# umar-ahmed/webgpu-pathtracer

Measured on AMD Instinct MI355X. Metric: Mrays/s, higher is better.
Workload: dtype f32; 1 GPU; dragon-class procedural mesh (869882 triangles) + synthetic env map, 1920x1080, 8 bounces, 16 frames (= 16 spp) per step, 863 steps = 13808 spp; triangles=869882, bvh_nodes=1739763, max_bounces=8, parallelism=single GPU

## Files before the change

include/mi3pt.h:

```cpp
#ifndef MI3PT_H
#define MI3PT_H

#include <stddef.h>
#include <stdint.h>

#ifdef __cplusplus
extern "C" {
#endif

#define MI3PT_ABI_VERSION 4

typedef enum mi3pt_status {
    MI3PT_OK = 0,
    MI3PT_ERR_INVALID = 1,
    MI3PT_ERR_NO_DEVICE = 2,
    MI3PT_ERR_HIP = 3,
    MI3PT_ERR_STATE = 4
} mi3pt_status;

#define MI3PT_TRIANGLE_STRIDE 112
#define MI3PT_BVHNODE_STRIDE 48
#define MI3PT_MATERIAL_STRIDE 64
#define MI3PT_RAYTRACE_UNIFORMS_SIZE 96
#define MI3PT_ACCUMULATE_UNIFORMS_SIZE 16
// ... 47 lines not shown
int mi3pt_device_count(int *count);
int mi3pt_device_name(int device, char *name, size_t capacity);

int mi3pt_create(int device, mi3pt_ctx **out_ctx);
int mi3pt_destroy(mi3pt_ctx *ctx);
int mi3pt_create_group(const int *devices, int ndevices, int block_rows, mi3pt_ctx **out_ctx);
int mi3pt_group_size(mi3pt_ctx *ctx, int *members);
int mi3pt_group_member(mi3pt_ctx *ctx, int index, mi3pt_ctx **member);

int mi3pt_set_stream(mi3pt_ctx *ctx, void *hip_stream);
int mi3pt_set_storage(mi3pt_ctx *ctx, int storage );

int mi3pt_set_tile(mi3pt_ctx *ctx, int rank, int nranks, int block_rows);
int mi3pt_tile_local_rows(int height, int rank, int nranks, int block_rows);
int mi3pt_tile_global_row(int local_row, int rank, int nranks, int block_rows);
int mi3pt_tile_owner(int y, int nranks, int block_rows);

int mi3pt_upload_triangles(mi3pt_ctx *ctx, const void *bytes, size_t nbytes);
int mi3pt_upload_materials(mi3pt_ctx *ctx, const void *bytes, size_t nbytes);
int mi3pt_upload_bvh(mi3pt_ctx *ctx, const void *bytes, size_t nbytes);

int mi3pt_upload_environment(mi3pt_ctx *ctx, const float *rgba, int width, int height);
int mi3pt_upload_environment_cdf(mi3pt_ctx *ctx, const float *rgba, int width, int height);

int mi3pt_resize(mi3pt_ctx *ctx, int width, int height);
int mi3pt_reset(mi3pt_ctx *ctx);

int mi3pt_set_uniforms(mi3pt_ctx *ctx, int pass , const void *bytes, size_t nbytes);

int mi3pt_submit(mi3pt_ctx *ctx, unsigned pass_mask);
int mi3pt_submit_frames(mi3pt_ctx *ctx, unsigned pass_mask, uint32_t count);
int mi3pt_sync(mi3pt_ctx *ctx);
int mi3pt_set_present_mode(mi3pt_ctx *ctx, int mode );
int mi3pt_flush(mi3pt_ctx *ctx);
int mi3pt_batch_capacity(mi3pt_ctx *ctx, int *frames);

int mi3pt_read_texture(mi3pt_ctx *ctx, int which , float *dst, size_t nfloats);
int mi3pt_read_canvas_rgba8(mi3pt_ctx *ctx, uint8_t *dst, size_t nbytes);
int mi3pt_write_texture(mi3pt_ctx *ctx, int which , const float *src, size_t nfloats);

int mi3pt_accumulation_device_ptr(mi3pt_ctx *ctx, void **dev_ptr, size_t *nbytes);
int mi3pt_bind_accumulation(mi3pt_ctx *ctx, void *dev_ptr, size_t nbytes);

int mi3pt_enable_timing(mi3pt_ctx *ctx, int enabled);
int mi3pt_pass_time_us(mi3pt_ctx *ctx, int pass, float *microseconds);
int mi3pt_raytrace_launch_stats(mi3pt_ctx *ctx, int reset, double *total_ms, uint64_t *launches, uint64_t *frames);
int mi3pt_raytrace_launch_span(mi3pt_ctx *ctx, double *span_ms);

int mi3pt_get_counters(mi3pt_ctx *ctx, uint64_t out[MI3PT_CNT_COUNT]);
int mi3pt_reset_counters(mi3pt_ctx *ctx);

int mi3pt_set_kernel_variant(mi3pt_ctx *ctx, int variant);
typedef enum mi3pt_option {
    MI3PT_OPT_WALK_MIN = 0,
    MI3PT_OPT_LEAF_MIN = 1,
    MI3PT_OPT_SHADE_SPLIT = 2,
    MI3PT_OPT_TAIL_POLICY = 3,
    MI3PT_OPT_TOP_PACKETS = 4,
    MI3PT_OPT_TRI_PAIR = 5,
    MI3PT_OPT_JOB_REVERSE = 6,
    MI3PT_OPT_JOB_GROUP = 7,
    MI3PT_OPT_JOB_CHUNK = 8,
    MI3PT_OPT_BATCH_LIMIT = 9,
    MI3PT_OPT_BATCH = 10,
    MI3PT_OPT_WAVES_PER_CU = 11,
    MI3PT_OPT_CULL = 12,
    MI3PT_OPT_WIDE = 13,
    MI3PT_OPT_GATE = 14,
    MI3PT_OPT_GATE_TIMEOUT_MS = 22,
    MI3PT_OPT_GATE_RELEASES = 23,
    MI3PT_OPT_CAMERA_BASE = 25,
    MI3PT_OPT_PACKET_ORDER = 26,
    MI3PT_OPT_SIX_WAVES = 27,
    MI3PT_OPT_LAST_BUILD = 29,
    MI3PT_OPT_WALK_ADAPT = 30,
    MI3PT_OPT_COLLAPSE = 28,
    MI3PT_OPT_DEBUG_SUPPRESS_DRAIN = 24,
    MI3PT_OPT_SLOT_SETS = 15,
    MI3PT_OPT_PIPELINE = 16,
    MI3PT_OPT_PRESENT_DEPTH = 18,
    MI3PT_OPT_HOST_ANALYSES = 19,
    MI3PT_OPT_DIAG_LITE = 21,
    MI3PT_OPT_GATHER_STAGED = 20,
    MI3PT_OPT_COST_ORDER = 17
} mi3pt_option;
int mi3pt_debug_set_option(mi3pt_ctx *ctx, int option , int value);
int mi3pt_debug_get_option(mi3pt_ctx *ctx, int option , int *value);
int mi3pt_debug_active_variant(mi3pt_ctx *ctx, int *variant);
int mi3pt_debug_last_launch(mi3pt_ctx *ctx, int *kind, int *variant, int *lean, int *workgroups);
int mi3pt_set_env_sampling(mi3pt_ctx *ctx, int enabled);
int mi3pt_set_pipelining(mi3pt_ctx *ctx, int enabled);

int mi3pt_debug_intersect(mi3pt_ctx *ctx, const float *rays, size_t n, float *out);
int mi3pt_device_build_bvh(mi3pt_ctx *ctx, void *nodes_out, size_t nodes_capacity_bytes, size_t *nnodes_out, float *build_ms);

int mi3pt_debug_set_packet_layout(mi3pt_ctx *ctx, int layout);

int mi3pt_debug_math(mi3pt_ctx *ctx, int fn, const float *a, const float *b, float *out, size_t n);

int mi3pt_debug_wave_times(mi3pt_ctx *ctx, int enable, uint64_t *out, size_t capacity_slots, size_t *slots_out);

int mi3pt_host_build_bvh(const void *triangles, size_t ntris, void *nodes_out,
                         size_t nodes_capacity_bytes, size_t *nnodes_out, int nthreads);
int mi3pt_host_build_bvh_f64(const double *positions, size_t ntris, void *nodes_out,
                             size_t nodes_capacity_bytes, size_t *nnodes_out, int nthreads);
int mi3pt_host_env_cdf(const float *rgba, int width, int height, float *cdf_rgba_out);
int mi3pt_host_eight_wide_check(const void *nodes, size_t nodes_bytes, const void *triangles, size_t triangles_bytes, int greedy, uint64_t out[6]);

#ifdef __cplusplus
}
#endif
#endif
```

webgpu-pathtracer_amd/csrc/pt_context.hip:

```cpp
#include "../../include/mi3pt.h"
#include "pt_internal.h"
#include "pt_kernels.h"

#include <hip/hip_runtime.h>
#include <cmath>
#include <cstdio>
#include <cstdlib>
#include <array>
#include <cstring>
#include <string>
#include <utility>
#include <algorithm>
#include <vector>
#include <map>
#include <chrono>
#include <thread>

static thread_local std::string g_last_error;

int pt_set_error(int code, const std::string &msg)
{
    g_last_error = msg;
    return code;
}

#define HIP_TRY(expr)                                                                       \
    do {                                                                                    \
        hipError_t e_ = (expr);                                                             \
        if (e_ != hipSuccess)                                                               \
            return pt_set_error(MI3PT_ERR_HIP, std::string(#expr) + ": " + hipGetErrorString(e_)); \
    } while (0)

struct mi3pt_ctx {
    int device = 0;
    hipStream_t own_stream = nullptr;
    hipStream_t stream = nullptr;

    void *d_tris = nullptr, *d_nodes = nullptr, *d_mats = nullptr, *d_env = nullptr, *d_cdf = nullptr;
    void *d_packets = nullptr, *d_tripk = nullptr;
    void *d_leaf_rank = nullptr;
    int leaf_cap = 0;
    bool cull_stack_ok = false;
    size_t ntris = 0, nnodes = 0, nmats = 0, npackets = 0;
    uint32_t root_ref = 0;
    uint32_t scene_flags = 0;
    bool wide_root_nested = false;
    int64_t max_tri_ref = -1;
    int64_t max_mat_ref = -1;
    bool cull_enabled = true;
    bool cull_dirty = true;
    bool cull_ok = false;
    float cull_ka = 0.0f, cull_kb = 0.0f;
    bool wide_enabled = true;
#ifdef MI3PT_EXPERIMENTS
    bool exp_force_slow_slab = false;
    double exp_cull_scale = 1.0;
#endif
    int auto_wide_variant = 10;
    bool wide_ok = false;
    bool cwide_ok = false;
    void *d_cwide = nullptr, *d_tripk64 = nullptr;
    bool cw8_tried = false;
    bool cw8_ok = false;
    void *d_cw8 = nullptr, *d_tripk8 = nullptr;
    size_t ncw8 = 0, cw8_records = 0;
    int cw8_height = 0;
    void *d_wide = nullptr;
    size_t nwide = 0;
    int wide_leaf_cap = 0;
    uint32_t wide_root = 0;
    int num_cus = 256;
    pt::RtRoute last_route = { 0, 0, false, 0, 0, false, 0 };
    int layout = 0;
    bool layout_dirty = false;
    int cost_order = 0;
    int cost_state = 0;
    uint32_t *d_tile_cost = nullptr, *d_tile_perm[2] = { nullptr, nullptr };
    size_t cost_tiles = 0;
    int perm_cur = 0;
    hipEvent_t cost_event = nullptr, perm_used[2] = { nullptr, nullptr };
    bool perm_used_valid[2] = { false, false };
    hipStream_t cost_stream = nullptr;
    uint8_t cost_key[MI3PT_RAYTRACE_UNIFORMS_SIZE] = {};
    struct GroupState *group = nullptr;
    std::map<const void *, size_t> buf_bytes;
    uint64_t scene_epoch = 1;
    uint64_t host_analyses = 0;
    bool tree_proper = false;
    bool layout_active = false;
    void *d_tris_perm = nullptr;

    int width = 0, height = 0, local_rows = 0;
    int rank = 0, nranks = 1, block_rows = 8;
    int next_rank = 0, next_nranks = 1, next_block_rows = 8;
    bool partial() const { return nranks != 1; }
    float4 *d_radiance = nullptr, *d_accum_own = nullptr, *d_accum = nullptr, *d_canvas = nullptr;
    float4 *d_slots[3] = { nullptr, nullptr, nullptr };
    int slots_alloc[3] = { 0, 0, 0 };
    int slot_sets = 2;
    int batch_cap = 1;
    float4 *last_radiance = nullptr;
    float4 *d_cam_base[2] = { nullptr, nullptr };
    uint8_t cam_base_key[2][80] = {};
    bool cam_base_valid[2] = { false, false };
    bool cam_base_enabled = true;
    int collapse = -1;
    int six_waves = -1;
    int packet_order = 0;
    uint32_t *d_canvas8 = nullptr;
    bool output_is_accum = false;
    uint64_t *d_block_counters = nullptr;
    uint32_t *d_tile_counter = nullptr;
    int job_reverse = 1;
    int job_group = -1;
    int tri_pair = 1;
    int job_chunk = PT_DEFAULT_JOB_CHUNK;
    uint32_t *d_drain_flag = nullptr;
    bool gate_enabled = false;
    uint32_t launch_seq = 0;
    int gate_timeout_ms = 2000;
    int gate_releases = 0;
    int gate_stalls_in_a_row = 0;
    bool debug_suppress_drain = false;
    hipStream_t gate_release_stream = nullptr;
    volatile uint32_t *h_drain_flag = nullptr;
    int walk_adapt = 1;
    bool deep_by_view = false;
    uint64_t *h_walk_stats = nullptr;
    uint64_t *d_walk_stats = nullptr;
    uint64_t *d_walk_prev = nullptr;
    uint64_t walk_stats_seq = 0, walk_stats_seen = 0;
    float *d_park = nullptr;
    uint32_t *d_stack_overflow = nullptr;
    void *d_fs_taps = nullptr;
    float fs_taps_res[2] = { 0.0f, 0.0f };
    bool fs_taps_valid = false;
    uint8_t *d_service = nullptr;
    uint64_t *d_wave_times = nullptr;
    int diag_lite = 0;
    int wave_times_slots = 0;
    int nblocks = 0;

    uint8_t u_rt[MI3PT_RAYTRACE_UNIFORMS_SIZE] = {};
    uint8_t u_acc[MI3PT_ACCUMULATE_UNIFORMS_SIZE] = {};
    uint8_t u_fs[MI3PT_FULLSCREEN_UNIFORMS_SIZE] = {};

    int storage = MI3PT_STORAGE_F32;
    int variant = 0;
    bool env_sampling = false;
    int tail_policy = PT_DEFAULT_TAIL_POLICY;
    int shade_split = PT_DEFAULT_SHADE_SPLIT;
    int leaf_min = PT_DEFAULT_LEAF_MIN;
    int walk_min = 0;
    int waves_per_cu = 0;
    int top_packets = 64;

    bool pipeline = true;
    hipStream_t rt_stream[2] = { nullptr, nullptr };
    hipEvent_t rt_done[2] = {}, acc_done[3] = {}, main_mark = nullptr;
    bool acc_done_valid[3] = { false, false, false };
    bool main_dirty = true;
    uint64_t seq = 0;

    struct PendingFrame {
        uint8_t u_rt[MI3PT_RAYTRACE_UNIFORMS_SIZE] = {}; uint8_t u_acc[MI3PT_ACCUMULATE_UNIFORMS_SIZE] = {};
        bool present = false;
        uint8_t u_fs[MI3PT_FULLSCREEN_UNIFORMS_SIZE] = {};
    };
    std::vector<PendingFrame> pending;
    int batch_limit_frames = 512;
    int batch_max = 256;
    hipEvent_t ev_rt[2][2] = {};
    bool ev_rt_pending[2] = { false, false };
    double rt_total_ms = 0.0, rt_last_ms = 0.0;
    uint64_t rt_launches = 0, rt_frames = 0;
    int ev_rt_frames[2] = { 0, 0 };
    int ev_rt_newest = 0;
    hipEvent_t ev_span_start = nullptr;
    bool span_started = false;

    int present_mode = MI3PT_PRESENT_EXACT;
    int present_depth = 16;
    uint64_t accum_version = 1;
    uint64_t presented_version = 0;
    bool want_present = false;
    uint8_t presented_fs[MI3PT_FULLSCREEN_UNIFORMS_SIZE] = {};

    bool timing = false;
    hipEvent_t ev[3][2] = {};
    bool ev_recorded[3] = { false, false, false };
};

static_assert(MI3PT_ENV_WIDTH == pt::ENV_W && MI3PT_ENV_HEIGHT == pt::ENV_H, "the tuned kernels' environment size is the API's");
static const int SERVICE_SLOTS = 8;
static size_t service_slot_bytes() { return (pt::service_block_bytes() + 255) / 256 * 256; }

// ... 137 lines not shown
    return true;
}

static hipError_t ctx_wait(mi3pt_ctx *ctx, hipStream_t s, hipEvent_t ev, const char *why)
{
    if (!(ctx->gate_enabled && ctx->d_drain_flag && ctx->launch_seq != 0 && ctx->gate_timeout_ms > 0))
        return ev ? hipEventSynchronize(ev) : hipStreamSynchronize(s);
    using clock = std::chrono::steady_clock;
    const clock::time_point t0 = clock::now();
    clock::time_point mark = t0;
    GateView last = gate_view(ctx);
    for (unsigned spins = 0;; spins++) {
        const hipError_t e = ev ? hipEventQuery(ev) : hipStreamQuery(s);
        if (e != hipErrorNotReady) return e;
        (void)hipGetLastError();
        const clock::time_point now = clock::now();
        if (std::chrono::duration_cast<std::chrono::milliseconds>(now - mark).count() >= (ctx->gate_timeout_ms < 8 ? ctx->gate_timeout_ms : ctx->gate_timeout_ms / 8)) {
            const GateView v = gate_view(ctx);
            if (v.word != last.word || v.busy[0] != last.busy[0] || v.busy[1] != last.busy[1]) {
                last = v;
                mark = now;
                ctx->gate_stalls_in_a_row = 0;
            } else if (std::chrono::duration_cast<std::chrono::milliseconds>(now - mark).count() >= ctx->gate_timeout_ms) {
                if (gate_launch_held(ctx)) {
                    uint32_t published = v.word;
                    if (!gate_release_from_host(ctx, v, why, &published)) {
                        ctx->gate_enabled = false;
                        pt_set_error(MI3PT_ERR_HIP, std::string("launch gate: a launch is held and no way of publishing its mark from the host works (") + why + ")");
                        return hipErrorUnknown;
                    }
                    last = gate_view(ctx);
                    last.word = published;
                }
                mark = now;
            }
        }
        if (!ctx->gate_enabled) return ev ? hipEventSynchronize(ev) : hipStreamSynchronize(s);
        if (std::chrono::duration_cast<std::chrono::microseconds>(now - t0).count() < 3000) std::this_thread::yield();
        else std::this_thread::sleep_for(std::chrono::microseconds(spins < 4096 ? 50 : 500));
    }
}
static hipError_t ctx_stream_sync(mi3pt_ctx *ctx, hipStream_t s, const char *why = "stream wait") { return ctx_wait(ctx, s, nullptr, why); }
static hipError_t ctx_event_sync(mi3pt_ctx *ctx, hipEvent_t ev, const char *why = "event wait") { return ctx_wait(ctx, nullptr, ev, why); }

extern "C" int mi3pt_create(int device, mi3pt_ctx **out_ctx)
{
    if (!out_ctx) return pt_set_error(MI3PT_ERR_INVALID, "null argument");
    *out_ctx = nullptr;
    int n = 0;
    if (hipGetDeviceCount(&n) != hipSuccess || n <= 0) {
        (void)hipGetLastError();
        return pt_set_error(MI3PT_ERR_NO_DEVICE, "HIP device not found.");
    }
    if (device < 0 || device >= n) return pt_set_error(MI3PT_ERR_NO_DEVICE, "HIP device index out of range.");
    HIP_TRY(hipSetDevice(device));
    mi3pt_ctx *ctx = new mi3pt_ctx();
    ctx->device = device;
#define CREATE_TRY(expr)                                                                                \
    do {                                                                                                \
        hipError_t e_ = (expr);                                                                         \
        if (e_ != hipSuccess) {                                                                         \
            const std::string msg_ = std::string("mi3pt_create: " #expr ": ") + hipGetErrorString(e_);  \
            (void)hipGetLastError();                                                                    \
            mi3pt_destroy(ctx);                                                                         \
            return pt_set_error(MI3PT_ERR_HIP, msg_);                                                   \
        }                                                                                               \
    } while (0)
    hipDeviceProp_t prop;
    CREATE_TRY(hipGetDeviceProperties(&prop, device));
    ctx->num_cus = prop.multiProcessorCount > 0 ? prop.multiProcessorCount : 256;
    int prio_least = 0, prio_greatest = 0;
    CREATE_TRY(hipDeviceGetStreamPriorityRange(&prio_least, &prio_greatest));
    if (hipStreamCreateWithPriority(&ctx->own_stream, hipStreamNonBlocking, prio_greatest) != hipSuccess) {
        (void)hipGetLastError();
        CREATE_TRY(hipStreamCreateWithFlags(&ctx->own_stream, hipStreamNonBlocking));
    }
    ctx->stream = ctx->own_stream;
    for (int k = 0; k < 2; k++) {
        if (hipStreamCreateWithPriority(&ctx->rt_stream[k], hipStreamNonBlocking, prio_least) != hipSuccess) {
            (void)hipGetLastError();
            CREATE_TRY(hipStreamCreateWithFlags(&ctx->rt_stream[k], hipStreamNonBlocking));
        }
        CREATE_TRY(hipEventCreateWithFlags(&ctx->rt_done[k], hipEventDisableTiming));
    }
    for (int k = 0; k < 3; k++) CREATE_TRY(hipEventCreateWithFlags(&ctx->acc_done[k], hipEventDisableTiming));
    CREATE_TRY(hipEventCreateWithFlags(&ctx->main_mark, hipEventDisableTiming));
    for (int k = 0; k < 2; k++)
        for (int j = 0; j < 2; j++) CREATE_TRY(hipEventCreate(&ctx->ev_rt[k][j]));
    for (int p = 0; p < 3; p++)
        for (int k = 0; k < 2; k++) CREATE_TRY(hipEventCreate(&ctx->ev[p][k]));
    CREATE_TRY(hipEventCreate(&ctx->ev_span_start));
    CREATE_TRY(hipEventCreateWithFlags(&ctx->cost_event, hipEventDisableTiming));
    for (int k = 0; k < 2; k++) CREATE_TRY(hipEventCreateWithFlags(&ctx->perm_used[k], hipEventDisableTiming));
    CREATE_TRY(hipStreamCreateWithFlags(&ctx->cost_stream, hipStreamNonBlocking));
    const size_t env_bytes = (size_t)MI3PT_ENV_WIDTH * MI3PT_ENV_HEIGHT * 16;
    CREATE_TRY(hipMalloc(&ctx->d_env, env_bytes));
    CREATE_TRY(hipMalloc(&ctx->d_cdf, env_bytes));
    CREATE_TRY(hipMalloc((void **)&ctx->d_tile_counter, 256));
    CREATE_TRY(hipMalloc((void **)&ctx->d_stack_overflow, (size_t)2 * pt::PT_MAX_RESIDENT_WAVES * pt::SM_OVERFLOW_ENTRIES * 64 * 4));
    CREATE_TRY(hipMalloc((void **)&ctx->d_park, (size_t)2 * pt::PT_MAX_RESIDENT_WAVES * 6 * 64 * sizeof(float)));
    if (hipHostMalloc((void **)&ctx->h_walk_stats, 64, hipHostMallocMapped) == hipSuccess &&
        hipHostGetDevicePointer((void **)&ctx->d_walk_stats, ctx->h_walk_stats, 0) == hipSuccess &&
        hipMalloc((void **)&ctx->d_walk_prev, 32) == hipSuccess) {
        std::memset(ctx->h_walk_stats, 0, 64);
        CREATE_TRY(hipMemsetAsync(ctx->d_walk_prev, 0, 32, ctx->stream));
    } else {
        (void)hipGetLastError();
        if (ctx->h_walk_stats) (void)hipHostFree(ctx->h_walk_stats);
        ctx->h_walk_stats = nullptr; ctx->d_walk_stats = nullptr;
    }
    CREATE_TRY(hipMalloc((void **)&ctx->d_service, (size_t)(SERVICE_SLOTS + 1) * service_slot_bytes()));
    CREATE_TRY(hipMalloc(&ctx->d_fs_taps, pt::fullscreen_taps_bytes()));
    CREATE_TRY(hipMemsetAsync(ctx->d_tile_counter, 0, 256, ctx->stream));
    if (hipExtMallocWithFlags((void **)&ctx->d_drain_flag, 8, hipMallocSignalMemory) == hipSuccess) {
        CREATE_TRY(hipMemsetAsync(ctx->d_drain_flag, 0, 8, ctx->stream));
        ctx->gate_enabled = !profiler_attached();
        hipPointerAttribute_t attr;
        if (hipPointerGetAttributes(&attr, ctx->d_drain_flag) == hipSuccess && attr.type == hipMemoryTypeHost && attr.hostPointer)
            ctx->h_drain_flag = static_cast<volatile uint32_t *>(attr.hostPointer);
        else
            (void)hipGetLastError();
    } else {
        (void)hipGetLastError();
        ctx->d_drain_flag = nullptr;
    }
    CREATE_TRY(hipMemsetAsync(ctx->d_env, 0, env_bytes, ctx->stream));
    CREATE_TRY(hipMemsetAsync(ctx->d_cdf, 0, env_bytes, ctx->stream));
    CREATE_TRY(hipStreamSynchronize(ctx->stream));
#undef CREATE_TRY
#ifdef MI3PT_EXPERIMENTS
    {
        static const struct { const char *name; int opt; } env_opts[] = {
            { "MI3PT_WALK_MIN", MI3PT_OPT_WALK_MIN }, { "MI3PT_LEAF_MIN", MI3PT_OPT_LEAF_MIN }, { "MI3PT_SHADE_SPLIT", MI3PT_OPT_SHADE_SPLIT },
            { "MI3PT_TAIL_POLICY", MI3PT_OPT_TAIL_POLICY }, { "MI3PT_TOP_PACKETS", MI3PT_OPT_TOP_PACKETS }, { "MI3PT_TRI_PAIR", MI3PT_OPT_TRI_PAIR },
            { "MI3PT_JOB_REVERSE", MI3PT_OPT_JOB_REVERSE }, { "MI3PT_JOB_GROUP", MI3PT_OPT_JOB_GROUP }, { "MI3PT_JOB_CHUNK", MI3PT_OPT_JOB_CHUNK },
            { "MI3PT_BATCH_LIMIT", MI3PT_OPT_BATCH_LIMIT }, { "MI3PT_BATCH", MI3PT_OPT_BATCH }, { "MI3PT_WAVES_PER_CU", MI3PT_OPT_WAVES_PER_CU },
            { "MI3PT_CULL", MI3PT_OPT_CULL }, { "MI3PT_WIDE", MI3PT_OPT_WIDE }, { "MI3PT_GATE", MI3PT_OPT_GATE }, { "MI3PT_SLOT_SETS", MI3PT_OPT_SLOT_SETS },
            { "MI3PT_PIPELINE", MI3PT_OPT_PIPELINE }, { "MI3PT_COST_ORDER", MI3PT_OPT_COST_ORDER }, { "MI3PT_DIAG_LITE", MI3PT_OPT_DIAG_LITE },
        };
        for (const auto &eo : env_opts)
            if (const char *e = std::getenv(eo.name)) (void)mi3pt_debug_set_option(ctx, eo.opt, std::atoi(e));
        if (std::getenv("MI3PT_FORCE_SLOW_SLAB")) ctx->exp_force_slow_slab = true;
        if (const char *e = std::getenv("MI3PT_CULL_SCALE")) ctx->exp_cull_scale = std::atof(e);
    }
#endif
    std::memset(ctx->u_rt, 0, sizeof ctx->u_rt);
    std::memset(ctx->u_acc, 0, sizeof ctx->u_acc);
    std::memset(ctx->u_fs, 0, sizeof ctx->u_fs);
    *out_ctx = ctx;
    return MI3PT_OK;
}

static void free_textures(mi3pt_ctx *ctx)
{
    for (void *p : { (void *)ctx->d_radiance, (void *)ctx->d_slots[0], (void *)ctx->d_slots[1], (void *)ctx->d_slots[2], (void *)ctx->d_accum_own,
                     (void *)ctx->d_canvas, (void *)ctx->d_canvas8, (void *)ctx->d_block_counters, (void *)ctx->d_cam_base[0], (void *)ctx->d_cam_base[1] })
        if (p) (void)hipFree(p);
    ctx->d_cam_base[0] = ctx->d_cam_base[1] = nullptr;
    ctx->cam_base_valid[0] = ctx->cam_base_valid[1] = false;
    ctx->d_radiance = ctx->d_slots[0] = ctx->d_slots[1] = ctx->d_slots[2] = ctx->last_radiance = nullptr;
    ctx->slots_alloc[0] = ctx->slots_alloc[1] = ctx->slots_alloc[2] = 0;
    ctx->d_accum_own = ctx->d_accum = ctx->d_canvas = nullptr;
    ctx->d_canvas8 = nullptr;
    ctx->d_block_counters = nullptr;
    ctx->nblocks = 0;
}

extern "C" int mi3pt_destroy(mi3pt_ctx *ctx)
{
    PT_GROUP(ctx, group_destroy(ctx));
    if (!ctx) return MI3PT_OK;
    (void)hipSetDevice(ctx->device);
    if (ctx->d_drain_flag && ctx->launch_seq != 0) {
        hipStream_t rel = nullptr;
        if (hipStreamCreateWithFlags(&rel, hipStreamNonBlocking) == hipSuccess) {
            if (hipStreamWriteValue32(rel, ctx->d_drain_flag, ctx->launch_seq, 0) == hipSuccess) (void)hipStreamSynchronize(rel);
            (void)hipStreamDestroy(rel);
        }
        (void)hipGetLastError();
    }
    if (ctx->stream) (void)hipStreamSynchronize(ctx->stream);
    for (int k = 0; k < 2; k++)
        if (ctx->rt_stream[k]) (void)hipStreamSynchronize(ctx->rt_stream[k]);
    if (ctx->gate_release_stream) (void)hipStreamDestroy(ctx->gate_release_stream);
    if (ctx->h_walk_stats) (void)hipHostFree(ctx->h_walk_stats);
    if (ctx->d_walk_prev) (void)hipFree(ctx->d_walk_prev);
    free_textures(ctx);
    for (void *p : { ctx->d_cw8, ctx->d_tripk8, ctx->d_cwide, ctx->d_tripk64, ctx->d_wide, ctx->d_tris, ctx->d_tris_perm, ctx->d_nodes, ctx->d_mats, ctx->d_env, ctx->d_cdf, ctx->d_packets, ctx->d_tripk, ctx->d_leaf_rank,
                     (void *)ctx->d_tile_counter, (void *)ctx->d_drain_flag, (void *)ctx->d_wave_times, (void *)ctx->d_stack_overflow, (void *)ctx->d_park, (void *)ctx->d_service, ctx->d_fs_taps })
        if (p) (void)hipFree(p);
    for (int p = 0; p < 3; p++)
        for (int k = 0; k < 2; k++)
            if (ctx->ev[p][k]) (void)hipEventDestroy(ctx->ev[p][k]);
    for (int k = 0; k < 2; k++) {
        if (ctx->rt_stream[k]) (void)hipStreamDestroy(ctx->rt_stream[k]);
        if (ctx->rt_done[k]) (void)hipEventDestroy(ctx->rt_done[k]);
    }
    for (int k = 0; k < 3; k++)
        if (ctx->acc_done[k]) (void)hipEventDestroy(ctx->acc_done[k]);
    if (ctx->main_mark) (void)hipEventDestroy(ctx->main_mark);
    if (ctx->ev_span_start) (void)hipEventDestroy(ctx->ev_span_start);
    if (ctx->cost_event) (void)hipEventDestroy(ctx->cost_event);
    for (int k = 0; k < 2; k++)
        if (ctx->perm_used[k]) (void)hipEventDestroy(ctx->perm_used[k]);
    if (ctx->cost_stream) (void)hipStreamDestroy(ctx->cost_stream);
    for (void *q : { (void *)ctx->d_tile_cost, (void *)ctx->d_tile_perm[0], (void *)ctx->d_tile_perm[1] })
        if (q) (void)hipFree(q);
    for (int k = 0; k < 2; k++)
        for (int j = 0; j < 2; j++)
            if (ctx->ev_rt[k][j]) (void)hipEventDestroy(ctx->ev_rt[k][j]);
    if (ctx->own_stream) (void)hipStreamDestroy(ctx->own_stream);
    delete ctx;
    return MI3PT_OK;
}

extern "C" int mi3pt_set_stream(mi3pt_ctx *ctx, void *hip_stream)
{
    PT_GROUP(ctx, group_unsupported("mi3pt_set_stream: a device group runs on its members' own streams"));
    if (int rc = require_idle(ctx)) return rc;
    HIP_TRY(ctx_stream_sync(ctx, ctx->stream));
    ctx->stream = hip_stream ? static_cast<hipStream_t>(hip_stream) : ctx->own_stream;
    ctx->main_dirty = true;
    ctx->acc_done_valid[0] = ctx->acc_done_valid[1] = ctx->acc_done_valid[2] = false;
    return MI3PT_OK;
}

extern "C" int mi3pt_set_storage(mi3pt_ctx *ctx, int storage)
{
    PT_GROUP_ALL(ctx, true, mi3pt_set_storage(m, storage));
    if (!ctx) return pt_set_error(MI3PT_ERR_INVALID, "null context");
    if (storage != MI3PT_STORAGE_F32 && storage != MI3PT_STORAGE_F16)
        return pt_set_error(MI3PT_ERR_INVALID, "storage must be MI3PT_STORAGE_F32 or MI3PT_STORAGE_F16");
    if (int rc = require_idle(ctx)) return rc;
    ctx->storage = storage;
    return MI3PT_OK;
}

extern "C" int mi3pt_set_env_sampling(mi3pt_ctx *ctx, int enabled)
{
    PT_GROUP_ALL(ctx, false, mi3pt_set_env_sampling(m, enabled));
    if (int rc = require_idle(ctx)) return rc;
    if (enabled && !ctx->d_cdf)
        return pt_set_error(MI3PT_ERR_STATE, "environment CDF texture has not been uploaded (mi3pt_upload_environment_cdf)");
    ctx->env_sampling = enabled != 0;
    return MI3PT_OK;
}

extern "C" int mi3pt_set_kernel_variant(mi3pt_ctx *ctx, int variant)
{
    PT_GROUP_ALL(ctx, false, mi3pt_set_kernel_variant(m, variant));
    if (!ctx) return pt_set_error(MI3PT_ERR_INVALID, "null context");
    if (variant < 0 || variant > 14) return pt_set_error(MI3PT_ERR_INVALID, "variant must be 0..14");
#ifndef MI3PT_EXPERIMENTS
    if (variant == 3 || variant == 5 || variant == 6 || variant == 8 || variant == 11 || variant == 12)
        return pt_set_error(MI3PT_ERR_INVALID, "kernel variants 3, 5, 6, 8 (measured, not adopted) and 11, 12 (superseded by 13) exist in the experiment build only: make -C webgpu-pathtracer_amd/csrc experiments");
#endif
    if (int rc = require_idle(ctx)) return rc;
    ctx->variant = variant;
    if (variant == 14 && !ctx->cw8_ok && !ctx->cw8_tried) ctx->cull_dirty = true;
    return MI3PT_OK;
}

static void recompute_batch_cap(mi3pt_ctx *ctx)
{
    if (ctx->width == 0) return;
    ctx->batch_cap = batch_limit(ctx, ctx->nranks);
    const size_t tex_bytes = (size_t)ctx->local_rows * ctx->width * 16;
    size_t free_b = 0, total_b = 0;
    if (tex_bytes && hipMemGetInfo(&free_b, &total_b) == hipSuccess) {
        const size_t per_frame = (size_t)ctx->slot_sets * tex_bytes;
        const size_t fit = (free_b / 4) / per_frame;
        if ((size_t)ctx->batch_cap > fit) ctx->batch_cap = fit < 1 ? 1 : (int)fit;
    } else {
        (void)hipGetLastError();
    }
}

extern "C" int mi3pt_debug_set_option(mi3pt_ctx *ctx, int option, int value)
{
    PT_GROUP(ctx, group_set_option(ctx, option, value));
    if (!ctx) return pt_set_error(MI3PT_ERR_INVALID, "null context");
    if (int rc = require_idle(ctx)) return rc;
    switch (option) {
    case MI3PT_OPT_WALK_MIN: ctx->walk_min = value; break;
    case MI3PT_OPT_LEAF_MIN: ctx->leaf_min = value; break;
    case MI3PT_OPT_SHADE_SPLIT: ctx->shade_split = value; break;
    case MI3PT_OPT_TAIL_POLICY: ctx->tail_policy = value; break;
    case MI3PT_OPT_TOP_PACKETS: ctx->top_packets = value; break;
    case MI3PT_OPT_TRI_PAIR: ctx->tri_pair = value != 0; break;
    case MI3PT_OPT_JOB_REVERSE: ctx->job_reverse = value != 0; break;
    case MI3PT_OPT_JOB_GROUP: ctx->job_group = value; break;
    case MI3PT_OPT_JOB_CHUNK: ctx->job_chunk = (value < 1 || value > 64) ? 1 : value; break;
    case MI3PT_OPT_BATCH_LIMIT:
        if (value < 1 || value > 4096) return pt_set_error(MI3PT_ERR_INVALID, "batch limit must be in [1, 4096]");
        ctx->batch_limit_frames = value;
        if (ctx->batch_max > ctx->batch_limit_frames) ctx->batch_max = ctx->batch_limit_frames;
        recompute_batch_cap(ctx);
        break;
    case MI3PT_OPT_BATCH:
        ctx->batch_max = value < 1 ? 1 : (value > ctx->batch_limit_frames ? ctx->batch_limit_frames : value);
        recompute_batch_cap(ctx);
        break;
    case MI3PT_OPT_WAVES_PER_CU: ctx->waves_per_cu = value; break;
    case MI3PT_OPT_CULL: ctx->cull_enabled = value != 0; break;
    case MI3PT_OPT_WIDE: ctx->wide_enabled = value != 0; break;
    case MI3PT_OPT_GATE: ctx->gate_enabled = value != 0 && ctx->d_drain_flag != nullptr; if (ctx->gate_enabled) { ctx->gate_releases = 0; ctx->gate_stalls_in_a_row = 0; } break;
    case MI3PT_OPT_CAMERA_BASE: ctx->cam_base_enabled = value != 0; break;
    case MI3PT_OPT_SIX_WAVES: ctx->six_waves = value < 0 ? -1 : (value != 0 ? 1 : 0); break;
    case MI3PT_OPT_WALK_ADAPT: ctx->walk_adapt = value != 0; if (!ctx->walk_adapt) ctx->deep_by_view = false; break;
    case MI3PT_OPT_COLLAPSE:
        if (value < -1 || value > 1) return pt_set_error(MI3PT_ERR_INVALID, "collapse: 0 greedy, 1 optimal, -1 by the packet width");
        if (ctx->collapse != value) { ctx->collapse = value; ctx->cull_dirty = true; }
        break;
    case MI3PT_OPT_PACKET_ORDER:
        if (value < 0 || value > 2) return pt_set_error(MI3PT_ERR_INVALID, "packet order: 0 breadth-first, 1 depth-first, 2 treelets");
        if (ctx->packet_order != value) { ctx->packet_order = value; ctx->cull_dirty = true; }
        break;
    case MI3PT_OPT_GATE_TIMEOUT_MS: if (value < 0) return pt_set_error(MI3PT_ERR_INVALID, "gate time-out must be >= 0 ms"); ctx->gate_timeout_ms = value; break;
    case MI3PT_OPT_GATE_RELEASES: return pt_set_error(MI3PT_ERR_INVALID, "MI3PT_OPT_GATE_RELEASES is read-only");
    case MI3PT_OPT_LAST_BUILD: return pt_set_error(MI3PT_ERR_INVALID, "MI3PT_OPT_LAST_BUILD is read-only");
    case MI3PT_OPT_DEBUG_SUPPRESS_DRAIN: ctx->debug_suppress_drain = value != 0; break;
    case MI3PT_OPT_SLOT_SETS:
        if (value != 2 && value != 3) return pt_set_error(MI3PT_ERR_INVALID, "slot sets: 2 or 3");
        if (ctx->width != 0 && value != ctx->slot_sets) return pt_set_error(MI3PT_ERR_STATE, "slot sets must be chosen before mi3pt_resize");
        ctx->slot_sets = value;
        break;
    case MI3PT_OPT_PIPELINE: ctx->pipeline = value != 0; break;
    case MI3PT_OPT_COST_ORDER: ctx->cost_order = value < 0 ? 0 : (value > 2 ? 2 : value); ctx->cost_state = 0; break;
    case MI3PT_OPT_HOST_ANALYSES: return pt_set_error(MI3PT_ERR_INVALID, "MI3PT_OPT_HOST_ANALYSES is read-only");
    case MI3PT_OPT_DIAG_LITE:
#ifdef MI3PT_EXPERIMENTS
        ctx->diag_lite = value != 0;
        break;
#else
        return pt_set_error(MI3PT_ERR_INVALID, "MI3PT_OPT_DIAG_LITE: the lean build with lane counts exists in the experiment build only");
#endif
    case MI3PT_OPT_GATHER_STAGED: break;
    case MI3PT_OPT_PRESENT_DEPTH:
        if (value < 1) return pt_set_error(MI3PT_ERR_INVALID, "present depth must be >= 1");
        ctx->present_depth = value;
        break;
    default:
        return pt_set_error(MI3PT_ERR_INVALID, "unknown option");
    }
    return MI3PT_OK;
}

static int group_get_option(mi3pt_ctx *g, int option, int *value);

extern "C" int mi3pt_debug_get_option(mi3pt_ctx *ctx, int option, int *value)
{
    PT_GROUP(ctx, group_get_option(ctx, option, value));
    if (!ctx || !value) return pt_set_error(MI3PT_ERR_INVALID, "null argument");
    switch (option) {
    case MI3PT_OPT_HOST_ANALYSES: *value = (int)ctx->host_analyses; break;
    case MI3PT_OPT_DIAG_LITE: *value = ctx->diag_lite; break;
    case MI3PT_OPT_GATHER_STAGED: *value = 0; break;
    case MI3PT_OPT_WALK_MIN: *value = ctx->walk_min; break;
    case MI3PT_OPT_LEAF_MIN: *value = ctx->leaf_min; break;
    case MI3PT_OPT_SHADE_SPLIT: *value = ctx->shade_split; break;
    case MI3PT_OPT_TAIL_POLICY: *value = ctx->tail_policy; break;
    case MI3PT_OPT_TOP_PACKETS: *value = ctx->top_packets; break;
    case MI3PT_OPT_TRI_PAIR: *value = ctx->tri_pair ? 1 : 0; break;
    case MI3PT_OPT_JOB_REVERSE: *value = ctx->job_reverse ? 1 : 0; break;
    case MI3PT_OPT_JOB_GROUP: *value = ctx->job_group; break;
    case MI3PT_OPT_JOB_CHUNK: *value = ctx->job_chunk; break;
    case MI3PT_OPT_BATCH_LIMIT: *value = ctx->batch_limit_frames; break;
    case MI3PT_OPT_BATCH: *value = ctx->batch_max; break;
    case MI3PT_OPT_WAVES_PER_CU: *value = ctx->waves_per_cu; break;
    case MI3PT_OPT_CULL: *value = ctx->cull_enabled ? 1 : 0; break;
    case MI3PT_OPT_WIDE: *value = ctx->wide_enabled ? 1 : 0; break;
    case MI3PT_OPT_GATE: *value = ctx->gate_enabled ? 1 : 0; break;
    case MI3PT_OPT_CAMERA_BASE: *value = ctx->cam_base_enabled ? 1 : 0; break;
    case MI3PT_OPT_SIX_WAVES: *value = ctx->six_waves; break;
    case MI3PT_OPT_COLLAPSE: *value = ctx->collapse; break;
    case MI3PT_OPT_WALK_ADAPT: *value = ctx->walk_adapt; break;
    case MI3PT_OPT_LAST_BUILD: *value = ctx->last_route.waves | (ctx->last_route.ymax ? 0x100 : 0) | (ctx->last_route.walk_min << 16); break;
    case MI3PT_OPT_PACKET_ORDER: *value = ctx->packet_order; break;
    case MI3PT_OPT_GATE_TIMEOUT_MS: *value = ctx->gate_timeout_ms; break;
    case MI3PT_OPT_GATE_RELEASES: *value = ctx->gate_releases; break;
    case MI3PT_OPT_DEBUG_SUPPRESS_DRAIN: *value = ctx->debug_suppress_drain ? 1 : 0; break;
    case MI3PT_OPT_SLOT_SETS: *value = ctx->slot_sets; break;
    case MI3PT_OPT_PIPELINE: *value = ctx->pipeline ? 1 : 0; break;
    case MI3PT_OPT_COST_ORDER: *value = ctx->cost_order; break;
    case MI3PT_OPT_PRESENT_DEPTH: *value = ctx->present_depth; break;
    default:
        return pt_set_error(MI3PT_ERR_INVALID, "unknown option");
    }
    return MI3PT_OK;
}

extern "C" int mi3pt_debug_active_variant(mi3pt_ctx *ctx, int *variant)
{
    PT_GROUP(ctx, mi3pt_debug_active_variant(group_member0(ctx), variant));
    if (!ctx || !variant) return pt_set_error(MI3PT_ERR_INVALID, "null argument");
    if (int rc = require_idle(ctx)) return rc;
    if (int rc = check_scene(ctx)) return rc;
    if (int rc = prepare_layout(ctx)) return rc;
    if (int rc = prepare_cull(ctx)) return rc;
    *variant = pick_variant(ctx);
    return MI3PT_OK;
}

extern "C" int mi3pt_debug_last_launch(mi3pt_ctx *ctx, int *kind, int *variant, int *lean, int *workgroups)
{
    PT_GROUP(ctx, mi3pt_debug_last_launch(group_member0(ctx), kind, variant, lean, workgroups));
    if (!ctx) return pt_set_error(MI3PT_ERR_INVALID, "null context");
    if (kind) *kind = ctx->last_route.kind;
    if (variant) *variant = ctx->last_route.variant;
    if (lean) *lean = ctx->last_route.lean ? 1 : 0;
    if (workgroups) *workgroups = ctx->last_route.blocks;
    return MI3PT_OK;
}

extern "C" int mi3pt_set_pipelining(mi3pt_ctx *ctx, int enabled)
{
    PT_GROUP_ALL(ctx, false, mi3pt_set_pipelining(m, enabled));
    if (int rc = require_idle(ctx)) return rc;
    HIP_TRY(ctx_stream_sync(ctx, ctx->stream));
    ctx->pipeline = enabled != 0;
    ctx->main_dirty = true;
    return MI3PT_OK;
}

extern "C" int mi3pt_set_tile(mi3pt_ctx *ctx, int rank, int nranks, int block_rows)
{
    PT_GROUP(ctx, group_unsupported("mi3pt_set_tile: a device group deals the image's row blocks to its members itself"));
    if (!ctx) return pt_set_error(MI3PT_ERR_INVALID, "null context");
    if (nranks <= 0 || rank < 0 || rank >= nranks || block_rows <= 0)
        return pt_set_error(MI3PT_ERR_INVALID, "bad tile: need 0 <= rank < nranks, block_rows > 0");
    ctx->next_rank = rank;
    ctx->next_nranks = nranks;
    ctx->next_block_rows = block_rows;
    return MI3PT_OK;
}

static int replace_buffer(mi3pt_ctx *ctx, void **dst, const void *bytes, size_t nbytes)
{
    void *fresh = nullptr;
    HIP_TRY(hipMalloc(&fresh, nbytes));
    hipError_t e = ctx_stream_sync(ctx, ctx->stream, "upload");
    if (e == hipSuccess) e = hipMemcpyAsync(fresh, bytes, nbytes, hipMemcpyHostToDevice, ctx->stream);
    if (e == hipSuccess) e = ctx_stream_sync(ctx, ctx->stream);
    if (e != hipSuccess) {
        (void)hipFree(fresh);
        return pt_set_error(MI3PT_ERR_HIP, std::string("upload: ") + hipGetErrorString(e));
    }
    if (*dst) { ctx->buf_bytes.erase(*dst); (void)hipFree(*dst); }
    *dst = fresh;
    ctx->buf_bytes[fresh] = nbytes;
    ctx->scene_epoch++;
    return MI3PT_OK;
}

static pt::TriPacket tri_packet_of(const uint8_t *rec)
{
// ... 116 lines not shown
        } else {
            for (size_t off : { (size_t)32, (size_t)36 }) {
                const int32_t c = ldi(r, off);
                if (c >= 0 && ((size_t)c >= n || (size_t)c <= i))
                    return pt_set_error(MI3PT_ERR_INVALID,
                                        "BVH child index must be greater than its parent's and inside the buffer "
                                        "(breadth-first order, raytrace.ts:667-694)");
            }
            packet_of[i] = (uint32_t)npackets++;
        }
    }
    std::vector<pt::NodePacket> pk;
    build_packets(src, n, packet_of, npackets, nullptr, pk);
    auto ref_of = [&](int32_t child) -> uint32_t { return child_ref(src, packet_of, nullptr, child); };
    std::vector<uint32_t> leaf_rank((size_t)(max_tri + 1 > 0 ? max_tri + 1 : 1), 0xffffffffu);
    int leaf_cap = 0;
    bool cull_stack_ok = false, tree_proper = false;
    {
        std::vector<uint32_t> st;
        std::vector<uint8_t> seen(n, 0);
        st.push_back(0);
        size_t visited = 0, worst = 0, worst_internal = 0, internal = 0;
        uint32_t rank = 0;
        bool proper = true;
        auto is_leaf = [&](uint32_t node) { return ldi(src + (size_t)node * MI3PT_BVHNODE_STRIDE, 28) == 1; };
        if (!is_leaf(0)) internal = 1;
        while (!st.empty() && proper) {
            if (st.size() > worst) worst = st.size();
            if (internal > worst_internal) worst_internal = internal;
            const uint32_t node = st.back();
            st.pop_back();
            if (seen[node]) { proper = false; break; }
            seen[node] = 1;
            visited++;
            const uint8_t *r = src + (size_t)node * MI3PT_BVHNODE_STRIDE;
            if (ldi(r, 28) == 1) {
                const int32_t ti = ldi(r, 40);
                if (leaf_rank[(size_t)ti] != 0xffffffffu) { proper = false; break; }
                leaf_rank[(size_t)ti] = rank++;
            } else {
                internal--;
                const int32_t left = ldi(r, 32), right = ldi(r, 36);
                if (left < 0 || right < 0) { proper = false; break; }
                st.push_back((uint32_t)left);
                st.push_back((uint32_t)right);
                internal += (is_leaf((uint32_t)left) ? 0 : 1) + (is_leaf((uint32_t)right) ? 0 : 1);
            }
        }
        if (proper && worst < 64 && (int)worst_internal <= pt::SM_LDS_DEPTH - 4) leaf_cap = pt::SM_LDS_DEPTH - (int)worst_internal;
        tree_proper = proper && worst < 64;
        (void)visited;
        cull_stack_ok = false;
        if (proper && worst < 64 && !is_leaf(0)) {
            std::vector<std::pair<uint32_t, uint32_t>> work;
            work.emplace_back(0u, 1u);
            size_t worst_any = 1;
            while (!work.empty()) {
                const auto [node, occ] = work.back();
                work.pop_back();
                const uint8_t *r = src + (size_t)node * MI3PT_BVHNODE_STRIDE;
                const uint32_t kids[2] = { (uint32_t)ldi(r, 32), (uint32_t)ldi(r, 36) };
                const uint32_t m = (is_leaf(kids[0]) ? 0u : 1u) + (is_leaf(kids[1]) ? 0u : 1u);
                for (uint32_t c : kids) {
                    if (is_leaf(c)) continue;
                    const uint32_t oc = occ - 1u + m;
                    if (oc > worst_any) worst_any = oc;
                    work.emplace_back(c, oc);
                }
            }
            cull_stack_ok = worst_any <= (size_t)pt::SM_CULL_STACK_MAX;
        }
    }
    if (int rc = replace_buffer(ctx, &ctx->d_nodes, bytes, nbytes)) return rc;
    if (int rc = replace_buffer(ctx, &ctx->d_packets, pk.data(), pk.size() * sizeof(pt::NodePacket))) return rc;
    if (int rc = replace_buffer(ctx, &ctx->d_leaf_rank, leaf_rank.data(), leaf_rank.size() * sizeof(uint32_t))) return rc;
    ctx->leaf_cap = leaf_cap;
    ctx->cull_stack_ok = cull_stack_ok;
    ctx->tree_proper = tree_proper;
    ctx->nnodes = n;
    ctx->npackets = npackets;
    ctx->root_ref = ref_of(0);
    ctx->scene_flags = node_box_safe(src, 0) ? 1u : 0u;
    ctx->max_tri_ref = max_tri;
    ctx->cull_dirty = true;
    ctx->cost_state = 0;
    ctx->layout_active = false;
    ctx->layout_dirty = ctx->layout != 0;
    ctx->scene_epoch++;
    ctx->host_analyses++;
    return MI3PT_OK;
}

static int upload_env_like(mi3pt_ctx *ctx, void *dst, const float *rgba, int width, int height)
{
    if (int rc = require_idle(ctx)) return rc;
    if (!rgba) return pt_set_error(MI3PT_ERR_INVALID, "null argument");
    if (width != MI3PT_ENV_WIDTH || height != MI3PT_ENV_HEIGHT)
        return pt_set_error(MI3PT_ERR_INVALID,
                            "Environment texture must be 1024x512 pixels. Please resize the texture and try again.");
    const size_t nbytes = (size_t)width * height * 16;
    HIP_TRY(ctx_stream_sync(ctx, ctx->stream, "upload"));
    HIP_TRY(hipMemcpyAsync(dst, rgba, nbytes, hipMemcpyHostToDevice, ctx->stream));
    HIP_TRY(ctx_stream_sync(ctx, ctx->stream));
    ctx->scene_epoch++;
    return MI3PT_OK;
}

extern "C" int mi3pt_upload_environment(mi3pt_ctx *ctx, const float *rgba, int width, int height)
{
    PT_GROUP(ctx, mi3pt_upload_environment(group_member0(ctx), rgba, width, height));
    if (!ctx) return pt_set_error(MI3PT_ERR_INVALID, "null context");
    return upload_env_like(ctx, ctx->d_env, rgba, width, height);
}

extern "C" int mi3pt_upload_environment_cdf(mi3pt_ctx *ctx, const float *rgba, int width, int height)
{
    PT_GROUP(ctx, mi3pt_upload_environment_cdf(group_member0(ctx), rgba, width, height));
    if (!ctx) return pt_set_error(MI3PT_ERR_INVALID, "null context");
    return upload_env_like(ctx, ctx->d_cdf, rgba, width, height);
}

static pt::Tile tile_of(const mi3pt_ctx *ctx)
{
    pt::Tile t;
    t.tex_w = ctx->width; t.tex_h = ctx->height; t.local_rows = ctx->local_rows;
    t.rank = ctx->rank; t.nranks = ctx->nranks; t.block_rows = ctx->block_rows;
    return t;
}

static int zero_textures(mi3pt_ctx *ctx)
{
    const size_t tex_bytes = (size_t)ctx->local_rows * ctx->width * 16;
    const size_t canvas_px = (size_t)ctx->width * ctx->height;
    if (tex_bytes) {
        HIP_TRY(hipMemsetAsync(ctx->d_radiance, 0, tex_bytes, ctx->stream));
        HIP_TRY(hipMemsetAsync(ctx->d_accum, 0, tex_bytes, ctx->stream));
    }
    if (canvas_px) {
        HIP_TRY(hipMemsetAsync(ctx->d_canvas, 0, canvas_px * 16, ctx->stream));
        HIP_TRY(hipMemsetAsync(ctx->d_canvas8, 0, canvas_px * 4, ctx->stream));
    }
    ctx->output_is_accum = false;
    ctx->last_radiance = ctx->d_radiance;
    ctx->main_dirty = true;
    ctx->accum_version++;
    ctx->presented_version = 0;
    ctx->want_present = false;
    return MI3PT_OK;
}

static int batch_limit(const mi3pt_ctx *ctx, int nranks)
{
    long b = (long)ctx->batch_max * (nranks > 1 ? nranks : 1);
    if (ctx->batch_max <= 1) b = 1;
    return (int)(b > ctx->batch_limit_frames ? ctx->batch_limit_frames : b);
}

extern "C" int mi3pt_resize(mi3pt_ctx *ctx, int width, int height)
{
    PT_GROUP(ctx, group_resize(ctx, width, height));
    if (int rc = require_idle(ctx)) return rc;
    if (width <= 0 || height <= 0 || width > 32768 || height > 32768)
        return pt_set_error(MI3PT_ERR_INVALID, "width/height must be in [1, 32768]");
    HIP_TRY(ctx_stream_sync(ctx, ctx->stream));
    for (int k = 0; k < 2; k++) HIP_TRY(ctx_stream_sync(ctx, ctx->rt_stream[k]));
    free_textures(ctx);
// ... 653 lines not shown
    ctx->presented_version = 0;
    ctx->want_present = false;
    return MI3PT_OK;
}

static int auto_exact_wide(const mi3pt_ctx *ctx)
{
#ifdef MI3PT_EXPERIMENTS
    return ctx->auto_wide_variant;
#else
    (void)ctx;
    return 10;
#endif
}

static int pick_variant(const mi3pt_ctx *ctx)
{
    if (ctx->env_sampling) return 2;
    const bool defer_ok = ctx->leaf_cap >= 4;
    const bool cull_ok = ctx->cull_stack_ok && ctx->cull_ok && !ctx->cull_dirty;
    const bool wide_ok = cull_ok && ctx->wide_ok;
    if (ctx->variant == 0)
        return cull_ok && ctx->cull_enabled ? (wide_ok && ctx->wide_enabled ? (ctx->cwide_ok ? 13 : auto_exact_wide(ctx)) : 9) : (defer_ok ? 7 : 4);
    if (ctx->variant == 14 && cull_ok && ctx->cw8_ok) return 14;
    if ((ctx->variant == 13 || ctx->variant == 14) && wide_ok && ctx->cwide_ok) return 13;
    if ((ctx->variant == 13 || ctx->variant == 14) && !(wide_ok && ctx->cwide_ok)) return wide_ok ? auto_exact_wide(ctx) : (cull_ok ? 9 : (defer_ok ? 7 : 4));
    if (ctx->variant >= 10 && ctx->variant <= 12 && !wide_ok) return cull_ok ? 9 : (defer_ok ? 7 : 4);
    if (ctx->variant == 9 && !cull_ok) return defer_ok ? 7 : 4;
    if ((ctx->variant == 7 || ctx->variant == 8) && !defer_ok) return ctx->variant == 8 ? 6 : 4;
    return ctx->variant;
}
static int pick_walk(const mi3pt_ctx *ctx) { return ctx->variant == 0 ? 3 : (ctx->variant >= 4 ? 3 : (ctx->variant == 3 ? 2 : ctx->variant)); }

static pt::AccUniforms acc_uniforms(const mi3pt_ctx *ctx)
{
    pt::AccUniforms a;
    a.res_w = ldu(ctx->u_acc, 0); a.res_h = ldu(ctx->u_acc, 4);
    a.frame = ldu(ctx->u_acc, 8); a.enabled = ldu(ctx->u_acc, 12);
    return a;
}

static pt::RtLaunch build_launch(const mi3pt_ctx *ctx, const uint8_t *u, const pt::AccUniforms &acc)
{
    pt::RtLaunch L;
    L.scene = scene_refs(ctx);
    L.un.res_x = ldf(u, 0); L.un.res_y = ldf(u, 4); L.un.aspect = ldf(u, 8);
    L.un.frame = ldu(u, 12);
    L.un.max_bounces = ldi(u, 16); L.un.samples_per_frame = ldi(u, 20);
    for (int k = 0; k < 3; k++) { L.un.cam_pos[k] = ldf(u, 32 + 4 * k); L.un.cam_dir[k] = ldf(u, 48 + 4 * k); }
    L.un.fov = ldf(u, 60); L.un.focal_distance = ldf(u, 64); L.un.aperture = ldf(u, 68);
    L.un.env_intensity = ldf(u, 80); L.un.env_rotation = ldf(u, 84);
    L.acc = acc;
    L.tile = tile_of(ctx);
    L.radiance = ctx->d_radiance;
    L.slot_pixels = (size_t)ctx->local_rows * ctx->width;
    L.nframes = 1;
    L.accum = ctx->d_accum;
    L.block_counters = ctx->d_block_counters;
    L.tile_counter = ctx->d_tile_counter;
    L.job_chunk = ctx->job_chunk;
    L.job_reverse = ctx->job_reverse;
    L.tri_pair = ctx->tri_pair;
    L.job_group = ctx->job_group;
    if (ctx->job_group < 0) {
        const int tiles_x = (L.tile.tex_w + 7) / 8, ntiles = tiles_x * ((L.tile.local_rows + 7) / 8);
        const int rows = ntiles / 8 / tiles_x;
        L.job_group = (rows < 1 ? 1 : rows) * tiles_x;
    }
    L.wave_times = ctx->d_wave_times;
    L.diag_lite = ctx->diag_lite;
    L.stack_overflow = ctx->d_stack_overflow;
    L.store_f16 = ctx->storage == MI3PT_STORAGE_F16;
    L.walk_min = ctx->variant == 5 ? 48 : (ctx->walk_min > 0 ? ctx->walk_min
                                           : ((pick_variant(ctx) == 13 ? (ctx->nwide >= (1u << 20) && ctx->wide_ok && ctx->cwide_ok) : (pick_variant(ctx) == 14 && ctx->ncw8 >= (1u << 19))) ? PT_DEEP_WALK_MIN : PT_DEFAULT_WALK_MIN));
    L.leaf_min = ctx->leaf_min;
    L.shade_split = ctx->shade_split;
    L.tail_policy = ctx->tail_policy;
    L.drain_flag = nullptr;
    L.drain_seq = 0;
    L.waves_per_cu = ctx->waves_per_cu;
    L.num_cus = ctx->num_cus;
    L.service = nullptr;
    L.cam_base = nullptr;
    L.park = ctx->d_park;
    L.six_waves = ctx->six_waves;
    L.tile_cost = nullptr;
    L.tile_perm = nullptr;
    L.top_packets = ctx->top_packets;
    if (pick_variant(ctx) == 13 && (size_t)L.top_packets > ctx->nwide) L.top_packets = (int)ctx->nwide;
    if (pick_variant(ctx) == 1) L.scene.tris = static_cast<const float4 *>(ctx->d_tris);
    return L;
}

static pt::AccUniforms acc_from(const uint8_t *u)
{
    pt::AccUniforms a;
    a.res_w = ldu(u, 0); a.res_h = ldu(u, 4); a.frame = ldu(u, 8); a.enabled = ldu(u, 12);
    return a;
}

static int collect_rt_time(mi3pt_ctx *ctx, int par)
{
    if (!ctx->ev_rt_pending[par]) return MI3PT_OK;
    HIP_TRY(ctx_event_sync(ctx, ctx->ev_rt[par][1]));
    float ms = 0.0f;
    HIP_TRY(hipEventElapsedTime(&ms, ctx->ev_rt[par][0], ctx->ev_rt[par][1]));
    ctx->rt_total_ms += ms;
    ctx->rt_last_ms = ms;
    ctx->rt_launches++;
    ctx->rt_frames += (uint64_t)ctx->ev_rt_frames[par];
    ctx->ev_rt_pending[par] = false;
    return MI3PT_OK;
}

static int ensure_slots(mi3pt_ctx *ctx, int par , int n)
{
    if (ctx->slots_alloc[par] >= n) return MI3PT_OK;
    const size_t tex_bytes = (size_t)ctx->local_rows * ctx->width * 16;
    int want = n <= 1 ? 1 : (n <= 8 ? 8 : ctx->batch_cap);
    if (want > ctx->batch_cap) want = ctx->batch_cap;
    if (want > n && tex_bytes) {
        size_t free_b = 0, total_b = 0;
        if (hipMemGetInfo(&free_b, &total_b) == hipSuccess) {
            const size_t fit = (free_b / 2) / ((size_t)ctx->slot_sets * tex_bytes);
            if ((size_t)want > fit) want = fit > (size_t)n ? (int)fit : n;
        } else {
            (void)hipGetLastError();
        }
    }
    if (want < n) want = n;
    float4 *fresh = nullptr;
    hipError_t e = hipMalloc((void **)&fresh, tex_bytes ? tex_bytes * (size_t)want : 16);
    if (e != hipSuccess && want > n) {
        (void)hipGetLastError();
        want = n;
        e = hipMalloc((void **)&fresh, tex_bytes ? tex_bytes * (size_t)want : 16);
    }
    if (e != hipSuccess) {
        (void)hipGetLastError();
        return pt_set_error(MI3PT_ERR_HIP, std::string("radiance slots: ") + hipGetErrorString(e));
    }
    if (ctx->d_slots[par]) (void)hipFree(ctx->d_slots[par]);
    ctx->d_slots[par] = fresh;
    ctx->slots_alloc[par] = want;
    if (want == ctx->batch_cap && want > 8) {
        for (int other = 0; other < ctx->slot_sets; other++) {
            if (other == par || ctx->slots_alloc[other] >= want) continue;
            float4 *more = nullptr;
            if (hipMalloc((void **)&more, tex_bytes ? tex_bytes * (size_t)want : 16) != hipSuccess) { (void)hipGetLastError(); break; }
            if (ctx->d_slots[other]) (void)hipFree(ctx->d_slots[other]);
            ctx->d_slots[other] = more;
            ctx->slots_alloc[other] = want;
        }
    }
    return MI3PT_OK;
}

static int cost_order_collect(mi3pt_ctx *ctx, bool wait)
{
    if (ctx->cost_state != 1) return MI3PT_OK;
    if (!wait) {
        const hipError_t q = hipEventQuery(ctx->cost_event);
        if (q == hipErrorNotReady) { (void)hipGetLastError(); return MI3PT_OK; }
        if (q != hipSuccess) { (void)hipGetLastError(); ctx->cost_state = 0; return MI3PT_OK; }
    }
    const size_t n = ctx->cost_tiles;
// ... 2 lines not shown
    std::vector<uint32_t> cost(n), perm(n);
    HIP_TRY(hipStreamWaitEvent(ctx->cost_stream, ctx->cost_event, 0));
    HIP_TRY(hipMemcpyAsync(cost.data(), ctx->d_tile_cost, n * 4, hipMemcpyDeviceToHost, ctx->cost_stream));
    HIP_TRY(hipStreamSynchronize(ctx->cost_stream));
    if (ctx->perm_used_valid[target]) HIP_TRY(hipEventSynchronize(ctx->perm_used[target]));
    std::vector<uint32_t> sorted(cost);
    const size_t q = n / 4;
    std::nth_element(sorted.begin(), sorted.begin() + (std::ptrdiff_t)q, sorted.end());
    const uint32_t cut = sorted[q];
    size_t at = 0;
    if (ctx->cost_order == 2) {
        for (size_t t = 0; t < n; t++) perm[t] = (uint32_t)t;
        std::stable_sort(perm.begin(), perm.end(), [&](uint32_t a, uint32_t b) { return cost[a] > cost[b]; });
        at = n;
    } else {
        for (size_t t = n; t-- > 0;) if (cost[t] >= cut) perm[at++] = (uint32_t)t;
        for (size_t t = n; t-- > 0;) if (cost[t] < cut) perm[at++] = (uint32_t)t;
    }
    HIP_TRY(hipMemcpyAsync(ctx->d_tile_perm[target], perm.data(), n * 4, hipMemcpyHostToDevice, ctx->cost_stream));
    HIP_TRY(hipStreamSynchronize(ctx->cost_stream));
    ctx->perm_cur = target;
    ctx->cost_state = 2;
    return MI3PT_OK;
}

static int cost_order_prepare(mi3pt_ctx *ctx, pt::RtLaunch &L, const uint8_t *u_rt, int variant, hipStream_t rs, bool *measuring, bool *ordered)
{
    *measuring = *ordered = false;
    const size_t n = (size_t)pt::raytrace_grid_blocks(L.tile);
    if (!ctx->cost_order || variant < 9 || variant > 13 || L.un.samples_per_frame != 1 || n < 2) return MI3PT_OK;
    uint8_t key[MI3PT_RAYTRACE_UNIFORMS_SIZE];
    std::memcpy(key, u_rt, sizeof key);
    std::memset(key + 12, 0, 4);
    if (ctx->cost_tiles != n) {
        HIP_TRY(ctx_stream_sync(ctx, ctx->rt_stream[0]));
        HIP_TRY(ctx_stream_sync(ctx, ctx->rt_stream[1]));
        for (uint32_t **q : { &ctx->d_tile_cost, &ctx->d_tile_perm[0], &ctx->d_tile_perm[1] }) {
            if (*q) (void)hipFree(*q);
            *q = nullptr;
            HIP_TRY(hipMalloc((void **)q, n * 4));
        }
        ctx->cost_tiles = n;
        ctx->cost_state = 0;
        ctx->perm_used_valid[0] = ctx->perm_used_valid[1] = false;
    }
    if (ctx->cost_state != 0 && std::memcmp(key, ctx->cost_key, sizeof key) != 0) ctx->cost_state = 0;
    if (int rc = cost_order_collect(ctx, false)) return rc;
    if (ctx->cost_state == 0) {
        std::memcpy(ctx->cost_key, key, sizeof key);
        HIP_TRY(hipMemsetAsync(ctx->d_tile_cost, 0, n * 4, rs));
        L.tile_cost = ctx->d_tile_cost;
        *measuring = true;
    } else if (ctx->cost_state == 2) {
        L.tile_perm = ctx->d_tile_perm[ctx->perm_cur];
        L.job_reverse = 0;
        *ordered = true;
    }
    return MI3PT_OK;
}

static int run_fullscreen(mi3pt_ctx *ctx, const uint8_t *u_fs);

#define WALK_ADAPT_ENTER 40.0
#define WALK_ADAPT_LEAVE 30.0
static void adapt_walk(mi3pt_ctx *ctx)
{
    if (!ctx->walk_adapt || !ctx->h_walk_stats) { ctx->deep_by_view = false; return; }
    volatile uint64_t *h = ctx->h_walk_stats;
    uint64_t best_seq = ctx->walk_stats_seen, box = 0, rays = 0;
    for (int par = 0; par < 2; par++) {
        const uint64_t s0 = __atomic_load_n(&ctx->h_walk_stats[4 * par], __ATOMIC_ACQUIRE);
        const uint64_t b = h[4 * par + 1], r = h[4 * par + 2];
        const uint64_t s1 = __atomic_load_n(&ctx->h_walk_stats[4 * par], __ATOMIC_ACQUIRE);
        if (s0 == s1 && s0 > best_seq && s0 <= ctx->walk_stats_seq) { best_seq = s0; box = b; rays = r; }
    }
    if (best_seq == ctx->walk_stats_seen) return;
    ctx->walk_stats_seen = best_seq;
    if (rays < 65536) return;
    const double per_ray = (double)box / (double)rays;
    if (per_ray >= WALK_ADAPT_ENTER) ctx->deep_by_view = true;
    else if (per_ray <= WALK_ADAPT_LEAVE) ctx->deep_by_view = false;
}

static int launch_batch(mi3pt_ctx *ctx, const mi3pt_ctx::PendingFrame *frames, int n)
{
    adapt_walk(ctx);
    const mi3pt_ctx::PendingFrame &first = frames[0];
    const pt::AccUniforms acc = acc_from(first.u_acc);
    pt::RtLaunch L = build_launch(ctx, first.u_rt, acc);
    const bool f16 = ctx->storage == MI3PT_STORAGE_F16;
    const int par = (int)(ctx->seq & 1u);
    const int set = (int)(ctx->seq % (uint64_t)ctx->slot_sets);
    if (int rc = ensure_slots(ctx, set, n)) {
        if (n == 1 || ensure_slots(ctx, set, 1) != MI3PT_OK) return rc;
        ctx->batch_cap = 1;
        return MI3PT_ERR_STATE;
    }
    ctx->seq++;
    hipStream_t rs = ctx->rt_stream[par];
    if (ctx->main_dirty) {
        HIP_TRY(hipEventRecord(ctx->main_mark, ctx->stream));
        HIP_TRY(hipStreamWaitEvent(ctx->rt_stream[0], ctx->main_mark, 0));
        HIP_TRY(hipStreamWaitEvent(ctx->rt_stream[1], ctx->main_mark, 0));
        ctx->main_dirty = false;
    }
    if (ctx->acc_done_valid[set]) HIP_TRY(hipStreamWaitEvent(rs, ctx->acc_done[set], 0));
    L.radiance = ctx->d_slots[set];
    L.nframes = n;
    if (ctx->deep_by_view && ctx->walk_min == 0 && L.walk_min == PT_DEFAULT_WALK_MIN && pick_variant(ctx) == 13 &&
        (long long)pt::raytrace_grid_blocks(L.tile) * n >= 250000)
        L.walk_min = PT_DEEP_WALK_MIN;
    L.block_counters = ctx->d_block_counters + (size_t)par * ctx->nblocks * pt::CNT_COUNT;
    L.tile_counter = ctx->d_tile_counter + par * 32;
    L.stack_overflow = ctx->d_stack_overflow + (size_t)par * pt::PT_MAX_RESIDENT_WAVES * pt::SM_OVERFLOW_ENTRIES * 64;
    L.park = ctx->d_park + (size_t)par * pt::PT_MAX_RESIDENT_WAVES * 6 * 64;
    L.service = reinterpret_cast<pt::RtService *>(ctx->d_service + (size_t)((ctx->seq - 1) % SERVICE_SLOTS) * service_slot_bytes());
    bool cost_measuring = false, cost_ordered = false;
    if (int rc = cost_order_prepare(ctx, L, first.u_rt, pick_variant(ctx), rs, &cost_measuring, &cost_ordered)) return rc;
    if (ctx->timing)
        if (int rc = collect_rt_time(ctx, par)) return rc;
    const uint32_t seq_before = ctx->launch_seq;
    const bool launches = pt::raytrace_grid_blocks(L.tile) > 0;
    ctx->last_route = pt::raytrace_route(L, pick_variant(ctx));
    uint32_t publish_after = 0;
    if (ctx->gate_enabled && launches) {
        if (ctx->launch_seq != 0 &&
            hipStreamWaitValue32(rs, ctx->d_drain_flag, ctx->launch_seq, hipStreamWaitValueGte, 0xffffffffu) != hipSuccess) {
            (void)hipGetLastError();
            ctx->gate_enabled = false;
        } else if (ctx->last_route.kind == 1) {
            ++ctx->launch_seq;
            if (!ctx->debug_suppress_drain) { L.drain_flag = ctx->d_drain_flag; L.drain_seq = ctx->launch_seq; }
        } else {
            publish_after = ++ctx->launch_seq;
        }
    }
    if (ctx->cam_base_enabled && ctx->last_route.kind == 1 && launches) {
        uint8_t key[80];
        std::memset(key, 0, sizeof key);
        std::memcpy(key, first.u_rt, 12);
        std::memcpy(key + 12, first.u_rt + 32, 36);
        const int32_t tl[6] = { L.tile.tex_w, L.tile.tex_h, L.tile.local_rows, L.tile.rank, L.tile.nranks, L.tile.block_rows };
        std::memcpy(key + 48, tl, sizeof tl);
        if (!ctx->d_cam_base[par]) {
            if (hipMalloc((void **)&ctx->d_cam_base[par], L.slot_pixels * sizeof(float4)) != hipSuccess) {
                (void)hipGetLastError();
                ctx->d_cam_base[par] = nullptr;
                ctx->cam_base_enabled = false;
            }
            ctx->cam_base_valid[par] = false;
        }
        if (ctx->d_cam_base[par]) {
            if (!ctx->cam_base_valid[par] || std::memcmp(key, ctx->cam_base_key[par], sizeof key) != 0) {
                pt::launch_camera_base(L, ctx->d_cam_base[par], rs);
                std::memcpy(ctx->cam_base_key[par], key, sizeof key);
                ctx->cam_base_valid[par] = true;
            }
            L.cam_base = ctx->d_cam_base[par];
        }
    }
    pt::launch_raytrace_setup(L, false, pick_variant(ctx), rs);
    if (ctx->timing) {
        HIP_TRY(hipEventRecord(ctx->ev_rt[par][0], rs));
        if (!ctx->span_started) { HIP_TRY(hipEventRecord(ctx->ev_span_start, rs)); ctx->span_started = true; }
    }
    pt::launch_raytrace(L, false, pick_variant(ctx), rs);
    if (publish_after && !ctx->debug_suppress_drain && hipStreamWriteValue32(rs, ctx->d_drain_flag, publish_after, 0) != hipSuccess) {
        (void)hipGetLastError();
        ctx->gate_enabled = false;
    }
    if (cost_measuring && launches) { HIP_TRY(hipEventRecord(ctx->cost_event, rs)); ctx->cost_state = 1; }
    if (cost_ordered && launches) { HIP_TRY(hipEventRecord(ctx->perm_used[ctx->perm_cur], rs)); ctx->perm_used_valid[ctx->perm_cur] = true; }
    if (hipError_t e = hipGetLastError()) {
        if (ctx->launch_seq != seq_before && hipStreamWriteValue32(rs, ctx->d_drain_flag, ctx->launch_seq, 0) != hipSuccess) {
            (void)hipGetLastError();
            ctx->launch_seq = seq_before;
            ctx->gate_enabled = false;
        }
        return pt_set_error(MI3PT_ERR_HIP, std::string("raytrace launch: ") + hipGetErrorString(e));
    }
    if (ctx->timing) {
        HIP_TRY(hipEventRecord(ctx->ev_rt[par][1], rs));
        ctx->ev_rt_pending[par] = true;
        ctx->ev_rt_frames[par] = n;
        ctx->ev_rt_newest = par;
    }
    HIP_TRY(hipEventRecord(ctx->rt_done[par], rs));
    HIP_TRY(hipStreamWaitEvent(ctx->stream, ctx->rt_done[par], 0));
    if (ctx->walk_adapt && ctx->h_walk_stats && launches && ctx->last_route.kind == 1 && ctx->last_route.lean && ctx->last_route.variant == 13 && ctx->walk_min == 0) {
        pt::launch_walk_stats(L.block_counters, ctx->nblocks, ctx->d_walk_prev + 2 * par, ctx->d_walk_stats + 4 * par, ++ctx->walk_stats_seq, rs);
        (void)hipGetLastError();
    }
    ctx->last_radiance = L.radiance + (size_t)(n - 1) * L.slot_pixels;
    ctx->output_is_accum = true;
    for (int k = 0; k < n;) {
        int e = k;
        while (e < n - 1 && !frames[e].present) e++;
        const bool last_run = e == n - 1;
        pt::AccUniforms a = acc;
        a.frame = acc.frame + (uint32_t)k;
        if (ctx->timing && last_run) HIP_TRY(hipEventRecord(ctx->ev[1][0], ctx->stream));
        pt::launch_accumulate_batch(a, L.tile, L.radiance + (size_t)k * L.slot_pixels, L.slot_pixels, e - k + 1, ctx->d_accum, f16, ctx->stream);
        HIP_TRY(hipGetLastError());
        if (ctx->timing && last_run) { HIP_TRY(hipEventRecord(ctx->ev[1][1], ctx->stream)); ctx->ev_recorded[1] = true; }
        ctx->accum_version++;
        if (frames[e].present)
            if (int rc = run_fullscreen(ctx, frames[e].u_fs)) return rc;
        k = e + 1;
    }
    HIP_TRY(hipEventRecord(ctx->acc_done[set], ctx->stream));
    ctx->acc_done_valid[set] = true;
    return MI3PT_OK;
}

static int flush_pending(mi3pt_ctx *ctx)
{
    if (ctx->pending.empty()) return MI3PT_OK;
    std::vector<mi3pt_ctx::PendingFrame> q;
    q.swap(ctx->pending);
    size_t at = 0;
    while (at < q.size()) {
        int n = (int)(q.size() - at);
        if (n > ctx->batch_cap) n = ctx->batch_cap;
        const int rc = launch_batch(ctx, &q[at], n);
        if (rc == MI3PT_ERR_STATE && n > 1) continue;
        if (rc != MI3PT_OK) return rc;
        at += (size_t)n;
    }
    return MI3PT_OK;
}

static int require_idle(mi3pt_ctx *ctx)
{
    if (int rc = require_ctx(ctx)) return rc;
    return flush_pending(ctx);
}

static bool batch_compatible(const mi3pt_ctx::PendingFrame &last, const mi3pt_ctx::PendingFrame &next)
{
    if (std::memcmp(last.u_rt, next.u_rt, 12) || std::memcmp(last.u_rt + 16, next.u_rt + 16, 80)) return false;
    if (std::memcmp(last.u_acc, next.u_acc, 8) || std::memcmp(last.u_acc + 12, next.u_acc + 12, 4)) return false;
    return ldu(next.u_rt, 12) == ldu(last.u_rt, 12) + 1u && ldu(next.u_acc, 8) == ldu(last.u_acc, 8) + 1u;
}

static int run_fullscreen(mi3pt_ctx *ctx, const uint8_t *u_fs)
{
    pt::FsUniforms fs;
    fs.res_x = ldf(u_fs, 0); fs.res_y = ldf(u_fs, 4); fs.aspect = ldf(u_fs, 8);
    fs.scaling = ldf(u_fs, 12); fs.denoise = ldu(u_fs, 16); fs.tonemapping = ldu(u_fs, 20);
    const float4 *tex = ctx->output_is_accum ? ctx->d_accum : ctx->last_radiance;
    if (ctx->timing) HIP_TRY(hipEventRecord(ctx->ev[2][0], ctx->stream));
    const bool taps_current = ctx->fs_taps_valid && std::memcmp(ctx->fs_taps_res, &fs.res_x, 4) == 0 && std::memcmp(ctx->fs_taps_res + 1, &fs.res_y, 4) == 0;
    pt::launch_fullscreen(fs, tex, ctx->width, ctx->height, ctx->width, ctx->height, ctx->d_fs_taps, taps_current, ctx->d_canvas,
                          ctx->d_canvas8, ctx->stream);
    if (hipError_t e = hipGetLastError()) {
        ctx->fs_taps_valid = false;
        return pt_set_error(MI3PT_ERR_HIP, std::string("fullscreen launch: ") + hipGetErrorString(e));
    }
    if (fs.denoise == 1u) { ctx->fs_taps_res[0] = fs.res_x; ctx->fs_taps_res[1] = fs.res_y; ctx->fs_taps_valid = true; }
    if (ctx->timing) { HIP_TRY(hipEventRecord(ctx->ev[2][1], ctx->stream)); ctx->ev_recorded[2] = true; }
    ctx->presented_version = ctx->accum_version;
    std::memcpy(ctx->presented_fs, u_fs, sizeof ctx->presented_fs);
    return MI3PT_OK;
}

extern "C" int mi3pt_submit(mi3pt_ctx *ctx, unsigned pass_mask)
{
    PT_GROUP(ctx, group_submit_frames(ctx, pass_mask, 1));
    if (int rc = require_ctx(ctx)) return rc;
    if (ctx->width == 0) return pt_set_error(MI3PT_ERR_STATE, "submit before resize");
    if (pass_mask & ~(MI3PT_SUBMIT_RAYTRACE | MI3PT_SUBMIT_ACCUMULATE | MI3PT_SUBMIT_FULLSCREEN))
        return pt_set_error(MI3PT_ERR_INVALID, "unknown bits in pass_mask");
    const bool do_rt = pass_mask & MI3PT_SUBMIT_RAYTRACE, do_acc = pass_mask & MI3PT_SUBMIT_ACCUMULATE;
    const bool do_fs = pass_mask & MI3PT_SUBMIT_FULLSCREEN;
    if (do_fs && ctx->partial())
// ... 509 lines not shown
    delete gs;
    g->group = nullptr;
    delete g;
    return rc;
}

static int group_resize(mi3pt_ctx *g, int width, int height)
{
    GroupState *gs = g->group;
    gs->width = gs->height = 0;
    if (int rc = group_each(g, true, [&](mi3pt_ctx *m) { return mi3pt_resize(m, width, height); })) return rc;
    gs->width = width;
    gs->height = height;
    g->width = width; g->height = height;
    gs->gathered = true;
    gs->want_present = false;
    return MI3PT_OK;
}

static int group_reset(mi3pt_ctx *g)
{
    GroupState *gs = g->group;
    if (int rc = group_each(g, true, [&](mi3pt_ctx *m) { return mi3pt_reset(m); })) return rc;
    gs->gathered = true;
    gs->want_present = false;
    return MI3PT_OK;
}

static int group_set_uniforms(mi3pt_ctx *g, int pass, const void *bytes, size_t nbytes)
{
    if (pass == MI3PT_PASS_FULLSCREEN) return mi3pt_set_uniforms(g->group->present, pass, bytes, nbytes);
    return group_each(g, false, [&](mi3pt_ctx *m) { return mi3pt_set_uniforms(m, pass, bytes, nbytes); });
}

static size_t group_global_row(int ly, int i, int n, int br)
{
    const int b = ly / br;
    return ((size_t)b * (size_t)n + (size_t)((b & 1) ? n - 1 - i : i)) * (size_t)br + (size_t)(ly % br);
}

static int clone_buffer(mi3pt_ctx *dst, void **dptr, const mi3pt_ctx *src, const void *sptr)
{
    if (*dptr) { dst->buf_bytes.erase(*dptr); (void)hipFree(*dptr); *dptr = nullptr; }
    if (!sptr) return MI3PT_OK;
    const auto it = src->buf_bytes.find(sptr);
    if (it == src->buf_bytes.end()) return pt_set_error(MI3PT_ERR_STATE, "group: a scene buffer of unknown size");
    HIP_TRY(hipMalloc(dptr, it->second ? it->second : 16));
    if (it->second) HIP_TRY(hipMemcpyPeerAsync(*dptr, dst->device, sptr, src->device, it->second, dst->stream));
    dst->buf_bytes[*dptr] = it->second;
    return MI3PT_OK;
}

static int clone_scene(mi3pt_ctx *dst, const mi3pt_ctx *src)
{
    if (int rc = require_idle(dst)) return rc;
    HIP_TRY(ctx_stream_sync(dst, dst->stream));
    for (int k = 0; k < 2; k++) HIP_TRY(ctx_stream_sync(dst, dst->rt_stream[k]));
    if (int rc = clone_buffer(dst, &dst->d_tris, src, src->d_tris)) return rc;
    if (int rc = clone_buffer(dst, &dst->d_tris_perm, src, src->d_tris_perm)) return rc;
    if (int rc = clone_buffer(dst, &dst->d_nodes, src, src->d_nodes)) return rc;
    if (int rc = clone_buffer(dst, &dst->d_mats, src, src->d_mats)) return rc;
    if (int rc = clone_buffer(dst, &dst->d_packets, src, src->d_packets)) return rc;
    if (int rc = clone_buffer(dst, &dst->d_tripk, src, src->d_tripk)) return rc;
    if (int rc = clone_buffer(dst, &dst->d_leaf_rank, src, src->d_leaf_rank)) return rc;
    if (int rc = clone_buffer(dst, &dst->d_wide, src, src->d_wide)) return rc;
    if (int rc = clone_buffer(dst, &dst->d_cwide, src, src->d_cwide)) return rc;
    if (int rc = clone_buffer(dst, &dst->d_tripk64, src, src->d_tripk64)) return rc;
    if (int rc = clone_buffer(dst, &dst->d_cw8, src, src->d_cw8)) return rc;
    if (int rc = clone_buffer(dst, &dst->d_tripk8, src, src->d_tripk8)) return rc;
    const size_t env_bytes = (size_t)MI3PT_ENV_WIDTH * MI3PT_ENV_HEIGHT * 16;
    HIP_TRY(hipMemcpyPeerAsync(dst->d_env, dst->device, src->d_env, src->device, env_bytes, dst->stream));
    HIP_TRY(hipMemcpyPeerAsync(dst->d_cdf, dst->device, src->d_cdf, src->device, env_bytes, dst->stream));
    HIP_TRY(ctx_stream_sync(dst, dst->stream));
    dst->ntris = src->ntris; dst->nnodes = src->nnodes; dst->nmats = src->nmats; dst->npackets = src->npackets;
    dst->root_ref = src->root_ref; dst->scene_flags = src->scene_flags; dst->wide_root_nested = src->wide_root_nested;
    dst->max_tri_ref = src->max_tri_ref; dst->max_mat_ref = src->max_mat_ref;
    dst->leaf_cap = src->leaf_cap; dst->cull_stack_ok = src->cull_stack_ok; dst->tree_proper = src->tree_proper;
    dst->cull_dirty = src->cull_dirty; dst->cull_ok = src->cull_ok; dst->cull_ka = src->cull_ka; dst->cull_kb = src->cull_kb;
    dst->auto_wide_variant = src->auto_wide_variant; dst->wide_ok = src->wide_ok; dst->cwide_ok = src->cwide_ok; dst->nwide = src->nwide;
    dst->cw8_ok = src->cw8_ok; dst->cw8_tried = src->cw8_tried; dst->ncw8 = src->ncw8; dst->cw8_records = src->cw8_records; dst->cw8_height = src->cw8_height;
    dst->wide_leaf_cap = src->wide_leaf_cap; dst->wide_root = src->wide_root;
    dst->layout = src->layout; dst->layout_dirty = src->layout_dirty; dst->layout_active = src->layout_active;
    dst->cost_state = 0;
    dst->main_dirty = true;
    dst->scene_epoch++;
    return MI3PT_OK;
}

static int group_sync_scene(mi3pt_ctx *g)
{
    GroupState *gs = g->group;
    mi3pt_ctx *m0 = gs->members[0];
    if (int rc = require_ctx(m0)) return rc;
    if (int rc = check_scene(m0)) return rc;
    if (int rc = prepare_layout(m0)) return rc;
    if (int rc = prepare_cull(m0)) return rc;
    if (m0->scene_epoch == gs->cloned_epoch) return MI3PT_OK;
    for (size_t i = 1; i < gs->members.size(); i++)
        if (int rc = clone_scene(gs->members[i], m0)) return rc;
    gs->cloned_epoch = m0->scene_epoch;
    return MI3PT_OK;
}

static int group_submit_frames(mi3pt_ctx *g, unsigned pass_mask, uint32_t count)
{
    GroupState *gs = g->group;
    if (gs->width == 0) return pt_set_error(MI3PT_ERR_STATE, "submit before resize");
    const unsigned sample = pass_mask & (MI3PT_SUBMIT_RAYTRACE | MI3PT_SUBMIT_ACCUMULATE);
    if (pass_mask & MI3PT_SUBMIT_RAYTRACE)
        if (int rc = group_sync_scene(g)) return rc;
    if (sample) {
        if (int rc = group_each(g, false, [&](mi3pt_ctx *m) { return count == 1 ? mi3pt_submit(m, sample) : mi3pt_submit_frames(m, sample, count); })) return rc;
        if (sample & MI3PT_SUBMIT_ACCUMULATE) gs->gathered = false;
    }
    if (pass_mask & MI3PT_SUBMIT_FULLSCREEN) gs->want_present = true;
    return MI3PT_OK;
}

static int group_flush(mi3pt_ctx *g) { return group_each(g, false, [&](mi3pt_ctx *m) { return mi3pt_flush(m); }); }

static int group_sync(mi3pt_ctx *g)
{
    if (int rc = group_flush(g)) return rc;
    return group_each(g, true, [&](mi3pt_ctx *m) { return mi3pt_sync(m); });
}

static int gather_member(GroupState *gs, int i, bool direct)
{
    mi3pt_ctx *p = gs->present;
    const mi3pt_ctx *m = gs->members[(size_t)i];
    const int n = (int)gs->members.size(), br = gs->block_rows, W = gs->width, H = gs->height;
    const size_t row_bytes = (size_t)W * 16, block_bytes = row_bytes * (size_t)br;
    uint8_t *dst = reinterpret_cast<uint8_t *>(p->d_accum);
    const uint8_t *src = reinterpret_cast<const uint8_t *>(m->d_accum);
    const int rows = m->local_rows;
    if (rows == 0) return MI3PT_OK;
    const int full = rows / br, tail = rows - full * br;
    const size_t grow = group_global_row(full * br, i, n, br);
    if (tail > 0 && (int)grow + tail > H) return pt_set_error(MI3PT_ERR_STATE, "gather: tile geometry mismatch");
    hipMemcpyKind kind = hipMemcpyDeviceToDevice;
    if (!direct) {
        const size_t need = (size_t)rows * row_bytes;
        if (gs->stage_bytes < need) {
            if (gs->stage) (void)hipHostFree(gs->stage);
            gs->stage = nullptr; gs->stage_bytes = 0;
            HIP_TRY(hipHostMalloc(&gs->stage, need, hipHostMallocDefault));
            gs->stage_bytes = need;
        }
        HIP_TRY(hipSetDevice(m->device));
        HIP_TRY(hipMemcpy(gs->stage, src, need, hipMemcpyDeviceToHost));
        HIP_TRY(hipSetDevice(p->device));
        src = static_cast<const uint8_t *>(gs->stage);
        kind = hipMemcpyHostToDevice;
    }
    const int n_even = (full + 1) / 2, n_odd = full / 2;
    if (n_even > 0)
        HIP_TRY(hipMemcpy2DAsync(dst + (size_t)i * block_bytes, 2 * (size_t)n * block_bytes, src, 2 * block_bytes, block_bytes, (size_t)n_even, kind, p->stream));
    if (n_odd > 0)
        HIP_TRY(hipMemcpy2DAsync(dst + (size_t)(n + n - 1 - i) * block_bytes, 2 * (size_t)n * block_bytes, src + block_bytes, 2 * block_bytes, block_bytes, (size_t)n_odd, kind, p->stream));
    if (tail > 0)
        HIP_TRY(hipMemcpyAsync(dst + grow * row_bytes, src + (size_t)full * block_bytes, (size_t)tail * row_bytes, kind, p->stream));
    if (!direct) HIP_TRY(ctx_stream_sync(p, p->stream));
    return MI3PT_OK;
}

static int group_gather(mi3pt_ctx *g)
// ... 196 lines not shown
```

webgpu-pathtracer_amd/csrc/pt_internal.h:

```cpp
#pragma once
#include <string>

int pt_set_error(int code, const std::string &msg);

#include <hip/hip_runtime.h>
namespace pt {
int lbvh_build(const void *d_tris, size_t n, void *nodes_out, float *build_ms, hipStream_t stream, std::string &err);
}

#include <array>
#include <cstdint>
#include <cstring>
#include <vector>
#include "pt_kernels.h"
#include "../../include/mi3pt.h"
static inline float ldf(const uint8_t *p, size_t off) { float f; std::memcpy(&f, p + off, 4); return f; }
static inline int32_t ldi(const uint8_t *p, size_t off) { int32_t v; std::memcpy(&v, p + off, 4); return v; }
static inline uint32_t ldu(const uint8_t *p, size_t off) { uint32_t v; std::memcpy(&v, p + off, 4); return v; }
bool node_box_safe(const uint8_t *src, size_t node);
struct WideCollapse {
    int W = 4;
    std::vector<uint8_t> k0;
    std::vector<uint8_t> split;
    const uint8_t *src = nullptr;
    bool leaf(size_t i) const { return ldi(src + i * MI3PT_BVHNODE_STRIDE, 28) == 1; }
    int32_t left(size_t i) const { return ldi(src + i * MI3PT_BVHNODE_STRIDE, 32); }
    int32_t right(size_t i) const { return ldi(src + i * MI3PT_BVHNODE_STRIDE, 36); }
    void children_of(size_t x, std::vector<int32_t> &out) const
    {
        out.clear();
        std::vector<std::pair<int32_t, int>> work;
        work.emplace_back(right(x), W - (int)k0[x]);
        work.emplace_back(left(x), (int)k0[x]);
        while (!work.empty()) {
            auto [c, i] = work.back();
            work.pop_back();
            if (leaf((size_t)c) || i <= 1) { out.push_back(c); continue; }
            int k = 0;
            while (i >= 2 && (k = split[(size_t)c * (size_t)W + (size_t)i]) == 0) i--;
            if (i < 2) { out.push_back(c); continue; }
            work.emplace_back(right((size_t)c), i - k);
            work.emplace_back(left((size_t)c), k);
        }
    }
};
bool collapse_optimal(const uint8_t *src, size_t n, int W, const std::vector<uint8_t> *closed, WideCollapse &out);
struct Cw8Build {
    std::vector<pt::CW8Packet> packets;
    std::vector<pt::TriPacket64> records;
    int height = 0;
    double mean_children = 0.0;
};
bool build_cw8(const uint8_t *src, size_t n, const float *verts , size_t nt,
               const std::vector<float> &wmax, Cw8Build &out, bool greedy = false);
```

webgpu-pathtracer_amd/csrc/pt_kernels.h:

```cpp
#pragma once
#include <hip/hip_runtime.h>
#include <stdint.h>

namespace pt {

#ifndef PT_MAX_WAVES_PER_CU
#define PT_MAX_WAVES_PER_CU 24
#endif
constexpr int PT_MAX_RESIDENT_WAVES = 256 * PT_MAX_WAVES_PER_CU;

#ifndef PT_SM_LDS_DEPTH_VALUE
#define PT_SM_LDS_DEPTH_VALUE 24
#endif
constexpr int SM_LDS_DEPTH = PT_SM_LDS_DEPTH_VALUE;
#ifndef PT_SM_LDS_DEPTH_SIX_VALUE
#define PT_SM_LDS_DEPTH_SIX_VALUE 19
#endif
constexpr int SM_LDS_DEPTH_SIX = PT_SM_LDS_DEPTH_SIX_VALUE;
constexpr int SM_LDS_DEPTH_SIX_DEEP = 25;
constexpr int SM_OVERFLOW_ENTRIES = 64 - (SM_LDS_DEPTH_SIX < SM_LDS_DEPTH ? SM_LDS_DEPTH_SIX : SM_LDS_DEPTH);
static_assert(SM_LDS_DEPTH_SIX_DEEP >= SM_LDS_DEPTH_SIX && 4 * 6 * SM_LDS_DEPTH_SIX_DEEP * 256 < 160 * 1024, "six-wave deep build: LDS");
#ifndef PT_CULL_LEAF_CAP_VALUE
#define PT_CULL_LEAF_CAP_VALUE 8
#endif
// ... 100 lines not shown
    int32_t env_sampling;
    uint32_t ntris, nnodes, nmats, npackets;
    uint32_t root_ref;
    uint32_t flags;
    float cull_ka, cull_kb;
    int32_t env_w, env_h;
};

struct RtUniforms {
    float res_x, res_y, aspect;
    uint32_t frame;
    int32_t max_bounces, samples_per_frame;
    float cam_pos[3], cam_dir[3];
    float fov, focal_distance, aperture;
    float env_intensity, env_rotation;
};

struct AccUniforms {
    uint32_t res_w, res_h, frame, enabled;
};

struct FsUniforms {
    float res_x, res_y, aspect, scaling;
    uint32_t denoise, tonemapping;
};

struct Tile {
    int32_t tex_w, tex_h;
    int32_t local_rows;
    int32_t rank, nranks, block_rows;
};

#ifndef PT_DEFAULT_WALK_MIN
#define PT_DEFAULT_WALK_MIN 32
#endif
#ifndef PT_DEEP_WALK_MIN
#define PT_DEEP_WALK_MIN 44
#endif
#ifndef PT_DEFAULT_LEAF_MIN
#define PT_DEFAULT_LEAF_MIN 24
#endif
#ifndef PT_DEFAULT_SHADE_SPLIT
#define PT_DEFAULT_SHADE_SPLIT 64
#endif
#ifndef PT_DEFAULT_TAIL_POLICY
#define PT_DEFAULT_TAIL_POLICY 7
#endif
#ifndef PT_DEFAULT_JOB_CHUNK
#define PT_DEFAULT_JOB_CHUNK 4
#endif

struct RtService;

struct RtLaunch {
    SceneRefs scene;
    RtUniforms un;
    AccUniforms acc;
    Tile tile;
    float4 *radiance;
    size_t slot_pixels;
    int32_t nframes;
    float4 *accum;
    uint64_t *block_counters;
    uint32_t *tile_counter;
    int32_t job_group;
    int32_t tri_pair;
    int32_t job_reverse;
    int32_t job_chunk;
    uint32_t *stack_overflow;
    uint64_t *wave_times;
    int32_t diag_lite;
    int32_t store_f16;
    int32_t walk_min;
    int32_t leaf_min;
    int32_t tail_policy;
    int32_t shade_split;
    uint32_t *drain_flag;
    uint32_t drain_seq;
    int32_t top_packets;
    int32_t waves_per_cu;
    int32_t num_cus;
    uint32_t *tile_cost;
    const uint32_t *tile_perm;
    const float4 *cam_base;
    int32_t six_waves;
    float *park;
    RtService *service;
};
size_t service_block_bytes();

struct RtRoute { int kind, variant; bool lean; int blocks; int waves; bool ymax; int walk_min; };
RtRoute raytrace_route(const RtLaunch &L, int variant);
bool raytrace_variant_fuses(int variant);
void launch_raytrace_setup(const RtLaunch &L, bool fuse_accumulate, int variant, hipStream_t s);
void launch_raytrace(const RtLaunch &L, bool fuse_accumulate, int variant, hipStream_t s);
void launch_camera_base(const RtLaunch &L, float4 *out, hipStream_t s);
void launch_accumulate_batch(const AccUniforms &acc0, const Tile &tile, const float4 *slots, size_t slot_pixels,
                             int nframes, float4 *accum, int store_f16, hipStream_t s);
void launch_accumulate(const AccUniforms &acc, const Tile &tile, const float4 *input, float4 *accum,
                       int store_f16, hipStream_t s);
size_t fullscreen_taps_bytes();
void launch_fullscreen(const FsUniforms &fs, const float4 *tex, int tex_w, int tex_h, int canvas_w, int canvas_h,
                       void *taps, bool taps_current, float4 *out_f32, uint32_t *out_rgba8, hipStream_t s);
void launch_debug_intersect(const SceneRefs &scene, const float *rays, size_t n, float *out, int variant,
                            hipStream_t s);
void launch_debug_math(int fn, const float *a, const float *b, float *out, size_t n, hipStream_t s);
void launch_walk_stats(const uint64_t *counters, int nblocks, uint64_t *prev, uint64_t *out, uint64_t seq, hipStream_t s);
int raytrace_grid_blocks(const Tile &tile);
int raytrace_persistent_blocks(const Tile &tile, int nframes, int waves_per_cu, int num_cus, bool tuned = false, int waves_per_simd = 0);
void launch_pack_vertices(const float4 *tris, float4 *out, uint32_t ntris, hipStream_t s);
void launch_patch_cull(float4 *packets, const uint32_t *cull, uint32_t npackets, hipStream_t s);

}
```

webgpu-pathtracer_amd/csrc/pt_kernels.hip:

```cpp
#include "pt_kernels.h"
#include "pt_devmath.h"
#include <hip/hip_fp16.h>

namespace pt {

#define PT_SEED 123456789u
#define PT_TWOPI 6.28318530718f
#define PT_INVPI 0.31830988618f
#define PT_INVTWOPI 0.15915494309f
#define PT_INF 1e20f
#define PT_EPSILON 1e-6f
#define PT_MAX_STACK 64

#define PT_REF_LEAF pt::REF_LEAF
#define PT_REF_NONE pt::REF_NONE

struct f3 { float x, y, z; };

using ptm::div_pre;
using ptm::rcp_exact;

typedef float pt_keep4 __attribute__((ext_vector_type(4)));
template <bool WHOLE>
PT_DEV void keep16(float4 &v)
// ... 373 lines not shown
    if (VARIANT == 3) traverse_packets_pre(sc, o, d, stack, best, cnt);
    else if (VARIANT == 2) traverse_packets(sc, o, d, stack, best, cnt);
    else traverse_generic(sc, o, d, stack, best, cnt);
}

PT_DEV void finish_hit(const SceneRefs &sc, const f3 &o, const f3 &d, const Best &best,
                       f3 &position, f3 &normal, int32_t &material)
{
    const float4 q3 = sc.tris[(size_t)best.tri * 7 + 3];
    const float4 q4 = sc.tris[(size_t)best.tri * 7 + 4];
    const float4 q5 = sc.tris[(size_t)best.tri * 7 + 5];
    const float w = 1.0f - best.u - best.v;
    position = o + d * best.t;
    normal = normalize((xyz(q3) * w + xyz(q4) * best.u) + xyz(q5) * best.v);
    material = __float_as_int(q5.w);
}

PT_DEV float rand1(uint32_t &seed)
{
    seed = seed * 747796405u + 2891336453u;
    const uint32_t s = seed;
    uint32_t r = ((s >> ((s >> 28u) + 4u)) ^ s) * 277803737u;
    r = (r >> 22u) ^ r;
    return (float)r / 4294967296.0f;
}

PT_DEV float rand_normal(uint32_t &seed)
{
    const float theta = PT_TWOPI * rand1(seed);
    const float rho = ptm::sqrt_exact(-2.0f * ptm::log1_unit(rand1(seed)));
    return rho * ptm::cos1(theta);
}

PT_DEV f3 rand_direction(uint32_t &seed)
{
    const float x = rand_normal(seed);
    const float y = rand_normal(seed);
    const float z = rand_normal(seed);
    return normalize(F3(x, y, z));
}

PT_DEV void rand_point_in_circle(uint32_t &seed, float &px, float &py)
{
    const float theta = PT_TWOPI * rand1(seed);
    const float rho = ptm::sqrt_exact(rand1(seed));
    float s, c;
    ptm::sincos(theta, s, c);
    px = rho * c;
    py = rho * s;
}

PT_DEV void env_uv_from_dir(const f3 &dir, float sinr, float cosr, float &u, float &v)
{
    const f3 dr = F3(dir.x * cosr - dir.z * sinr, dir.y, dir.x * sinr + dir.z * cosr);
    const float phi = ptm::atan2_1(dr.x, dr.z);
    const float theta = ptm::asin1(clamp1(dr.y, -1.0f, 1.0f));
    u = phi * PT_INVTWOPI + 0.5f;
    v = -theta * PT_INVPI + 0.5f;
}

PT_DEV f3 sample_env(const float4 *env, int W, int H, float u, float v)
{
    const float x = u * (float)W - 0.5f;
    const float y = v * (float)H - 0.5f;
    const float x0f = floorf(x), y0f = floorf(y);
    const float fx = x - x0f, fy = y - y0f;
    float x0c = fminf(fmaxf(x0f, -1.0f), (float)W);
    float y0c = fminf(fmaxf(y0f, -1.0f), (float)H);
    if (x0c != x0c) x0c = 0.0f;
    if (y0c != y0c) y0c = 0.0f;
    const int x0 = (int)x0c, y0 = (int)y0c;
    const int xa = min(max(x0, 0), W - 1), xb = min(max(x0 + 1, 0), W - 1);
    const int ya = min(max(y0, 0), H - 1), yb = min(max(y0 + 1, 0), H - 1);
    const float4 p00 = env[(size_t)ya * W + xa];
    const float4 p10 = env[(size_t)ya * W + xb];
    const float4 p01 = env[(size_t)yb * W + xa];
    const float4 p11 = env[(size_t)yb * W + xb];
    const float wx0 = 1.0f - fx, wy0 = 1.0f - fy;
    f3 r;
    r.x = (p00.x * wx0 + p10.x * fx) * wy0 + (p01.x * wx0 + p11.x * fx) * fy;
    r.y = (p00.y * wx0 + p10.y * fx) * wy0 + (p01.y * wx0 + p11.y * fx) * fy;
    r.z = (p00.z * wx0 + p10.z * fx) * wy0 + (p01.z * wx0 + p11.z * fx) * fy;
    return r;
}

PT_DEV float4 cdf_texel(const float4 *cdf, int W, int H, float u, float v)
{
    float xf = floorf(u * (float)W), yf = floorf(v * (float)H);
    xf = fminf(fmaxf(xf, 0.0f), (float)(W - 1));
    yf = fminf(fmaxf(yf, 0.0f), (float)(H - 1));
    if (xf != xf) xf = 0.0f;
    if (yf != yf) yf = 0.0f;
    return cdf[(size_t)(int)yf * W + (int)xf];
}

PT_DEV void env_uv_sampled(const float4 *cdf, int W, int H, uint32_t &seed, float &u_out, float &v_out)
{
    const float r1 = rand1(seed);
    const float r2 = rand1(seed);
    float v_min = 0.0f, v_max = 1.0f;
    for (int i = 0; i < 8; i++) {
        const float v_mid = (v_min + v_max) / 2.0f;
        const float c = fmaxf(cdf_texel(cdf, W, H, 0.5f, v_mid).x, PT_EPSILON);
        if (c < r1) v_min = v_mid; else v_max = v_mid;
    }
    const float v = (v_min + v_max) / 2.0f;
    float u_min = 0.0f, u_max = 1.0f;
    for (int i = 0; i < 8; i++) {
        const float u_mid = (u_min + u_max) / 2.0f;
        const float c = fmaxf(cdf_texel(cdf, W, H, u_mid, v).y, PT_EPSILON);
        if (c < r2) u_min = u_mid; else u_max = u_mid;
    }
    u_out = (u_min + u_max) / 2.0f;
    v_out = v;
}

struct CameraFrame {
    float t, r;
    f3 w, u_dir, v_dir;
};

PT_DEV CameraFrame camera_frame(const RtUniforms &un)
{
    CameraFrame cf;
    const float rad = un.fov * 3.14159265358979323846f / 180.0f;
    cf.t = ptm::tan1(rad / 2.0f);
    cf.r = un.aspect * cf.t;
    cf.w = normalize(neg(F3(un.cam_dir[0], un.cam_dir[1], un.cam_dir[2])));
    f3 up = F3(0.0f, 1.0f, 0.0f);
    if (fabsf(dot(cf.w, up)) > 0.99999f) up = F3(0.0f, 0.0f, 1.0f);
    cf.u_dir = normalize(cross(up, cf.w));
    cf.v_dir = cross(cf.w, cf.u_dir);
    return cf;
}

PT_DEV f3 camera_direction(const CameraFrame &cf, float aspect, float uvx, float uvy)
{
    const float b = -cf.t;
    const float l = -cf.r;
    const float u = l + (cf.r - l) * uvx;
    const float v = b + (cf.t - b) * uvy;
    return normalize((cf.u_dir * u + cf.v_dir * v) - cf.w * aspect);
}

struct FastDiv { uint32_t m, sh; };
PT_DEV FastDiv fast_div_of(uint32_t d)
{
    FastDiv f;
    const uint32_t s = d <= 1u ? 0u : 32u - (uint32_t)__builtin_clz(d - 1u);
    f.sh = 31u + s;
    f.m = (uint32_t)((1ull << f.sh) / (d ? d : 1u)) + 1u;
    return f;
}
PT_DEV int fast_div(int t, const FastDiv &f) { return (int)(uint32_t)(((uint64_t)(uint32_t)t * f.m) >> f.sh); }

PT_DEV int local_to_global_row(int ly, const Tile &t)
{
    if (t.nranks == 1) return ly;
    if (t.block_rows == 8) {
        const int b = ly >> 3;
        return (((b * t.nranks + ((b & 1) ? t.nranks - 1 - t.rank : t.rank)) << 3) | (ly & 7));
    }
    const int b = ly / t.block_rows;
    return (b * t.nranks + ((b & 1) ? t.nranks - 1 - t.rank : t.rank)) * t.block_rows + (ly - b * t.block_rows);
}

// ... 290 lines not shown
            } else {
                cnt.miss++;
                float u, v;
                env_uv_from_dir(p.d, sinr, cosr, u, v);
                const f3 env = sample_env(sc.env, sc.env_w, sc.env_h, u, v);
                p.light = p.light + (p.ray_color * env) * un.env_intensity;
                ended = true;
            }
            if (ended) {
                p.incoming = p.incoming + p.light;
                p.sample++;
                next_path();
            }
        }
    }

    if (lane == 0) {
        const uint32_t left = atomicAdd(L.tile_counter + 1, 1u);
        if (left == gridDim.x - 1u) {
            __hip_atomic_store(L.tile_counter, 0u, __ATOMIC_RELAXED, __HIP_MEMORY_SCOPE_AGENT);
            __hip_atomic_store(L.tile_counter + 1, 0u, __ATOMIC_RELAXED, __HIP_MEMORY_SCOPE_AGENT);
        }
    }
    const uint32_t s_rays = wave_sum(cnt.rays), s_box = wave_sum(cnt.box), s_tri = wave_sum(cnt.tri);
    const uint32_t s_hit = wave_sum(cnt.hit), s_miss = wave_sum(cnt.miss);
    const uint32_t s_ovf = wave_sum(cnt.overflow), s_pix = wave_sum(cnt.pixels);
    if (lane == 0 && L.block_counters) {
        uint64_t *c = L.block_counters + (size_t)blockIdx.x * CNT_COUNT;
        c[CNT_RAYS] += s_rays; c[CNT_BOX] += s_box; c[CNT_TRI] += s_tri; c[CNT_HIT] += s_hit;
        c[CNT_MISS] += s_miss; c[CNT_OVERFLOW] += s_ovf; c[CNT_PIXELS] += s_pix;
    }
}

#endif

enum { M_DEAD = 0, M_TRAV = 1, M_SHADE = 2, M_PATH = 3 };

PT_DEV void cull_setup(const f3 &d, const RayPre &pre, float scene_ka, float scene_kb, float &ka, float &kb)
{
    const float dd = dot(d, d) * 1.0000005f;
    const bool ok = (pre.flags & 8u) == 0u && dd <= 4.0f;
    ka = ok ? scene_ka * dd : __builtin_inff();
    kb = ok ? scene_kb * fmaxf(1.0f, dd) : __builtin_inff();
}

struct RtService {
    RtLaunch L;
    CameraFrame cf;
    f3 cam_pos;
    float sinr, cosr;
    float root_mn[3], root_mx[3];
    float inv_res_x, inv_res_y, spf_f;
    uint32_t res_w, res_h;
    int32_t pinhole, res_ordinary;
    int32_t tiles_x, ntiles_frame, ntiles;
    int32_t grp_jobs, grp_full, grp_last;
    FastDiv dv_frame, dv_grp, dv_gs, dv_last, dv_tx, dv_w;
};
static_assert(sizeof(RtService) % 4 == 0, "loaded as dwords");
size_t service_block_bytes() { return sizeof(RtService); }

PT_DEV RtService compute_service(const RtLaunch &L, bool scene_has_nodes)
{
    RtService S;
    const RtUniforms &un = L.un;
    S.L = L;
    S.cf = camera_frame(un);
    S.cam_pos = F3(un.cam_pos[0], un.cam_pos[1], un.cam_pos[2]);
    ptm::sincos(un.env_rotation, S.sinr, S.cosr);
    float4 root0 = make_float4(0.0f, 0.0f, 0.0f, 0.0f), root1 = root0;
    if (scene_has_nodes) { root0 = L.scene.nodes[0]; root1 = L.scene.nodes[1]; }
    S.root_mn[0] = root0.x; S.root_mn[1] = root0.y; S.root_mn[2] = root0.z;
    S.root_mx[0] = root1.x; S.root_mx[1] = root1.y; S.root_mx[2] = root1.z;
    S.inv_res_x = 1.0f / un.res_x;
    S.inv_res_y = 1.0f / un.res_y;
    S.res_ordinary = (un.res_x >= 9.5367431640625e-07f && un.res_x <= 1.099511627776e12f &&
                      un.res_y >= 9.5367431640625e-07f && un.res_y <= 1.099511627776e12f) ? 1 : 0;
    S.spf_f = (float)un.samples_per_frame;
    S.res_w = (uint32_t)un.res_x;
    S.res_h = (uint32_t)un.res_y;
    S.pinhole = (un.aperture == 0.0f && __float_as_uint(un.cam_pos[0]) != 0x80000000u &&
                 __float_as_uint(un.cam_pos[1]) != 0x80000000u && __float_as_uint(un.cam_pos[2]) != 0x80000000u) ? 1 : 0;
    S.tiles_x = (L.tile.tex_w + 7) >> 3;
    S.ntiles_frame = S.tiles_x * ((L.tile.local_rows + 7) >> 3);
    S.ntiles = S.ntiles_frame * L.nframes;
    S.grp_jobs = (L.job_group > 0 && L.job_group < S.ntiles_frame) ? L.job_group * L.nframes : 0;
    S.grp_full = S.grp_jobs ? S.ntiles_frame / L.job_group : 0;
    S.grp_last = S.grp_jobs ? S.ntiles_frame - S.grp_full * L.job_group : 1;
    S.dv_frame = fast_div_of((uint32_t)S.ntiles_frame);
    S.dv_grp = fast_div_of((uint32_t)(S.grp_jobs ? S.grp_jobs : 1));
    S.dv_gs = fast_div_of((uint32_t)(L.job_group > 0 ? L.job_group : 1));
    S.dv_last = fast_div_of((uint32_t)(S.grp_last > 0 ? S.grp_last : 1));
    S.dv_tx = fast_div_of((uint32_t)S.tiles_x);
    S.dv_w = fast_div_of((uint32_t)(L.tile.tex_w > 0 ? L.tile.tex_w : 1));
    return S;
}

__global__ void __launch_bounds__(256) k_camera_base(const RtLaunch L, float4 *out)
{
    const int px = blockIdx.x * 64 + (threadIdx.x & 63);
    const int ly = blockIdx.y * 4 + (threadIdx.x >> 6);
    if (px >= L.tile.tex_w || ly >= L.tile.local_rows) return;
    const RtUniforms &un = L.un;
    const CameraFrame cf = camera_frame(un);
    const int pgy = local_to_global_row(ly, L.tile);
    const bool ordinary = un.res_x >= 9.5367431640625e-07f && un.res_x <= 1.099511627776e12f &&
                          un.res_y >= 9.5367431640625e-07f && un.res_y <= 1.099511627776e12f;
    float uvx, uvy;
    if (ordinary) { uvx = div_pre((float)px, un.res_x, 1.0f / un.res_x); uvy = div_pre((float)pgy, un.res_y, 1.0f / un.res_y); }
    else { uvx = (float)px / un.res_x; uvy = (float)pgy / un.res_y; }
    const f3 dir0 = camera_direction(cf, un.aspect, uvx, uvy);
    const f3 base = F3(un.cam_pos[0], un.cam_pos[1], un.cam_pos[2]) + dir0 * un.focal_distance;
    out[(size_t)ly * L.tile.tex_w + px] = make_float4(base.x, base.y, base.z, 0.0f);
}

void launch_camera_base(const RtLaunch &L, float4 *out, hipStream_t s)
{
    if (L.tile.tex_w <= 0 || L.tile.local_rows <= 0) return;
    hipLaunchKernelGGL(k_camera_base, dim3((L.tile.tex_w + 63) / 64, (L.tile.local_rows + 3) / 4), dim3(256), 0, s, L, out);
}

__global__ void __launch_bounds__(64) k_rt_service_setup(const RtLaunch L, RtService *out)
{
    const RtService S = compute_service(L, L.scene.nnodes != 0);
    if (threadIdx.x == 0) *out = S;
}

template <class T>
PT_DEV T load_const_block(const T *g)
{
    static_assert(sizeof(T) % 4 == 0 && __is_trivially_copyable(T), "dwords");
    uint32_t off = 0;
    asm volatile("" : "+s"(off));
    typedef const __attribute__((address_space(4))) uint32_t *cptr;
    const cptr p = (cptr)((uintptr_t)g + off);
    uint32_t w[sizeof(T) / 4];
#pragma unroll
    for (size_t i = 0; i < sizeof(T) / 4; i++) w[i] = p[i];
    T t;
    __builtin_memcpy(&t, w, sizeof(T));
    return t;
}
template <class T>
PT_DEV T uniform_block(const T &v)
{
    uint32_t w[sizeof(T) / 4];
    __builtin_memcpy(w, &v, sizeof(T));
#pragma unroll
    for (size_t i = 0; i < sizeof(T) / 4; i++) w[i] = (uint32_t)__builtin_amdgcn_readfirstlane((int)w[i]);
    T t;
    __builtin_memcpy(&t, w, sizeof(T));
    return t;
}

#ifndef PT_CW_NO_PAIR_TEST
#define PT_CW_NO_PAIR_TEST 0
#endif
#define PT_SM_LDS_DEPTH pt::SM_LDS_DEPTH
#ifndef PT_LONG_QUEUE
#define PT_LONG_QUEUE 16
#endif
#ifndef PT_DEEP_LEAF_MIN
#define PT_DEEP_LEAF_MIN 32
#endif
#ifndef PT_DEEP_LEAF_CAP
#define PT_DEEP_LEAF_CAP 10
#endif
// ... 640 lines not shown

        RtService *const service_block = L.service;
        RtService S;
        if constexpr (TUNED) S = load_const_block(service_block); else S = S0;
#define PT_SERVICE_PART() do { if constexpr (TUNED) S = load_const_block(service_block); } while (0)
        const RtLaunch &L = S.L;
        const SceneRefs &sc = L.scene;
        const RtUniforms &un = L.un;
        const CameraFrame &cf = S.cf;
        const f3 &cam_pos = S.cam_pos;
        const float &sinr = S.sinr, &cosr = S.cosr, &inv_res_x = S.inv_res_x, &inv_res_y = S.inv_res_y, &spf_f = S.spf_f;
        const uint32_t &res_w = S.res_w, &res_h = S.res_h;
        const int32_t &pinhole = S.pinhole, &res_ordinary_ = S.res_ordinary;
        const int &tiles_x = S.tiles_x, &ntiles_frame = S.ntiles_frame, &ntiles = S.ntiles;
        const int &grp_jobs = S.grp_jobs, &grp_full = S.grp_full, &grp_last = S.grp_last;
        const FastDiv &dv_frame = S.dv_frame, &dv_grp = S.dv_grp, &dv_gs = S.dv_gs, &dv_last = S.dv_last, &dv_tx = S.dv_tx;
        const unsigned long long m_hit = __ballot(mode == M_SHADE && best.tri >= 0);
        const int n_hit = (int)__popcll(m_hit);
        const int n_b = (int)__popcll(__ballot((mode == M_SHADE && best.tri < 0) || mode == M_PATH || (mode == M_DEAD && !feed_empty)));
        bool do_hit = n_hit > 0, do_b = true;
        if (k_shade_split > 0 && nwalk > 0 && n_hit > 0 && n_b > 0 && !(feed_empty && (k_tail_policy & 4))) {
            if (n_hit >= n_b) do_b = n_b >= k_shade_split;
            else do_hit = n_hit >= k_shade_split;
        }
        if (wave_times) {
            st_switch(2);
            if (feed_empty) st_tail_service++;
        }
        if (count_on) {
            st_service_steps++;
            if (do_hit) { st_hit_steps++; st_hit_lanes += (uint32_t)n_hit; }
            if (do_b) { st_b_steps++; st_shade_lanes += (uint32_t)__popcll(__ballot(mode == M_SHADE && best.tri < 0)); }
        }
        bool need_segment = false;
        {
            const bool shade_hit = do_hit && mode == M_SHADE && best.tri >= 0;
            const bool shade_miss = do_b && mode == M_SHADE && best.tri < 0;
            u_hit += (uint32_t)__popcll(__ballot(shade_hit));
            u_miss += (uint32_t)__popcll(__ballot(shade_miss));
            bool ended = true;
            if (shade_hit || shade_miss) {
                if constexpr (PARKG) {
                    ray_color = F3(parkg[0], parkg[64], parkg[128]);
                    light = F3(parkg[192], parkg[256], parkg[320]);
                } else {
                    ray_color = F3(park[0], park[64], park[128]);
                    light = F3(park[192], park[256], park[320]);
                }
            }
#ifdef PT_DIAG_SERVICE
            if (wave_times) st_switch(3);
#endif
            if (shade_hit) {
                
                float4 q3 = sc.tris[(size_t)best.tri * 7 + 3];
                float4 q4 = sc.tris[(size_t)best.tri * 7 + 4];
                float4 q5 = sc.tris[(size_t)best.tri * 7 + 5];
                const f3 rdir = rand_direction(seed);
                asm volatile("" : "+v"(q5.w));
                const int32_t mi = __float_as_int(q5.w);
                const float4 m0 = sc.mats[(size_t)mi * 4 + 0];
                const float4 m1 = sc.mats[(size_t)mi * 4 + 1];
                const float4 m2 = sc.mats[(size_t)mi * 4 + 2];
                const float4 m3 = sc.mats[(size_t)mi * 4 + 3];
                const float w = 1.0f - best.u - best.v;
                const f3 position = o + d * best.t;
                const f3 normal = normalize((xyz(q3) * w + xyz(q4) * best.u) + xyz(q5) * best.v);
                const f3 diffuse_dir = normalize(normal + rdir);
                const f3 specular_dir = reflect(d, normal);
                float is_specular = 0.0f;
                if (m2.x >= rand1(seed)) is_specular = 1.0f;
                o = position;
                d = mix(diffuse_dir, specular_dir, is_specular * (1.0f - m1.w));
                const f3 emitted = xyz(m3) * m3.w;
                light = light + emitted * ray_color;
                ray_color = ray_color * mix(xyz(m0), xyz(m1), is_specular);
                slot++;
                ended = (int32_t)(slot & 0xffffu) >= un.max_bounces;
            }
#ifdef PT_DIAG_SERVICE
            if (wave_times) st_switch(4);
#endif
            PT_SERVICE_PART();
            if (shade_miss) {
                
                float u, v;
                env_uv_from_dir(d, sinr, cosr, u, v);
                const f3 env = sample_env(sc.env, ENV_W, ENV_H, u, v);
                light = light + (ray_color * env) * un.env_intensity;
            }
            PT_SERVICE_PART();
            if (shade_hit || shade_miss) {
                mode = M_DEAD;
                if (ended) {
                    {
                        f3 pix = F3(0.0f, 0.0f, 0.0f) + light;
                        bool finished = true;
                        if (un.samples_per_frame != 1) {
                            float4 *const px = L.radiance + ((size_t)(slot >> 16) * L.slot_pixels + gx);
                            const float4 sum = *px;
                            pix = xyz(sum) + light;
                            const float taken = sum.w + 1.0f;
                            finished = taken >= spf_f;
                            if (finished) pix = F3(pix.x / spf_f, pix.y / spf_f, pix.z / spf_f);
                            else { *px = make_float4(pix.x, pix.y, pix.z, taken); mode = M_PATH; }
                        }
                        if (finished) write_radiance(L, gx, slot >> 16, pix);
                        if constexpr (DIAG) {
                            if (L.tile_cost) {
                                const int row = fast_div((int)gx, S.dv_w), col = (int)gx - row * L.tile.tex_w;
                                atomicAdd(L.tile_cost + ((row >> 3) * S.tiles_x + (col >> 3)), lane_cost + 10u * ((slot & 0xffffu) + 1u));
                            }
                            lane_cost = 0u;
                        }
                    }
                } else {
                    need_segment = true;
                }
            }
        }
#ifdef PT_DIAG_SERVICE
        if (wave_times) st_switch(5);
#endif
        PT_SERVICE_PART();
        uint32_t job_px = 0u, job_py = 0u;
        if (do_b) {
            unsigned long long dead = __ballot(mode == M_DEAD && !need_segment);
            while (dead != 0ull && !feed_empty) {
                if (cur_used >= 64) {
                    cur_tile = have_at;
                    if (cur_tile >= ntiles) {
                        feed_empty = true;
                        if (wave_times) {
                            t_empty_rt = __builtin_amdgcn_s_memrealtime();
                            st_live_at_empty = (uint32_t)__popcll(__ballot(mode != M_DEAD || need_segment));
                        }
                        break;
                    }
                    if (L.job_reverse) cur_tile = ntiles - 1 - cur_tile;
                    if (grp_jobs == 0) {
                        cur_fslot = fast_div(cur_tile, dv_frame);
                        cur_ftile = cur_tile - cur_fslot * ntiles_frame;
                    } else {
                        int g = fast_div(cur_tile, dv_grp), r = cur_tile - g * grp_jobs, gs = L.job_group;
                        const bool last = g >= grp_full;
                        if (last) { g = grp_full; r = cur_tile - grp_full * grp_jobs; gs = grp_last; }
                        cur_fslot = last ? fast_div(r, dv_last) : fast_div(r, dv_gs);
                        cur_ftile = g * L.job_group + (r - cur_fslot * gs);
                    }
                    if (L.tile_perm) cur_ftile = (int)L.tile_perm[cur_ftile];
                    have_at++;
                    if (--have == 0) draw(S);
                    cur_used = 0;
                }
                const int take = min((int)__popcll(dead), 64 - cur_used);
                const int rank = lane_rank(dead);
                const bool mine = ((dead >> lane) & 1ull) != 0ull && rank < take;
                bool got_job = false;
                if (mine) {
                    const int j = cur_used + rank;
                    const int fslot = cur_fslot, ftile = cur_ftile;
                    const int trow = fast_div(ftile, dv_tx);
                    const int px = (ftile - trow * tiles_x) * 8 + (j & 7);
                    const int ply = trow * 8 + (j >> 3);
                    const int pgy = local_to_global_row(ply, L.tile);
                    const bool ok = px < L.tile.tex_w && ply < L.tile.local_rows && pgy < L.tile.tex_h &&
                                    (uint32_t)px < res_w && (uint32_t)pgy < res_h;
                    if (ok) {
                        got_job = true;
                        seed = ((uint32_t)px + (uint32_t)pgy * res_w) + (un.frame + (uint32_t)fslot) * 719393u + PT_SEED;
                        job_px = (uint32_t)px; job_py = (uint32_t)pgy;
                        gx = (uint32_t)ply * (uint32_t)L.tile.tex_w + (uint32_t)px;
                        slot = (uint32_t)fslot << 16;
                        if (un.samples_per_frame != 1)
                            L.radiance[(size_t)fslot * L.slot_pixels + gx] = make_float4(0.0f, 0.0f, 0.0f, 0.0f);
                        mode = M_PATH;
                    }
                }
                cur_used += take;
                u_pix += (uint32_t)__popcll(__ballot(got_job));
                dead = __ballot(mode == M_DEAD && !need_segment && !mine);
            }
        }
        PT_SERVICE_PART();
        if (count_on) st_path_lanes += (uint32_t)__popcll(__ballot(do_b && mode == M_PATH));
        if (do_b && mode == M_PATH) {
            mode = M_DEAD;
            {
                float uvx, uvy;
                uint32_t pxx = job_px, pyy = job_py;
                {
                    if (un.samples_per_frame != 1) {
                        const int row = fast_div((int)gx, S.dv_w);
                        pxx = gx - (uint32_t)row * (uint32_t)L.tile.tex_w;
                        pyy = (uint32_t)local_to_global_row(row, L.tile);
                    }
                }
                f3 fbase;
                if (L.cam_base) {
                    const float4 cb = L.cam_base[gx];
                    fbase = xyz(cb);
                } else {
                    if (ASSUME || res_ordinary_ != 0) { uvx = div_pre((float)pxx, un.res_x, inv_res_x); uvy = div_pre((float)pyy, un.res_y, inv_res_y); }
                    else { uvx = (float)pxx / un.res_x; uvy = (float)pyy / un.res_y; }
                    const f3 dir0 = camera_direction(cf, un.aspect, uvx, uvy);
                    fbase = cam_pos + dir0 * un.focal_distance;
                }
                float jx, jy, kx, ky;
                rand_point_in_circle(seed, jx, jy);
                const f3 jitter = F3(jx * inv_res_x, jy * inv_res_y, 0.0f);
                const f3 focal = fbase + jitter;
                if (pinhole) {
                    (void)rand1(seed);
                    (void)rand1(seed);
                    o = cam_pos;
                } else {
                    rand_point_in_circle(seed, kx, ky);
                    const f3 jitter2 = F3(kx * un.aperture, ky * un.aperture, 0.0f);
                    o = cam_pos + jitter2;
                }
                d = normalize(focal - o);
                if (un.samples_per_frame < 1 || un.max_bounces < 1) {
                    const float z = un.samples_per_frame == 1 ? 0.0f : 0.0f / spf_f;
                    write_radiance(L, gx, slot >> 16, F3(z, z, z));
                } else {
                    need_segment = true;
                }
                slot &= 0xffff0000u;
                light = F3(0.0f, 0.0f, 0.0f);
                ray_color = F3(1.0f, 1.0f, 1.0f);
            }
        }
#ifdef PT_DIAG_SERVICE
        if (wave_times) st_switch(6);
#endif
        PT_SERVICE_PART();
        if (count_on) st_segment_lanes += (uint32_t)__popcll(__ballot(need_segment));
        {
            const uint32_t nseg = (uint32_t)__popcll(__ballot(need_segment));
            if (DIAG) u_rays += nseg;
            if (ASSUME || sc.nnodes != 0) u_box += nseg;
        }
        bool slow_segment = false;
        if (need_segment) {
            if constexpr (PARKG) {
                parkg[0] = ray_color.x; parkg[64] = ray_color.y; parkg[128] = ray_color.z;
                parkg[192] = light.x; parkg[256] = light.y; parkg[320] = light.z;
            } else {
                park[0] = ray_color.x; park[64] = ray_color.y; park[128] = ray_color.z;
                park[192] = light.x; park[256] = light.y; park[320] = light.z;
            }
        }
        ray_color = F3(0.0f, 0.0f, 0.0f);
        light = F3(0.0f, 0.0f, 0.0f);
        if (need_segment) {
            best.t = PT_INF; best.u = 0.0f; best.v = 0.0f; best.tri = -1;
            
            mode = M_SHADE;
            const bool nan_ray = CULL && (!(d.x == d.x) || !(d.y == d.y) || !(d.z == d.z) ||
                                          !(o.x == o.x) || !(o.y == o.y) || !(o.z == o.z));
            if ((ASSUME || sc.nnodes != 0) && !nan_ray) {
                pre = ray_prepare(o, d, sc.flags);
                slow_segment = (pre.flags & 8u) != 0u;
                if (CULL) cull_setup(d, pre, sc.cull_ka, sc.cull_kb, cull_ka, cull_kb);
                
                const bool skip_root = WIDE && (sc.flags & 2u) != 0u;
                if (skip_root || ray_aabb_pre(o, d, pre, !ASSUME && (sc.flags & 1u) == 0u, S.root_mn[0], S.root_mn[1], S.root_mn[2], S.root_mx[0], S.root_mx[1], S.root_mx[2])) {
                    if (!ASSUME && DEFER && (sc.root_ref & PT_REF_LEAF)) {
                        stack[(DEPTH - 1) * 64] = sc.root_ref & 0x7fffffffu;
                        sp = 0; nl = 1;
                    } else if constexpr (W8) {
                        pre.flags |= (pre.ix < 0.0f ? 0u : 16u) | (pre.iy < 0.0f ? 0u : 32u) | (pre.iz < 0.0f ? 0u : 64u);
                        stack[0] = 0u; stack[64] = 1u;
                        sp = 1; nl = 0;
                    } else {
                        st_store(0, WIDE ? sc.wide_root : sc.root_ref);
                        sp = 1; nl = 0;
                    }
                    mode = M_TRAV;
                }
            }
        }
        if (DIAG) u_slow += (uint32_t)__popcll(__ballot(slow_segment));
#undef PT_SERVICE_PART
    }

    if constexpr (LITE && !DIAG) {
        if (L.wave_times && lane == 0) {
            uint64_t *w = L.wave_times + (size_t)blockIdx.x * 16;
            w[8] = st_tri_steps;
            w[9] = 0; w[10] = 0; w[11] = 0;
            w[12] = ((uint64_t)st_hit_steps << 32) | st_b_steps;
            w[13] = 0; w[14] = 0; w[15] = 0;
            w[0] = t_begin_rt;
            w[1] = 0;
            w[2] = __builtin_amdgcn_s_memrealtime();
            w[3] = __builtin_amdgcn_s_memtime() - t_begin_clk;
            w[4] = ((uint64_t)st_walk_steps << 32) | st_walk_lanes;
            w[5] = ((uint64_t)st_service_steps << 32) | st_leaf_lanes;
            w[6] = ((uint64_t)st_shade_lanes << 32) | st_hit_lanes;
            w[7] = ((uint64_t)st_path_lanes << 32) | st_segment_lanes;
        }
    }
    if (wave_times && lane == 0) {
        uint64_t *w = wave_times + (size_t)blockIdx.x * 16;
        st_switch(2);
        w[8] = ((uint64_t)st_parked << 32) | st_tri_steps;
        w[9] = st_cyc_node; w[10] = st_cyc_tri; w[11] = st_cyc_service;
        w[12] = ((uint64_t)st_hit_steps << 32) | st_b_steps;
#ifdef PT_DIAG_SERVICE
        w[12] = st_cyc_part[0]; w[13] = st_cyc_part[1]; w[14] = st_cyc_part[2]; w[15] = st_cyc_part[3];
#else
        w[13] = ((uint64_t)st_tail_node << 32) | st_tail_tri;
        w[14] = ((uint64_t)st_tail_service << 32) | st_live_at_empty;
        w[15] = st_tail_lanes;
#endif
        w[0] = t_begin_rt;
        w[1] = t_empty_rt;
        w[2] = __builtin_amdgcn_s_memrealtime();
        w[3] = __builtin_amdgcn_s_memtime() - t_begin_clk;
        w[4] = ((uint64_t)st_walk_steps << 32) | st_walk_lanes;
        w[5] = ((uint64_t)st_service_steps << 32) | st_leaf_lanes;
        w[6] = ((uint64_t)st_shade_lanes << 32) | st_hit_lanes;
        w[7] = ((uint64_t)st_path_lanes << 32) | st_segment_lanes;
    }
    if (lane == 0) {
        const uint32_t left = atomicAdd(L.tile_counter + 1, 1u);
        if (left == gridDim.x - 1u) {
            __hip_atomic_store(L.tile_counter, 0u, __ATOMIC_RELAXED, __HIP_MEMORY_SCOPE_AGENT);
            __hip_atomic_store(L.tile_counter + 1, 0u, __ATOMIC_RELAXED, __HIP_MEMORY_SCOPE_AGENT);
        }
    }
    const uint32_t s_rays = DIAG ? u_rays : u_hit + u_miss, s_box = wave_sum(cnt.box) + u_box, s_tri = wave_sum(cnt.tri) + u_tri;
    const uint32_t s_hit = u_hit, s_miss = u_miss;
    const uint32_t s_ovf = wave_sum(cnt.overflow), s_pix = u_pix, s_slow = u_slow;
    if (lane == 0 && L.block_counters) {
        uint64_t *c = L.block_counters + (size_t)blockIdx.x * CNT_COUNT;
        c[CNT_RAYS] += s_rays; c[CNT_BOX] += s_box; c[CNT_TRI] += s_tri; c[CNT_HIT] += s_hit;
        c[CNT_MISS] += s_miss; c[CNT_OVERFLOW] += s_ovf; c[CNT_PIXELS] += s_pix;
        c[CNT_RESERVED] += s_slow;
    }
}

int raytrace_persistent_blocks(const Tile &tile, int nframes, int waves_per_cu, int num_cus, bool tuned, int waves_per_simd)
{
    const int ntiles = raytrace_grid_blocks(tile);
    if (num_cus <= 0) num_cus = 256;
    if (waves_per_simd <= 0) waves_per_simd = tuned ? SM_TUNED_WAVES_PER_SIMD : SM_OTHER_WAVES_PER_SIMD;
    if (waves_per_cu > 4 * waves_per_simd) waves_per_cu = 0;
    if (waves_per_cu <= 0 || waves_per_cu > PT_MAX_WAVES_PER_CU) {
        waves_per_cu = 4 * waves_per_simd;
        const long long jobs = (long long)ntiles * (nframes > 0 ? nframes : 1);
        const long long want = (jobs + (long long)num_cus * 8 - 1) / ((long long)num_cus * 8);
        if (want < 16) waves_per_cu = want < 4 ? 4 : (int)want;
        else if (want < 48 && waves_per_cu > 16) waves_per_cu = 16;
    }
    int resident = num_cus * waves_per_cu;
    if (resident > PT_MAX_RESIDENT_WAVES) resident = PT_MAX_RESIDENT_WAVES;
    const long long jobs = (long long)ntiles * (nframes > 0 ? nframes : 1);
    return jobs < (long long)resident ? (int)jobs : resident;
}

int raytrace_grid_blocks(const Tile &tile)
{
    const int tiles_x = (tile.tex_w + 7) / 8;
    const int tiles_y = (tile.local_rows + 7) / 8;
    return tiles_x * tiles_y;
}

static bool launch_packs(const RtLaunch &L)
{
    return L.un.max_bounces < 65536 && L.nframes <= 65535 && L.un.samples_per_frame <= 16777216;
}
static bool launch_is_lean(const RtLaunch &L)
{
    return (!L.wave_times || L.diag_lite) && !L.tile_cost && (L.walk_min == PT_DEFAULT_WALK_MIN || L.walk_min == PT_DEEP_WALK_MIN) && L.leaf_min == PT_DEFAULT_LEAF_MIN && L.shade_split == PT_DEFAULT_SHADE_SPLIT &&
           L.tail_policy == PT_DEFAULT_TAIL_POLICY && L.job_chunk == PT_DEFAULT_JOB_CHUNK && L.tri_pair == 1 && L.service != nullptr;
}
static bool launch_assumptions_hold(const RtLaunch &L)
{
    return L.scene.nnodes != 0 && (L.scene.flags & 1u) != 0u && (L.scene.root_ref & PT_REF_LEAF) == 0u &&
           L.un.res_x >= 9.5367431640625e-07f && L.un.res_x <= 1.099511627776e12f &&
           L.un.res_y >= 9.5367431640625e-07f && L.un.res_y <= 1.099511627776e12f;
}

static RtRoute route_launch(const RtLaunch &L, int variant)
{
    RtRoute r = { 0, variant <= 1 ? 1 : 2, false, 0 };
    if (variant < 3) return r;
#ifdef MI3PT_EXPERIMENTS
    if (variant == 3) { r.kind = 2; r.variant = 3; return r; }
#else
    if (variant == 3) variant = 4;
    if (variant == 5 || variant == 6) variant = 4;
    if (variant == 8) variant = 7;
#endif
    if (!launch_packs(L)) return r;
    r.kind = 1;
    r.lean = launch_is_lean(L);
    if (variant == 14 && !(L.scene.cw8 && L.scene.tripk8 && (L.scene.flags & 2u))) variant = 13;
    if (variant == 13 && !(L.scene.cwide && L.scene.tripk64)) variant = 10;
    if (L.walk_min == PT_DEEP_WALK_MIN && variant != 13 && variant != 14) r.lean = false;
#ifndef MI3PT_EXPERIMENTS
    if (variant == 11 || variant == 12) variant = 10;
#endif
    if (variant >= 9 && variant <= 14 && r.lean && !launch_assumptions_hold(L)) variant = L.scene.leaf_cap >= 4 ? 7 : 4;
    if (variant >= 10 && variant <= 14 && !r.lean) variant = 10;
#ifndef MI3PT_EXPERIMENTS
    if (variant < 9 && !r.lean) {
        if (!L.service) { r.kind = 0; r.variant = 2; return r; }
        r.lean = true;
    }
#endif
    r.variant = variant;
    return r;
}
bool raytrace_variant_fuses(int variant)
{
#ifdef MI3PT_EXPERIMENTS
    return variant <= 3;
#else
    return variant <= 2;
#endif
}
#ifndef PT_SIX_WAVES_MIN_JOBS
#define PT_SIX_WAVES_MIN_JOBS 1500000
#endif
static int route_waves_per_simd(const RtLaunch &L, const RtRoute &r)
{
    if (!(r.kind == 1 && r.lean)) return SM_OTHER_WAVES_PER_SIMD;
    if (r.variant == 13 || r.variant == 14) {
#ifdef MI3PT_EXPERIMENTS
        if (L.wave_times && L.diag_lite) return SM_TUNED_WAVES_PER_SIMD;
#endif
        if (L.six_waves >= 0) return L.six_waves ? SM_SIX_WAVES_PER_SIMD : SM_TUNED_WAVES_PER_SIMD;
        const long long jobs = (long long)raytrace_grid_blocks(L.tile) * (L.nframes > 0 ? L.nframes : 1);
        return jobs >= (L.walk_min == PT_DEEP_WALK_MIN ? PT_SIX_WAVES_MIN_JOBS / 10 : PT_SIX_WAVES_MIN_JOBS) ? SM_SIX_WAVES_PER_SIMD : SM_TUNED_WAVES_PER_SIMD;
    }
    return SM_TUNED_WAVES_PER_SIMD;
}
static int persistent_blocks_for(const RtLaunch &L, const RtRoute &r)
{
    return raytrace_persistent_blocks(L.tile, L.nframes, L.waves_per_cu, L.num_cus, r.kind == 1 && r.lean, route_waves_per_simd(L, r));
}
RtRoute raytrace_route(const RtLaunch &L, int variant)
{
    RtRoute r = route_launch(L, variant);
    r.blocks = r.kind == 1 ? persistent_blocks_for(L, r) : raytrace_grid_blocks(L.tile);
    r.waves = r.kind == 1 ? route_waves_per_simd(L, r) : 0;
    r.ymax = r.kind == 1 && r.lean && r.variant >= 12 && (L.scene.flags & 4u) != 0u;
    r.walk_min = r.kind == 1 ? (r.lean ? ((r.variant == 13 || r.variant == 14) && L.walk_min == PT_DEEP_WALK_MIN ? PT_DEEP_WALK_MIN : PT_DEFAULT_WALK_MIN) : L.walk_min) : 0;
    return r;
}

void launch_raytrace_setup(const RtLaunch &L, bool fuse, int variant, hipStream_t s)
{
    (void)fuse;
    const RtRoute r = route_launch(L, variant);
    if (raytrace_grid_blocks(L.tile) > 0 && r.kind == 1 && r.lean)
        hipLaunchKernelGGL(k_rt_service_setup, dim3(1), dim3(64), 0, s, L, L.service);
}

void launch_raytrace(const RtLaunch &L, bool fuse, int variant, hipStream_t s)
{
    const int blocks = raytrace_grid_blocks(L.tile);
    if (blocks <= 0) return;
    const dim3 block(64);
    const RtRoute r = route_launch(L, variant);
    if (r.kind == 1) {
        const dim3 grid(persistent_blocks_for(L, r));
#define PT_SM(...) hipLaunchKernelGGL((k_raytrace_sm<__VA_ARGS__>), grid, block, 0, s, L)
#ifdef MI3PT_EXPERIMENTS
        if (r.lean && L.wave_times && L.diag_lite && r.variant >= 10) switch (r.variant) {
            case 14: if (L.scene.flags & 4u) PT_SM(true, true, true, true, true, false, false, true, true, PT_DEFAULT_WALK_MIN, SM_TUNED_WAVES_PER_SIMD, true);
                     else PT_SM(true, true, true, true, false, false, false, true, true, PT_DEFAULT_WALK_MIN, SM_TUNED_WAVES_PER_SIMD, true); break;
            case 13: if (L.scene.flags & 4u) PT_SM(true, true, true, true, true, false, false, true, true); else PT_SM(true, true, true, true, false, false, false, true, true); break;
            case 12: PT_SM(true,  true,  true,  true,  true,  false, false, true); break;
            case 11: PT_SM(true,  true,  true,  true,  false, false, false, true); break;
            default: PT_SM(true,  true,  true,  false, false, false, false, true); break;
        } else
#endif
#ifndef PT_X_TOP_CW
#define PT_TOP_CW false
#else
#define PT_TOP_CW true
#endif
        if (r.lean && r.variant == 14) {
            const bool six = route_waves_per_simd(L, r) == SM_SIX_WAVES_PER_SIMD, ymax = (L.scene.flags & 4u) != 0u;
            if (L.walk_min == PT_DEEP_WALK_MIN) {
                if (six) { if (ymax) PT_SM(true, true, true, true, true, false, false, false, true, PT_DEEP_WALK_MIN, SM_SIX_WAVES_PER_SIMD, true); else PT_SM(true, true, true, true, false, false, false, false, true, PT_DEEP_WALK_MIN, SM_SIX_WAVES_PER_SIMD, true); }
                else { if (ymax) PT_SM(true, true, true, true, true, false, false, false, true, PT_DEEP_WALK_MIN, SM_TUNED_WAVES_PER_SIMD, true); else PT_SM(true, true, true, true, false, false, false, false, true, PT_DEEP_WALK_MIN, SM_TUNED_WAVES_PER_SIMD, true); }
            } else {
                if (six) { if (ymax) PT_SM(true, true, true, true, true, false, false, false, true, PT_DEFAULT_WALK_MIN, SM_SIX_WAVES_PER_SIMD, true); else PT_SM(true, true, true, true, false, false, false, false, true, PT_DEFAULT_WALK_MIN, SM_SIX_WAVES_PER_SIMD, true); }
                else { if (ymax) PT_SM(true, true, true, true, true, false, false, false, true, PT_DEFAULT_WALK_MIN, SM_TUNED_WAVES_PER_SIMD, true); else PT_SM(true, true, true, true, false, false, false, false, true, PT_DEFAULT_WALK_MIN, SM_TUNED_WAVES_PER_SIMD, true); }
            }
        } else
        if (r.lean && r.variant == 13) {
            const bool six = route_waves_per_simd(L, r) == SM_SIX_WAVES_PER_SIMD, ymax = (L.scene.flags & 4u) != 0u;
            if (L.walk_min == PT_DEEP_WALK_MIN) {
                if (six) { if (ymax) PT_SM(true, true, true, true, true, false, PT_TOP_CW, false, true, PT_DEEP_WALK_MIN, SM_SIX_WAVES_PER_SIMD); else PT_SM(true, true, true, true, false, false, PT_TOP_CW, false, true, PT_DEEP_WALK_MIN, SM_SIX_WAVES_PER_SIMD); }
                else { if (ymax) PT_SM(true, true, true, true, true, false, PT_TOP_CW, false, true, PT_DEEP_WALK_MIN); else PT_SM(true, true, true, true, false, false, PT_TOP_CW, false, true, PT_DEEP_WALK_MIN); }
            } else {
                if (six) { if (ymax) PT_SM(true, true, true, true, true, false, PT_TOP_CW, false, true, PT_DEFAULT_WALK_MIN, SM_SIX_WAVES_PER_SIMD); else PT_SM(true, true, true, true, false, false, PT_TOP_CW, false, true, PT_DEFAULT_WALK_MIN, SM_SIX_WAVES_PER_SIMD); }
                else { if (ymax) PT_SM(true, true, true, true, true, false, PT_TOP_CW, false, true); else PT_SM(true, true, true, true, false, false, PT_TOP_CW, false, true); }
            }
        } else
        if (r.lean) switch (r.variant) {
#ifdef MI3PT_EXPERIMENTS
            case 12: PT_SM(true,  true,  true,  true,  true,  false); break;
            case 11: PT_SM(true,  true,  true,  true,  false, false); break;
#endif
            case 10: PT_SM(true,  true,  true,  false, false, false); break;
            case 9:  PT_SM(true,  true,  false, false, false, false); break;
            case 7:  PT_SM(true,  false, false, false, false, false); break;
            default: PT_SM(false, false, false, false, false, false); break;
        } else switch (r.variant) {
            case 10: PT_SM(true,  true,  true,  false, false, true); break;
            case 9:  PT_SM(true,  true,  false, false, false, true); break;
#ifdef MI3PT_EXPERIMENTS
            case 8:  PT_SM(true,  false, false, false, false, true, true); break;
            case 7:  PT_SM(true,  false, false, false, false, true); break;
            case 6:  PT_SM(false, false, false, false, false, true, true); break;
            default: PT_SM(false, false, false, false, false, true); break;
#else
            default: break;
#endif
// ... 383 lines not shown
    }
    f3 c = F3(c4.x, c4.y, c4.z);
    if (fs.tonemapping == 1u) c = aces_tonemap(c);
    else if (fs.tonemapping == 2u) c = F3(c.x / (c.x + 1.0f), c.y / (c.y + 1.0f), c.z / (c.z + 1.0f));
    const size_t i = (size_t)py * canvas_w + px;
    if (out_f32) out_f32[i] = make_float4(c.x, c.y, c.z, 1.0f);
    if (out_rgba8) out_rgba8[i] = to_unorm8(c.x) | (to_unorm8(c.y) << 8) | (to_unorm8(c.z) << 16) | 0xff000000u;
}

void launch_fullscreen(const FsUniforms &fs, const float4 *tex, int tex_w, int tex_h, int canvas_w,
                       int canvas_h, void *taps, bool taps_current, float4 *out_f32, uint32_t *out_rgba8, hipStream_t s)
{
    if (canvas_w <= 0 || canvas_h <= 0) return;
    if (fs.denoise == 1u && !taps_current)
        hipLaunchKernelGGL(k_fullscreen_setup, dim3(1), dim3(64), 0, s, fs, static_cast<DenoiseTaps *>(taps));
    const dim3 grid((canvas_w + 15) / 16, (canvas_h + 15) / 16), block(256);
    hipLaunchKernelGGL(k_fullscreen, grid, block, 0, s, fs, tex, tex_w, tex_h, canvas_w, canvas_h,
                       static_cast<const DenoiseTaps *>(taps), out_f32, out_rgba8);
}

template <int VARIANT>
__global__ void __launch_bounds__(64) k_debug_intersect(const SceneRefs sc, const float *__restrict__ rays,
                                                        size_t n, float *__restrict__ out)
{
    __shared__ uint32_t stack_lds[PT_MAX_STACK * 64];
    const size_t i = (size_t)blockIdx.x * 64 + threadIdx.x;
    if (i >= n) return;
    const f3 o = F3(rays[i * 6 + 0], rays[i * 6 + 1], rays[i * 6 + 2]);
    const f3 d = F3(rays[i * 6 + 3], rays[i * 6 + 4], rays[i * 6 + 5]);
    Counters cnt = { 0, 0, 0, 0, 0, 0, 0, 0 };
    Best best;
    traverse<VARIANT>(sc, o, d, stack_lds + threadIdx.x, best, cnt);
    float *r = out + i * 12;
    f3 position = F3(0.0f, 0.0f, 0.0f), normal = F3(0.0f, 0.0f, 0.0f);
    int32_t mi = -1;
    if (best.tri >= 0) finish_hit(sc, o, d, best, position, normal, mi);
    r[0] = best.tri >= 0 ? 1.0f : 0.0f;
    r[1] = best.t;
    r[2] = position.x; r[3] = position.y; r[4] = position.z;
    r[5] = normal.x; r[6] = normal.y; r[7] = normal.z;
    r[8] = (float)mi;
    r[9] = (float)cnt.box; r[10] = (float)cnt.tri; r[11] = (float)cnt.overflow;
}

void launch_debug_intersect(const SceneRefs &scene, const float *rays, size_t n, float *out, int variant,
                            hipStream_t s)
{
    if (n == 0) return;
    const dim3 grid((unsigned)((n + 63) / 64)), block(64);
    if (variant >= 3) hipLaunchKernelGGL(k_debug_intersect<3>, grid, block, 0, s, scene, rays, n, out);
    else if (variant == 2) hipLaunchKernelGGL(k_debug_intersect<2>, grid, block, 0, s, scene, rays, n, out);
    else hipLaunchKernelGGL(k_debug_intersect<1>, grid, block, 0, s, scene, rays, n, out);
}

__global__ void __launch_bounds__(256) k_debug_math(int fn, const float *__restrict__ a,
                                                    const float *__restrict__ b, float *__restrict__ out, size_t n)
{
    const size_t i = (size_t)blockIdx.x * 256 + threadIdx.x;
    if (i >= n) return;
    const float x = a[i], y = b ? b[i] : 0.0f;
    float r;
    switch (fn) {
    case 0: r = ptm::sin1(x); break;
    case 1: r = ptm::cos1(x); break;
    case 2: r = ptm::tan1(x); break;
    case 3: r = ptm::log1(x); break;
    case 4: r = ptm::exp1(x); break;
    case 5: r = ptm::atan2_1(x, y); break;
    case 6: r = ptm::asin1(x); break;
    case 7: r = ptm::pow1(x, y); break;
    case 8: r = ptm::round_f16(x); break;
    case 9: r = sqrtf(x); break;
    case 11: r = ptm::sqrt_exact(x); break;
    case 12: r = ptm::rcp_exact(x); break;
    case 13: r = normalize(F3(x, y, x - y)).x; break;
    case 14: r = normalize(F3(x, y, x - y)).y; break;
    case 15: r = normalize(F3(x, y, x - y)).z; break;
    case 16: r = ptm::log1_unit(x); break;
    default: r = x / y; break;
    }
    out[i] = r;
}

__global__ void __launch_bounds__(256) k_walk_stats(const uint64_t *__restrict__ counters, int nblocks, uint64_t *prev, uint64_t *out, uint64_t seq)
{
    __shared__ uint64_t sb[256], sr[256];
    uint64_t b = 0, r = 0;
    for (int i = (int)threadIdx.x; i < nblocks; i += 256) {
        b += counters[(size_t)i * CNT_COUNT + CNT_BOX];
        r += counters[(size_t)i * CNT_COUNT + CNT_RAYS];
    }
    sb[threadIdx.x] = b; sr[threadIdx.x] = r;
    __syncthreads();
    for (int s = 128; s > 0; s >>= 1) {
        if ((int)threadIdx.x < s) { sb[threadIdx.x] += sb[threadIdx.x + s]; sr[threadIdx.x] += sr[threadIdx.x + s]; }
        __syncthreads();
    }
    if (threadIdx.x == 0) {
        const uint64_t tb = sb[0], tr = sr[0], pb = prev[0], pr = prev[1];
        const bool restarted = tb < pb || tr < pr;
        prev[0] = tb; prev[1] = tr;
        __hip_atomic_store(out + 1, restarted ? tb : tb - pb, __ATOMIC_RELAXED, __HIP_MEMORY_SCOPE_SYSTEM);
        __hip_atomic_store(out + 2, restarted ? tr : tr - pr, __ATOMIC_RELAXED, __HIP_MEMORY_SCOPE_SYSTEM);
        __hip_atomic_store(out + 0, seq, __ATOMIC_RELEASE, __HIP_MEMORY_SCOPE_SYSTEM);
    }
}

void launch_walk_stats(const uint64_t *counters, int nblocks, uint64_t *prev, uint64_t *out, uint64_t seq, hipStream_t s)
{
    if (nblocks <= 0 || !counters || !prev || !out) return;
    hipLaunchKernelGGL(k_walk_stats, dim3(1), dim3(256), 0, s, counters, nblocks, prev, out, seq);
}

__global__ void __launch_bounds__(256) k_patch_cull(float4 *__restrict__ packets, const uint32_t *__restrict__ cull, uint32_t n)
{
    const uint32_t i = blockIdx.x * 256u + threadIdx.x;
    if (i < n) packets[(size_t)i * 4 + 3].w = __uint_as_float(cull[i]);
}

void launch_patch_cull(float4 *packets, const uint32_t *cull, uint32_t npackets, hipStream_t s)
{
    if (npackets == 0) return;
    hipLaunchKernelGGL(k_patch_cull, dim3((npackets + 255u) / 256u), dim3(256), 0, s, packets, cull, npackets);
}

__global__ void __launch_bounds__(256) k_pack_vertices(const float4 *__restrict__ tris, float4 *__restrict__ out, uint32_t n)
{
    const uint32_t i = blockIdx.x * 256u + threadIdx.x;
    if (i >= n) return;
#pragma unroll
    for (int k = 0; k < 3; k++) out[(size_t)i * 3 + k] = tris[(size_t)i * 7 + k];
}

void launch_pack_vertices(const float4 *tris, float4 *out, uint32_t ntris, hipStream_t s)
{
    if (ntris == 0) return;
    hipLaunchKernelGGL(k_pack_vertices, dim3((ntris + 255u) / 256u), dim3(256), 0, s, tris, out, ntris);
}

void launch_debug_math(int fn, const float *a, const float *b, float *out, size_t n, hipStream_t s)
{
    if (n == 0) return;
    hipLaunchKernelGGL(k_debug_math, dim3((unsigned)((n + 255) / 256)), dim3(256), 0, s, fn, a, b, out, n);
}

}
```

webgpu-pathtracer_amd/py/mi3pt_host/capi.py:

```python
import ctypes
import os

import numpy as np

PKG_ROOT = os.path.dirname(os.path.dirname(os.path.dirname(os.path.abspath(__file__))))
LIB_PATH = os.environ.get("MI3PT_LIBRARY") or os.path.join(PKG_ROOT, "libmi3pt.so")

PASS_RAYTRACE, PASS_ACCUMULATE, PASS_FULLSCREEN = 0, 1, 2
SUBMIT_RAYTRACE, SUBMIT_ACCUMULATE, SUBMIT_FULLSCREEN = 1, 2, 4
TEX_OUTPUT, TEX_ACCUMULATION, TEX_CANVAS = 0, 1, 2
STORAGE_F32, STORAGE_F16 = 0, 1
PRESENT_EXACT, PRESENT_LATEST = 0, 1
(OPT_WALK_MIN, OPT_LEAF_MIN, OPT_SHADE_SPLIT, OPT_TAIL_POLICY, OPT_TOP_PACKETS, OPT_TRI_PAIR, OPT_JOB_REVERSE, OPT_JOB_GROUP,
 OPT_JOB_CHUNK, OPT_BATCH_LIMIT, OPT_BATCH, OPT_WAVES_PER_CU, OPT_CULL, OPT_WIDE, OPT_GATE, OPT_SLOT_SETS, OPT_PIPELINE,
 OPT_COST_ORDER, OPT_PRESENT_DEPTH, OPT_HOST_ANALYSES, OPT_GATHER_STAGED, OPT_DIAG_LITE,
 OPT_GATE_TIMEOUT_MS, OPT_GATE_RELEASES, OPT_DEBUG_SUPPRESS_DRAIN, OPT_CAMERA_BASE, OPT_PACKET_ORDER, OPT_SIX_WAVES, OPT_COLLAPSE, OPT_LAST_BUILD, OPT_WALK_ADAPT) = range(31)
COUNTER_NAMES = ("rays", "box_tests", "tri_tests", "hits", "misses", "stack_overflows", "pixels", "reserved")

SYMBOLS = (
    "mi3pt_abi_version", "mi3pt_last_error", "mi3pt_device_count", "mi3pt_device_name",
    "mi3pt_create", "mi3pt_destroy", "mi3pt_set_stream", "mi3pt_set_storage", "mi3pt_set_tile",
    "mi3pt_tile_local_rows", "mi3pt_upload_triangles", "mi3pt_upload_materials", "mi3pt_upload_bvh",
    "mi3pt_upload_environment", "mi3pt_upload_environment_cdf", "mi3pt_resize", "mi3pt_reset",
    "mi3pt_set_uniforms", "mi3pt_submit", "mi3pt_sync", "mi3pt_read_texture", "mi3pt_read_canvas_rgba8",
    "mi3pt_write_texture",
    "mi3pt_accumulation_device_ptr", "mi3pt_bind_accumulation", "mi3pt_enable_timing",
    "mi3pt_pass_time_us", "mi3pt_raytrace_launch_stats", "mi3pt_get_counters", "mi3pt_reset_counters", "mi3pt_set_kernel_variant",
    "mi3pt_set_env_sampling", "mi3pt_device_build_bvh",
    "mi3pt_set_pipelining", "mi3pt_flush", "mi3pt_set_present_mode", "mi3pt_raytrace_launch_span", "mi3pt_batch_capacity", "mi3pt_debug_active_variant", "mi3pt_debug_last_launch", "mi3pt_submit_frames", "mi3pt_debug_set_packet_layout",
    "mi3pt_debug_intersect", "mi3pt_debug_math", "mi3pt_debug_wave_times", "mi3pt_host_build_bvh", "mi3pt_host_build_bvh_f64",
    "mi3pt_host_env_cdf", "mi3pt_host_eight_wide_check", "mi3pt_debug_set_option", "mi3pt_debug_get_option",
    "mi3pt_create_group", "mi3pt_group_size", "mi3pt_group_member",
    "mi3pt_tile_global_row", "mi3pt_tile_owner",
)


class Mi3ptError(RuntimeError):
    def __init__(self, code, message):
        super().__init__(f"mi3pt error {code}: {message}")
        self.code = code
        self.message = message


_lib = None


def load_library(path=None):
    global _lib
    if _lib is not None and path is None:
        return _lib
    path = path or LIB_PATH
    if not os.path.exists(path):
        raise Mi3ptError(-1, f"{path} not found: build it with `make -C webgpu-pathtracer_amd/csrc` "
                             "(or __graft_entry__.build())")
    lib = ctypes.CDLL(path)
    c_void_p, c_size_t, c_int = ctypes.c_void_p, ctypes.c_size_t, ctypes.c_int
    lib.mi3pt_last_error.restype = ctypes.c_char_p
    lib.mi3pt_create.argtypes = [c_int, ctypes.POINTER(c_void_p)]
    lib.mi3pt_destroy.argtypes = [c_void_p]
    lib.mi3pt_set_stream.argtypes = [c_void_p, c_void_p]
    lib.mi3pt_set_storage.argtypes = [c_void_p, c_int]
    lib.mi3pt_set_tile.argtypes = [c_void_p, c_int, c_int, c_int]
    lib.mi3pt_set_kernel_variant.argtypes = [c_void_p, c_int]
    lib.mi3pt_set_env_sampling.argtypes = [c_void_p, c_int]
    lib.mi3pt_set_pipelining.argtypes = [c_void_p, c_int]
    lib.mi3pt_set_present_mode.argtypes = [c_void_p, c_int]
    for name in ("mi3pt_upload_triangles", "mi3pt_upload_materials", "mi3pt_upload_bvh"):
        getattr(lib, name).argtypes = [c_void_p, c_void_p, c_size_t]
    for name in ("mi3pt_upload_environment", "mi3pt_upload_environment_cdf"):
        getattr(lib, name).argtypes = [c_void_p, c_void_p, c_int, c_int]
    lib.mi3pt_resize.argtypes = [c_void_p, c_int, c_int]
    lib.mi3pt_reset.argtypes = [c_void_p]
    lib.mi3pt_set_uniforms.argtypes = [c_void_p, c_int, c_void_p, c_size_t]
    lib.mi3pt_submit.argtypes = [c_void_p, ctypes.c_uint]
    lib.mi3pt_submit_frames.argtypes = [c_void_p, ctypes.c_uint, ctypes.c_uint32]
    lib.mi3pt_sync.argtypes = [c_void_p]
    lib.mi3pt_flush.argtypes = [c_void_p]
    lib.mi3pt_read_texture.argtypes = [c_void_p, c_int, c_void_p, c_size_t]
    lib.mi3pt_read_canvas_rgba8.argtypes = [c_void_p, c_void_p, c_size_t]
    lib.mi3pt_write_texture.argtypes = [c_void_p, c_int, c_void_p, c_size_t]
    lib.mi3pt_accumulation_device_ptr.argtypes = [c_void_p, ctypes.POINTER(c_void_p), ctypes.POINTER(c_size_t)]
    lib.mi3pt_bind_accumulation.argtypes = [c_void_p, c_void_p, c_size_t]
    lib.mi3pt_enable_timing.argtypes = [c_void_p, c_int]
    lib.mi3pt_pass_time_us.argtypes = [c_void_p, c_int, ctypes.POINTER(ctypes.c_float)]
    lib.mi3pt_raytrace_launch_stats.argtypes = [c_void_p, c_int, ctypes.POINTER(ctypes.c_double),
                                                ctypes.POINTER(ctypes.c_uint64), ctypes.POINTER(ctypes.c_uint64)]
    lib.mi3pt_raytrace_launch_span.argtypes = [c_void_p, ctypes.POINTER(ctypes.c_double)]
    lib.mi3pt_batch_capacity.argtypes = [c_void_p, ctypes.POINTER(c_int)]
    lib.mi3pt_debug_active_variant.argtypes = [c_void_p, ctypes.POINTER(c_int)]
    lib.mi3pt_debug_last_launch.argtypes = [c_void_p, ctypes.POINTER(c_int), ctypes.POINTER(c_int), ctypes.POINTER(c_int), ctypes.POINTER(c_int)]
    lib.mi3pt_create_group.argtypes = [ctypes.POINTER(c_int), c_int, c_int, ctypes.POINTER(c_void_p)]
    lib.mi3pt_group_size.argtypes = [c_void_p, ctypes.POINTER(c_int)]
    lib.mi3pt_group_member.argtypes = [c_void_p, c_int, ctypes.POINTER(c_void_p)]
    lib.mi3pt_debug_set_option.argtypes = [c_void_p, c_int, c_int]
    lib.mi3pt_debug_get_option.argtypes = [c_void_p, c_int, ctypes.POINTER(c_int)]
    lib.mi3pt_debug_set_packet_layout.argtypes = [c_void_p, c_int]
    lib.mi3pt_get_counters.argtypes = [c_void_p, c_void_p]
    lib.mi3pt_reset_counters.argtypes = [c_void_p]
    lib.mi3pt_debug_intersect.argtypes = [c_void_p, c_void_p, c_size_t, c_void_p]
    lib.mi3pt_debug_math.argtypes = [c_void_p, c_int, c_void_p, c_void_p, c_void_p, c_size_t]
    lib.mi3pt_device_build_bvh.argtypes = [c_void_p, c_void_p, c_size_t, c_void_p, c_void_p]
    lib.mi3pt_debug_wave_times.argtypes = [c_void_p, c_int, c_void_p, c_size_t, ctypes.POINTER(c_size_t)]
    lib.mi3pt_host_build_bvh.argtypes = [c_void_p, c_size_t, c_void_p, c_size_t, ctypes.POINTER(c_size_t), c_int]
    lib.mi3pt_host_build_bvh_f64.argtypes = [c_void_p, c_size_t, c_void_p, c_size_t, ctypes.POINTER(c_size_t), c_int]
    lib.mi3pt_host_env_cdf.argtypes = [c_void_p, c_int, c_int, c_void_p]
    lib.mi3pt_host_eight_wide_check.argtypes = [c_void_p, c_size_t, c_void_p, c_size_t, c_int, c_void_p]
    lib.mi3pt_device_count.argtypes = [ctypes.POINTER(c_int)]
    lib.mi3pt_device_name.argtypes = [c_int, ctypes.c_char_p, c_size_t]
    lib.mi3pt_tile_local_rows.argtypes = [c_int, c_int, c_int, c_int]
    lib.mi3pt_tile_global_row.argtypes = [c_int, c_int, c_int, c_int]
    lib.mi3pt_tile_owner.argtypes = [c_int, c_int, c_int]
    if path == LIB_PATH:
        _lib = lib
    return lib


def _check(lib, rc):
    if rc != 0:
        raise Mi3ptError(rc, lib.mi3pt_last_error().decode("utf-8", "replace"))


def _ptr(arr):
    return arr.ctypes.data_as(ctypes.c_void_p)


def device_count():
    lib = load_library()
    n = ctypes.c_int(0)
    _check(lib, lib.mi3pt_device_count(ctypes.byref(n)))
    return n.value


def device_name(device=0):
    lib = load_library()
    buf = ctypes.create_string_buffer(256)
    _check(lib, lib.mi3pt_device_name(device, buf, 256))
    return buf.value.decode()


def last_error():
    return load_library().mi3pt_last_error().decode(errors="replace")


def tile_local_rows(height, rank, nranks, block_rows):
    return load_library().mi3pt_tile_local_rows(height, rank, nranks, block_rows)


def tile_global_row(local_row, rank, nranks, block_rows):
    return load_library().mi3pt_tile_global_row(local_row, rank, nranks, block_rows)


def tile_owner(y, nranks, block_rows):
    return load_library().mi3pt_tile_owner(y, nranks, block_rows)



def host_build_bvh(triangles, nthreads=0):
    from . import layout
    lib = load_library()
    tri = np.ascontiguousarray(triangles)
    n = tri.nbytes // 112
    nodes = np.zeros(max(2 * n - 1, 1), layout.BVH_NODE)
    count = ctypes.c_size_t(0)
    _check(lib, lib.mi3pt_host_build_bvh(_ptr(tri), n, _ptr(nodes), nodes.nbytes, ctypes.byref(count), nthreads))
    return nodes[:count.value]


def host_build_bvh_f64(positions, nthreads=0):
    from . import layout
    lib = load_library()
    pos = np.ascontiguousarray(positions, np.float64)
    n = pos.size // 9
    nodes = np.zeros(max(2 * n - 1, 1), layout.BVH_NODE)
    count = ctypes.c_size_t(0)
    _check(lib, lib.mi3pt_host_build_bvh_f64(_ptr(pos), n, _ptr(nodes), nodes.nbytes, ctypes.byref(count), nthreads))
    return nodes[:count.value]


def host_eight_wide_check(nodes, triangles, greedy=False):
    lib = load_library()
    nd, tr = np.ascontiguousarray(nodes), np.ascontiguousarray(triangles)
    out = np.zeros(6, np.uint64)
    _check(lib, lib.mi3pt_host_eight_wide_check(_ptr(nd), nd.nbytes, _ptr(tr), tr.nbytes, 1 if greedy else 0, _ptr(out)))
    return {"packets": int(out[0]), "records": int(out[1]), "levels": int(out[2]), "children_per_packet": out[3] / 1000.0,
            "leaves": int(out[4]), "offered": bool(out[5])}


def host_env_cdf(rgba):
    lib = load_library()
    env = np.ascontiguousarray(rgba, np.float32)
    h, w = env.shape[0], env.shape[1]
    out = np.empty((h, w, 4), np.float32)
    _check(lib, lib.mi3pt_host_env_cdf(_ptr(env), w, h, _ptr(out)))
    return out


class Context:

    def __init__(self, device=0, devices=None, block_rows=8):
        self.lib = load_library()
        handle = ctypes.c_void_p()
        self.group_size = 1
        self._group_block_rows = block_rows
        if devices is not None:
            arr = (ctypes.c_int * len(devices))(*devices)
            _check(self.lib, self.lib.mi3pt_create_group(arr, len(devices), block_rows, ctypes.byref(handle)))
            self.group_size = len(devices)
        else:
            _check(self.lib, self.lib.mi3pt_create(device, ctypes.byref(handle)))
        self.handle = handle
        self.width = self.height = 0
        self.local_rows = 0
        self._tile = (0, 1, 8)
        self._next_tile = (0, 1, 8)

    def close(self):
        if self.handle and not getattr(self, "_borrowed", False):
            self.lib.mi3pt_destroy(self.handle)
        self.handle = None

    def member(self, index):
        h = ctypes.c_void_p()
        self._c(self.lib.mi3pt_group_member(self.handle, index, ctypes.byref(h)))
        m = Context.__new__(Context)
        m.lib, m.handle, m._borrowed, m.group_size = self.lib, h, True, 1
        m.width, m.height = self.width, self.height
        n = self.group_size
        m._group_block_rows = 8
        m._tile = m._next_tile = (0, 1, 8) if index < 0 or n == 1 else (index, n, self._group_block_rows)
        m.local_rows = tile_local_rows(self.height, *m._tile) if self.height else 0
        return m

    def __enter__(self):
        return self

    def __exit__(self, *exc):
        self.close()

    def __del__(self):
        try:
            self.close()
        except Exception:
            pass

    def _c(self, rc):
        _check(self.lib, rc)

    def set_stream(self, stream_ptr):
        self._c(self.lib.mi3pt_set_stream(self.handle, stream_ptr))

    def set_storage(self, storage):
        self._c(self.lib.mi3pt_set_storage(self.handle, storage))

    def set_kernel_variant(self, variant):
        self._c(self.lib.mi3pt_set_kernel_variant(self.handle, variant))

    def set_env_sampling(self, enabled):
        self._c(self.lib.mi3pt_set_env_sampling(self.handle, int(bool(enabled))))

# ... 168 lines not shown
```

Measured before the change: 17760 Mrays/s.

## Classify sky-only 8x8 tiles on host and shade them with a cheap miss kernel

Measured after the change: 19490 Mrays/s (median of 6 runs). 9.7% higher.

```diff
diff --git a/include/mi3pt.h b/include/mi3pt.h
--- a/include/mi3pt.h
+++ b/include/mi3pt.h
@@ -153,6 +153,7 @@
     MI3PT_OPT_HOST_ANALYSES = 19,
     MI3PT_OPT_DIAG_LITE = 21,
     MI3PT_OPT_GATHER_STAGED = 20,
+    MI3PT_OPT_SKY_TILES = 31,
     MI3PT_OPT_COST_ORDER = 17
 } mi3pt_option;
 int mi3pt_debug_set_option(mi3pt_ctx *ctx, int option , int value);
@@ -177,6 +178,8 @@
                              size_t nodes_capacity_bytes, size_t *nnodes_out, int nthreads);
 int mi3pt_host_env_cdf(const float *rgba, int width, int height, float *cdf_rgba_out);
 int mi3pt_host_eight_wide_check(const void *nodes, size_t nodes_bytes, const void *triangles, size_t triangles_bytes, int greedy, uint64_t out[6]);
+int mi3pt_host_sky_tiles(const void *nodes, size_t nodes_bytes, const void *raytrace_uniforms, int width, int height,
+                         int rank, int nranks, int block_rows, uint8_t *empty_out, size_t capacity, size_t *ntiles_out);
 
 #ifdef __cplusplus
 }
diff --git a/webgpu-pathtracer_amd/csrc/pt_context.hip b/webgpu-pathtracer_amd/csrc/pt_context.hip
--- a/webgpu-pathtracer_amd/csrc/pt_context.hip
+++ b/webgpu-pathtracer_amd/csrc/pt_context.hip
@@ -104,6 +104,24 @@
     uint8_t cam_base_key[2][80] = {};
     bool cam_base_valid[2] = { false, false };
     bool cam_base_enabled = true;
+#ifndef PT_SKY_TILES_DEFAULT
+#define PT_SKY_TILES_DEFAULT 1
+#endif
+    int sky_tiles = PT_SKY_TILES_DEFAULT;
+    std::vector<float> sky_cut;
+    bool sky_cut_ok = false;
+    uint8_t sky_key[104] = {}, sky_seen_key[104] = {};
+    bool sky_host_valid = false;
+    std::vector<uint32_t> sky_host;
+    int sky_host_active = 0;
+    uint64_t sky_host_pixels = 0;
+    uint32_t *d_sky_list[2] = { nullptr, nullptr };
+    size_t sky_list_cap[2] = { 0, 0 };
+    uint8_t sky_dev_key[2][104] = {};
+    bool sky_dev_valid[2] = { false, false };
+    std::vector<uint32_t> sky_staged[2];
+    hipEvent_t sky_copied[2] = {};
+    bool sky_copied_valid[2] = { false, false };
     int collapse = -1;
     int six_waves = -1;
     int packet_order = 0;
@@ -111,7 +129,10 @@
     bool output_is_accum = false;
     uint64_t *d_block_counters = nullptr;
     uint32_t *d_tile_counter = nullptr;
-    int job_reverse = 1;
+#ifndef PT_JOB_REVERSE_DEFAULT
+#define PT_JOB_REVERSE_DEFAULT 1
+#endif
+    int job_reverse = PT_JOB_REVERSE_DEFAULT;
     int job_group = -1;
     int tri_pair = 1;
     int job_chunk = PT_DEFAULT_JOB_CHUNK;
@@ -415,6 +436,7 @@
             CREATE_TRY(hipStreamCreateWithFlags(&ctx->rt_stream[k], hipStreamNonBlocking));
         }
         CREATE_TRY(hipEventCreateWithFlags(&ctx->rt_done[k], hipEventDisableTiming));
+        CREATE_TRY(hipEventCreateWithFlags(&ctx->sky_copied[k], hipEventDisableTiming));
     }
     for (int k = 0; k < 3; k++) CREATE_TRY(hipEventCreateWithFlags(&ctx->acc_done[k], hipEventDisableTiming));
     CREATE_TRY(hipEventCreateWithFlags(&ctx->main_mark, hipEventDisableTiming));
@@ -528,6 +550,9 @@
     for (int k = 0; k < 2; k++) {
         if (ctx->rt_stream[k]) (void)hipStreamDestroy(ctx->rt_stream[k]);
         if (ctx->rt_done[k]) (void)hipEventDestroy(ctx->rt_done[k]);
+        if (ctx->sky_copied[k]) (void)hipEventDestroy(ctx->sky_copied[k]);
+        if (ctx->d_sky_list[k]) (void)hipFree(ctx->d_sky_list[k]);
+        ctx->d_sky_list[k] = nullptr;
     }
     for (int k = 0; k < 3; k++)
         if (ctx->acc_done[k]) (void)hipEventDestroy(ctx->acc_done[k]);
@@ -639,6 +664,10 @@
     case MI3PT_OPT_WIDE: ctx->wide_enabled = value != 0; break;
     case MI3PT_OPT_GATE: ctx->gate_enabled = value != 0 && ctx->d_drain_flag != nullptr; if (ctx->gate_enabled) { ctx->gate_releases = 0; ctx->gate_stalls_in_a_row = 0; } break;
     case MI3PT_OPT_CAMERA_BASE: ctx->cam_base_enabled = value != 0; break;
+    case MI3PT_OPT_SKY_TILES:
+        if (value < 0 || value > 2) return pt_set_error(MI3PT_ERR_INVALID, "MI3PT_OPT_SKY_TILES: 0, 1 or 2");
+        ctx->sky_tiles = value;
+        break;
     case MI3PT_OPT_SIX_WAVES: ctx->six_waves = value < 0 ? -1 : (value != 0 ? 1 : 0); break;
     case MI3PT_OPT_WALK_ADAPT: ctx->walk_adapt = value != 0; if (!ctx->walk_adapt) ctx->deep_by_view = false; break;
     case MI3PT_OPT_COLLAPSE:
@@ -705,6 +734,7 @@
     case MI3PT_OPT_WIDE: *value = ctx->wide_enabled ? 1 : 0; break;
     case MI3PT_OPT_GATE: *value = ctx->gate_enabled ? 1 : 0; break;
     case MI3PT_OPT_CAMERA_BASE: *value = ctx->cam_base_enabled ? 1 : 0; break;
+    case MI3PT_OPT_SKY_TILES: *value = ctx->sky_tiles; break;
     case MI3PT_OPT_SIX_WAVES: *value = ctx->six_waves; break;
     case MI3PT_OPT_COLLAPSE: *value = ctx->collapse; break;
     case MI3PT_OPT_WALK_ADAPT: *value = ctx->walk_adapt; break;
@@ -987,6 +1017,8 @@
     ctx->root_ref = ref_of(0);
     ctx->scene_flags = node_box_safe(src, 0) ? 1u : 0u;
     ctx->max_tri_ref = max_tri;
+    ctx->sky_cut_ok = tree_proper && pt::sky_cut_of(src, n, ctx->sky_cut);
+    ctx->sky_host_valid = false;
     ctx->cull_dirty = true;
     ctx->cost_state = 0;
     ctx->layout_active = false;
@@ -1806,6 +1838,7 @@
     L.num_cus = ctx->num_cus;
     L.service = nullptr;
     L.cam_base = nullptr;
+    L.ntiles_active = 0;
     L.park = ctx->d_park;
     L.six_waves = ctx->six_waves;
     L.tile_cost = nullptr;
@@ -1974,6 +2007,83 @@
     else if (per_ray <= WALK_ADAPT_LEAVE) ctx->deep_by_view = false;
 }
 
+#define SKY_MIN_FRAMES 8
+static int sky_prepare(mi3pt_ctx *ctx, pt::RtLaunch &L, const uint8_t *u_rt, int par, int n, hipStream_t rs,
+                       const uint32_t **sky_list, int *sky_count, uint64_t *sky_samples)
+{
+    *sky_list = nullptr; *sky_count = 0; *sky_samples = 0;
+    const pt::RtRoute &r = ctx->last_route;
+    if (!ctx->sky_tiles || !ctx->sky_cut_ok || ctx->env_sampling || !L.cam_base || L.tile_perm || L.tile_cost ||
+        !(r.kind == 1 && r.lean && r.variant >= 9 && r.variant <= 14))
+        return MI3PT_OK;
+    const int ntiles = pt::raytrace_grid_blocks(L.tile);
+    if (ntiles < 2) return MI3PT_OK;
+    uint8_t key[104];
+    std::memset(key, 0, sizeof key);
+    std::memcpy(key, u_rt, 12);
+    std::memcpy(key + 12, u_rt + 32, 40);
+    std::memcpy(key + 52, u_rt + 16, 8);
+    const int32_t tl[6] = { L.tile.tex_w, L.tile.tex_h, L.tile.local_rows, L.tile.rank, L.tile.nranks, L.tile.block_rows };
+    std::memcpy(key + 60, tl, sizeof tl);
+    std::memcpy(key + 88, &ctx->scene_epoch, 8);
+    if (!ctx->sky_host_valid || std::memcmp(key, ctx->sky_key, sizeof key) != 0) {
+        const bool stood_still = std::memcmp(key, ctx->sky_seen_key, sizeof key) == 0;
+        std::memcpy(ctx->sky_seen_key, key, sizeof key);
+        if (n < SKY_MIN_FRAMES && !stood_still) return MI3PT_OK;
+        std::vector<uint8_t> empty;
+        (void)pt::sky_classify(ctx->sky_cut, true, u_rt, L.tile.tex_w, L.tile.local_rows, L.tile.tex_h,
+                               L.tile.rank, L.tile.nranks, L.tile.block_rows, empty);
+        ctx->sky_host.assign((size_t)ntiles, 0u);
+        size_t at = 0;
+        for (int t = 0; t < ntiles; t++) if (!empty[(size_t)t]) ctx->sky_host[at++] = (uint32_t)t;
+        ctx->sky_host_active = (int)at;
+        const double rx = ldf(u_rt, 0), ry = ldf(u_rt, 4);
+        const long long res_w = rx >= 1.0 ? (long long)std::min(rx, 4294967295.0) : 0, res_h = ry >= 1.0 ? (long long)std::min(ry, 4294967295.0) : 0;
+        const int tiles_x = (L.tile.tex_w + 7) / 8;
+        uint64_t pixels = 0;
+        for (int t = 0; t < ntiles; t++) {
+            if (!empty[(size_t)t]) continue;
+            ctx->sky_host[at++] = (uint32_t)t;
+            const int trow = t / tiles_x, tcol = t - trow * tiles_x;
+            int cols = 0;
+            for (int px = tcol * 8; px < tcol * 8 + 8; px++) cols += px < L.tile.tex_w && (long long)px < res_w ? 1 : 0;
+            for (int ply = trow * 8; ply < trow * 8 + 8; ply++) {
+                if (ply >= L.tile.local_rows) continue;
+                const int pgy = L.tile.nranks <= 1 ? ply : mi3pt_tile_global_row(ply, L.tile.rank, L.tile.nranks, L.tile.block_rows);
+                if (pgy >= 0 && pgy < L.tile.tex_h && (long long)pgy < res_h) pixels += (uint64_t)cols;
+            }
+        }
+        ctx->sky_host_pixels = pixels;
+        std::memcpy(ctx->sky_key, key, sizeof key);
+        ctx->sky_host_valid = true;
+    }
+    const int active = ctx->sky_host_active, nempty = ntiles - active;
+    if (nempty <= 0 || active <= 0) return MI3PT_OK;
+    if (!ctx->sky_dev_valid[par] || std::memcmp(key, ctx->sky_dev_key[par], sizeof key) != 0) {
+        if (ctx->sky_copied_valid[par]) HIP_TRY(hipEventSynchronize(ctx->sky_copied[par]));
+        if (ctx->sky_list_cap[par] < (size_t)ntiles) {
+            uint32_t *fresh = nullptr;
+            if (hipMalloc((void **)&fresh, (size_t)ntiles * 4) != hipSuccess) { (void)hipGetLastError(); return MI3PT_OK; }
+            if (ctx->d_sky_list[par]) (void)hipFree(ctx->d_sky_list[par]);
+            ctx->d_sky_list[par] = fresh;
+            ctx->sky_list_cap[par] = (size_t)ntiles;
+        }
+        ctx->sky_dev_valid[par] = false;
+        ctx->sky_staged[par] = ctx->sky_host;
+        HIP_TRY(hipMemcpyAsync(ctx->d_sky_list[par], ctx->sky_staged[par].data(), (size_t)ntiles * 4, hipMemcpyHostToDevice, rs));
+        HIP_TRY(hipEventRecord(ctx->sky_copied[par], rs));
+        ctx->sky_copied_valid[par] = true;
+        std::memcpy(ctx->sky_dev_key[par], key, sizeof key);
+        ctx->sky_dev_valid[par] = true;
+    }
+    L.tile_perm = ctx->d_sky_list[par];
+    L.ntiles_active = active;
+    *sky_list = ctx->d_sky_list[par] + active;
+    *sky_count = nempty;
+    *sky_samples = ctx->sky_host_pixels * (uint64_t)n;
+    return MI3PT_OK;
+}
+
 static int launch_batch(mi3pt_ctx *ctx, const mi3pt_ctx::PendingFrame *frames, int n)
 {
     adapt_walk(ctx);
@@ -1999,9 +2109,6 @@
     if (ctx->acc_done_valid[set]) HIP_TRY(hipStreamWaitEvent(rs, ctx->acc_done[set], 0));
     L.radiance = ctx->d_slots[set];
     L.nframes = n;
-    if (ctx->deep_by_view && ctx->walk_min == 0 && L.walk_min == PT_DEFAULT_WALK_MIN && pick_variant(ctx) == 13 &&
-        (long long)pt::raytrace_grid_blocks(L.tile) * n >= 250000)
-        L.walk_min = PT_DEEP_WALK_MIN;
     L.block_counters = ctx->d_block_counters + (size_t)par * ctx->nblocks * pt::CNT_COUNT;
     L.tile_counter = ctx->d_tile_counter + par * 32;
     L.stack_overflow = ctx->d_stack_overflow + (size_t)par * pt::PT_MAX_RESIDENT_WAVES * pt::SM_OVERFLOW_ENTRIES * 64;
@@ -2051,12 +2158,23 @@
             L.cam_base = ctx->d_cam_base[par];
         }
     }
+    const uint32_t *sky_list = nullptr;
+    int sky_count = 0;
+    uint64_t sky_samples = 0;
+    if (launches)
+        if (int rc = sky_prepare(ctx, L, first.u_rt, par, n, rs, &sky_list, &sky_count, &sky_samples)) return rc;
+    if (ctx->deep_by_view && ctx->walk_min == 0 && L.walk_min == PT_DEFAULT_WALK_MIN && pick_variant(ctx) == 13 &&
+        (long long)pt::raytrace_grid_blocks(L.tile) * n >= 250000)
+        L.walk_min = PT_DEEP_WALK_MIN;
+    ctx->last_route = pt::raytrace_route(L, pick_variant(ctx));
     pt::launch_raytrace_setup(L, false, pick_variant(ctx), rs);
     if (ctx->timing) {
         HIP_TRY(hipEventRecord(ctx->ev_rt[par][0], rs));
         if (!ctx->span_started) { HIP_TRY(hipEventRecord(ctx->ev_span_start, rs)); ctx->span_started = true; }
     }
+    if (sky_count && ctx->sky_tiles != 2) pt::launch_sky_samples(L, sky_list, sky_count, sky_samples, rs);
     pt::launch_raytrace(L, false, pick_variant(ctx), rs);
+    if (sky_count && ctx->sky_tiles == 2) pt::launch_sky_samples(L, sky_list, sky_count, sky_samples, rs);
     if (publish_after && !ctx->debug_suppress_drain && hipStreamWriteValue32(rs, ctx->d_drain_flag, publish_after, 0) != hipSuccess) {
         (void)hipGetLastError();
         ctx->gate_enabled = false;
@@ -2077,12 +2195,12 @@
         ctx->ev_rt_frames[par] = n;
         ctx->ev_rt_newest = par;
     }
-    HIP_TRY(hipEventRecord(ctx->rt_done[par], rs));
-    HIP_TRY(hipStreamWaitEvent(ctx->stream, ctx->rt_done[par], 0));
     if (ctx->walk_adapt && ctx->h_walk_stats && launches && ctx->last_route.kind == 1 && ctx->last_route.lean && ctx->last_route.variant == 13 && ctx->walk_min == 0) {
         pt::launch_walk_stats(L.block_counters, ctx->nblocks, ctx->d_walk_prev + 2 * par, ctx->d_walk_stats + 4 * par, ++ctx->walk_stats_seq, rs);
         (void)hipGetLastError();
     }
+    HIP_TRY(hipEventRecord(ctx->rt_done[par], rs));
+    HIP_TRY(hipStreamWaitEvent(ctx->stream, ctx->rt_done[par], 0));
     ctx->last_radiance = L.radiance + (size_t)(n - 1) * L.slot_pixels;
     ctx->output_is_accum = true;
     for (int k = 0; k < n;) {
@@ -2758,6 +2876,7 @@
     dst->wide_leaf_cap = src->wide_leaf_cap; dst->wide_root = src->wide_root;
     dst->layout = src->layout; dst->layout_dirty = src->layout_dirty; dst->layout_active = src->layout_active;
     dst->cost_state = 0;
+    dst->sky_cut = src->sky_cut; dst->sky_cut_ok = src->sky_cut_ok; dst->sky_host_valid = false;
     dst->main_dirty = true;
     dst->scene_epoch++;
     return MI3PT_OK;
diff --git a/webgpu-pathtracer_amd/csrc/pt_host_sky.cpp b/webgpu-pathtracer_amd/csrc/pt_host_sky.cpp
--- /dev/null
+++ b/webgpu-pathtracer_amd/csrc/pt_host_sky.cpp
@@ -0,0 +1,186 @@
+#include "../../include/mi3pt.h"
+#include "pt_internal.h"
+
+#include <algorithm>
+#include <climits>
+#include <cmath>
+#include <queue>
+
+namespace pt {
+
+static bool finite3(const double *v) { return std::isfinite(v[0]) && std::isfinite(v[1]) && std::isfinite(v[2]); }
+
+static void node_box(const uint8_t *src, size_t i, double *mn, double *mx)
+{
+    const uint8_t *r = src + i * MI3PT_BVHNODE_STRIDE;
+    for (int k = 0; k < 3; k++) { mn[k] = (double)ldf(r, 4 * (size_t)k); mx[k] = (double)ldf(r, 16 + 4 * (size_t)k); }
+}
+
+bool sky_cut_of(const uint8_t *src, size_t n, std::vector<float> &boxes)
+{
+    boxes.clear();
+    if (!src || n == 0) return false;
+    auto is_leaf = [&](size_t i) { return ldi(src + i * MI3PT_BVHNODE_STRIDE, 28) == 1; };
+    for (size_t i = 0; i < n; i++) {
+        double mn[3], mx[3];
+        node_box(src, i, mn, mx);
+        if (!finite3(mn) || !finite3(mx) || mn[0] > mx[0] || mn[1] > mx[1] || mn[2] > mx[2]) return false;
+        if (is_leaf(i)) continue;
+        for (size_t off : { (size_t)32, (size_t)36 }) {
+            const int32_t c = ldi(src + i * MI3PT_BVHNODE_STRIDE, off);
+            if (c < 0) continue;
+            if ((size_t)c >= n || (size_t)c <= i) return false;
+            double cmn[3], cmx[3];
+            node_box(src, (size_t)c, cmn, cmx);
+            for (int k = 0; k < 3; k++)
+                if (!(cmn[k] >= mn[k] && cmx[k] <= mx[k])) return false;
+        }
+    }
+    constexpr size_t SKY_CUT_NODES = 48;
+    auto area = [&](size_t i) {
+        double mn[3], mx[3];
+        node_box(src, i, mn, mx);
+        const double ex = mx[0] - mn[0], ey = mx[1] - mn[1], ez = mx[2] - mn[2];
+        return ex * ey + ey * ez + ez * ex;
+    };
+    std::priority_queue<std::pair<double, size_t>> open;
+    std::vector<size_t> cut;
+    if (is_leaf(0)) cut.push_back(0); else open.emplace(area(0), 0);
+    while (!open.empty() && cut.size() + open.size() < SKY_CUT_NODES) {
+        const size_t i = open.top().second;
+        open.pop();
+        for (size_t off : { (size_t)32, (size_t)36 }) {
+            const int32_t c = ldi(src + i * MI3PT_BVHNODE_STRIDE, off);
+            if (c < 0) continue;
+            if (is_leaf((size_t)c)) cut.push_back((size_t)c); else open.emplace(area((size_t)c), (size_t)c);
+        }
+    }
+    for (; !open.empty(); open.pop()) cut.push_back(open.top().second);
+    for (size_t i : cut) {
+        const uint8_t *r = src + i * MI3PT_BVHNODE_STRIDE;
+        for (size_t off : { (size_t)0, (size_t)4, (size_t)8, (size_t)16, (size_t)20, (size_t)24 }) boxes.push_back(ldf(r, off));
+    }
+    return true;
+}
+
+static int global_row(int ly, int rank, int nranks, int block_rows)
+{
+    return nranks <= 1 ? ly : mi3pt_tile_global_row(ly, rank, nranks, block_rows);
+}
+
+size_t sky_classify(const std::vector<float> &boxes, bool have_cut, const uint8_t *u, int width, int local_rows, int height,
+                    int rank, int nranks, int block_rows, std::vector<uint8_t> &empty)
+{
+    const int tiles_x = (width + 7) / 8, tiles_y = (local_rows + 7) / 8;
+    empty.assign((size_t)tiles_x * (size_t)(tiles_y > 0 ? tiles_y : 0), 0);
+    if (!have_cut || empty.empty()) return 0;
+    const double res_x = ldf(u, 0), res_y = ldf(u, 4), aspect = ldf(u, 8);
+    const int32_t max_bounces = ldi(u, 16), spf = ldi(u, 20);
+    const double fov = ldf(u, 60), F = ldf(u, 64);
+    const float aperture = ldf(u, 68);
+    double o[3], cd[3];
+    for (int k = 0; k < 3; k++) {
+        if (ldu(u, 32 + 4 * (size_t)k) == 0x80000000u) return 0;
+        o[k] = ldf(u, 32 + 4 * (size_t)k);
+        cd[k] = ldf(u, 48 + 4 * (size_t)k);
+    }
+    if (!(aperture == 0.0f) || spf != 1 || max_bounces < 1) return 0;
+    if (!finite3(o) || !finite3(cd) || !(res_x >= 1.0 && res_x <= 65536.0) || !(res_y >= 1.0 && res_y <= 65536.0) ||
+        !(aspect >= 1e-3 && aspect <= 1e3) || !(fov >= 1.0 && fov <= 150.0) || !(F >= 1e-4 && F <= 1e6) ||
+        !(std::fabs(o[0]) + std::fabs(o[1]) + std::fabs(o[2]) <= 1e6))
+        return 0;
+    const double len = std::sqrt(cd[0] * cd[0] + cd[1] * cd[1] + cd[2] * cd[2]);
+    if (!(len >= 1e-12 && len <= 1e12)) return 0;
+    const double w[3] = { -cd[0] / len, -cd[1] / len, -cd[2] / len };
+    if (std::fabs(w[1]) > 0.999) return 0;
+    const double up[3] = { 0.0, 1.0, 0.0 };
+    double ud[3] = { up[1] * w[2] - up[2] * w[1], up[2] * w[0] - up[0] * w[2], up[0] * w[1] - up[1] * w[0] };
+    const double ul = std::sqrt(ud[0] * ud[0] + ud[1] * ud[1] + ud[2] * ud[2]);
+    if (!(ul >= 1e-6)) return 0;
+    for (double &x : ud) x /= ul;
+    const double vd[3] = { w[1] * ud[2] - w[2] * ud[1], w[2] * ud[0] - w[0] * ud[2], w[0] * ud[1] - w[1] * ud[0] };
+    const double t = std::tan(fov * 3.14159265358979323846 / 180.0 / 2.0), r = aspect * t;
+
+    constexpr double GROW = 1e-4, MARGIN = 1e-4;
+    struct Rect { double a0, a1, b0, b1; };
+    std::vector<Rect> rects;
+    for (size_t k = 0; k + 6 <= boxes.size(); k += 6) {
+        double reach = 0.0;
+        for (int i = 0; i < 3; i++)
+            reach = std::max(reach, std::max(std::fabs((double)boxes[k + i] - o[i]), std::fabs((double)boxes[k + 3 + i] - o[i])));
+        const double grow = GROW * reach + 1e-30;
+        Rect rc = { INFINITY, -INFINITY, INFINITY, -INFINITY };
+        for (int c = 0; c < 8; c++) {
+            double q[3];
+            for (int i = 0; i < 3; i++) q[i] = ((c >> i) & 1 ? (double)boxes[k + 3 + i] + grow : (double)boxes[k + i] - grow) - o[i];
+            const double depth = -(q[0] * w[0] + q[1] * w[1] + q[2] * w[2]);
+            const double ql = std::sqrt(q[0] * q[0] + q[1] * q[1] + q[2] * q[2]);
+            if (!(depth > 1e-3 * ql)) return 0;
+            const double a = (q[0] * ud[0] + q[1] * ud[1] + q[2] * ud[2]) / depth, b = (q[0] * vd[0] + q[1] * vd[1] + q[2] * vd[2]) / depth;
+            rc.a0 = std::min(rc.a0, a); rc.a1 = std::max(rc.a1, a);
+            rc.b0 = std::min(rc.b0, b); rc.b1 = std::max(rc.b1, b);
+        }
+        const double ma = MARGIN * (1.0 + std::max(std::fabs(rc.a0), std::fabs(rc.a1))), mb = MARGIN * (1.0 + std::max(std::fabs(rc.b0), std::fabs(rc.b1)));
+        rc.a0 -= ma; rc.a1 += ma; rc.b0 -= mb; rc.b1 += mb;
+        rects.push_back(rc);
+    }
+
+    const double ju = (std::fabs(ud[0]) / res_x + std::fabs(ud[1]) / res_y) * (1.0 + 1e-6);
+    const double jv = (std::fabs(vd[0]) / res_x + std::fabs(vd[1]) / res_y) * (1.0 + 1e-6);
+    const double jw = (std::fabs(w[0]) / res_x + std::fabs(w[1]) / res_y) * (1.0 + 1e-6);
+    const double cam1 = std::fabs(o[0]) + std::fabs(o[1]) + std::fabs(o[2]);
+    auto sq_max = [](double lo, double hi) { return std::max(lo * lo, hi * hi); };
+    size_t count = 0;
+    for (int ty = 0; ty < tiles_y; ty++) {
+        int g0 = INT32_MAX, g1 = INT32_MIN;
+        for (int ly = ty * 8; ly < std::min(ty * 8 + 8, local_rows); ly++) {
+            const int g = global_row(ly, rank, nranks, block_rows);
+            if (g >= height) continue;
+            g0 = std::min(g0, g); g1 = std::max(g1, g);
+        }
+        if (g0 > g1) continue;
+        const double v0 = -t + 2.0 * t * ((double)(g0 - 1) / res_y), v1 = -t + 2.0 * t * ((double)(g1 + 1) / res_y);
+        for (int tx = 0; tx < tiles_x; tx++) {
+            const int p0 = tx * 8, p1 = std::min(tx * 8 + 7, width - 1);
+            const double u0 = -r + 2.0 * r * ((double)(p0 - 1) / res_x), u1 = -r + 2.0 * r * ((double)(p1 + 1) / res_x);
+            const double nmax = std::sqrt(sq_max(u0, u1) + sq_max(v0, v1) + aspect * aspect);
+            const double gmax = nmax / F;
+            const double err = gmax * 1e-6 * (cam1 + F + 1.0);
+            const double a0 = u0 - gmax * ju - err, a1 = u1 + gmax * ju + err;
+            const double b0 = v0 - gmax * jv - err, b1 = v1 + gmax * jv + err;
+            const double c0 = aspect - gmax * jw - err, c1 = aspect + gmax * jw + err;
+            if (!(c0 > 0.05 * aspect)) continue;
+            double pa0 = std::min(a0 / c0, a0 / c1), pa1 = std::max(a1 / c0, a1 / c1);
+            double pb0 = std::min(b0 / c0, b0 / c1), pb1 = std::max(b1 / c0, b1 / c1);
+            const double ma = MARGIN * (1.0 + std::max(std::fabs(pa0), std::fabs(pa1))), mb = MARGIN * (1.0 + std::max(std::fabs(pb0), std::fabs(pb1)));
+            pa0 -= ma; pa1 += ma; pb0 -= mb; pb1 += mb;
+            bool hit = false;
+            for (const Rect &rc : rects)
+                if (pa0 <= rc.a1 && pa1 >= rc.a0 && pb0 <= rc.b1 && pb1 >= rc.b0) { hit = true; break; }
+            if (!hit) { empty[(size_t)ty * tiles_x + tx] = 1; count++; }
+        }
+    }
+    return count;
+}
+
+}
+
+extern "C" int mi3pt_host_sky_tiles(const void *nodes, size_t nodes_bytes, const void *raytrace_uniforms, int width, int height,
+                                    int rank, int nranks, int block_rows, uint8_t *empty_out, size_t capacity, size_t *ntiles_out)
+{
+    if (!nodes || !raytrace_uniforms || nodes_bytes == 0 || nodes_bytes % MI3PT_BVHNODE_STRIDE)
+        return pt_set_error(MI3PT_ERR_INVALID, "sky tiles: BVH bytes must be a non-zero multiple of 48");
+    if (width <= 0 || height <= 0 || width > 32768 || height > 32768 || nranks < 1 || rank < 0 || rank >= nranks || block_rows < 1)
+        return pt_set_error(MI3PT_ERR_INVALID, "sky tiles: bad image size or tile split");
+    const int local_rows = mi3pt_tile_local_rows(height, rank, nranks, block_rows);
+    const size_t ntiles = (size_t)((width + 7) / 8) * (size_t)((local_rows + 7) / 8);
+    if (ntiles_out) *ntiles_out = ntiles;
+    if (!empty_out) return MI3PT_OK;
+    if (capacity < ntiles) return pt_set_error(MI3PT_ERR_INVALID, "sky tiles: output too small");
+    std::vector<float> boxes;
+    const bool have = pt::sky_cut_of(static_cast<const uint8_t *>(nodes), nodes_bytes / MI3PT_BVHNODE_STRIDE, boxes);
+    std::vector<uint8_t> empty;
+    pt::sky_classify(boxes, have, static_cast<const uint8_t *>(raytrace_uniforms), width, local_rows, height, rank, nranks, block_rows, empty);
+    std::memcpy(empty_out, empty.data(), ntiles);
+    return MI3PT_OK;
+}
diff --git a/webgpu-pathtracer_amd/csrc/pt_internal.h b/webgpu-pathtracer_amd/csrc/pt_internal.h
--- a/webgpu-pathtracer_amd/csrc/pt_internal.h
+++ b/webgpu-pathtracer_amd/csrc/pt_internal.h
@@ -53,3 +53,8 @@
 };
 bool build_cw8(const uint8_t *src, size_t n, const float *verts , size_t nt,
                const std::vector<float> &wmax, Cw8Build &out, bool greedy = false);
+namespace pt {
+bool sky_cut_of(const uint8_t *src, size_t n, std::vector<float> &boxes);
+size_t sky_classify(const std::vector<float> &boxes, bool have_cut, const uint8_t *u, int width, int local_rows, int height,
+                    int rank, int nranks, int block_rows, std::vector<uint8_t> &empty);
+}
diff --git a/webgpu-pathtracer_amd/csrc/pt_kernels.h b/webgpu-pathtracer_amd/csrc/pt_kernels.h
--- a/webgpu-pathtracer_amd/csrc/pt_kernels.h
+++ b/webgpu-pathtracer_amd/csrc/pt_kernels.h
@@ -206,6 +206,7 @@
     int32_t num_cus;
     uint32_t *tile_cost;
     const uint32_t *tile_perm;
+    int32_t ntiles_active;
     const float4 *cam_base;
     int32_t six_waves;
     float *park;
@@ -231,7 +232,9 @@
 void launch_debug_math(int fn, const float *a, const float *b, float *out, size_t n, hipStream_t s);
 void launch_walk_stats(const uint64_t *counters, int nblocks, uint64_t *prev, uint64_t *out, uint64_t seq, hipStream_t s);
 int raytrace_grid_blocks(const Tile &tile);
-int raytrace_persistent_blocks(const Tile &tile, int nframes, int waves_per_cu, int num_cus, bool tuned = false, int waves_per_simd = 0);
+int raytrace_persistent_blocks(const Tile &tile, int nframes, int waves_per_cu, int num_cus, bool tuned = false, int waves_per_simd = 0, int job_tiles = 0);
+int raytrace_job_tiles(const RtLaunch &L);
+void launch_sky_samples(const RtLaunch &L, const uint32_t *tiles, int ntiles, uint64_t samples, hipStream_t s);
 void launch_pack_vertices(const float4 *tris, float4 *out, uint32_t ntris, hipStream_t s);
 void launch_patch_cull(float4 *packets, const uint32_t *cull, uint32_t npackets, hipStream_t s);
 
diff --git a/webgpu-pathtracer_amd/csrc/pt_kernels.hip b/webgpu-pathtracer_amd/csrc/pt_kernels.hip
--- a/webgpu-pathtracer_amd/csrc/pt_kernels.hip
+++ b/webgpu-pathtracer_amd/csrc/pt_kernels.hip
@@ -479,6 +479,27 @@
     r.y = (p00.y * wx0 + p10.y * fx) * wy0 + (p01.y * wx0 + p11.y * fx) * fy;
     r.z = (p00.z * wx0 + p10.z * fx) * wy0 + (p01.z * wx0 + p11.z * fx) * fy;
     return r;
+}
+
+PT_DEV f3 miss_light(const float4 *env, const f3 &d, float sinr, float cosr, const f3 &ray_color, const f3 &light, float env_intensity)
+{
+    float u, v;
+    env_uv_from_dir(d, sinr, cosr, u, v);
+    const f3 e = sample_env(env, ENV_W, ENV_H, u, v);
+    return light + (ray_color * e) * env_intensity;
+}
+
+PT_DEV uint32_t sample_seed(uint32_t px, uint32_t pgy, uint32_t res_w, uint32_t frame)
+{
+    return (px + pgy * res_w) + frame * 719393u + PT_SEED;
+}
+
+PT_DEV f3 camera_focal_point(uint32_t &seed, const f3 &fbase, float inv_res_x, float inv_res_y)
+{
+    float jx, jy;
+    rand_point_in_circle(seed, jx, jy);
+    const f3 jitter = F3(jx * inv_res_x, jy * inv_res_y, 0.0f);
+    return fbase + jitter;
 }
 
 PT_DEV float4 cdf_texel(const float4 *cdf, int W, int H, float u, float v)
@@ -935,7 +956,7 @@
     S.pinhole = (un.aperture == 0.0f && __float_as_uint(un.cam_pos[0]) != 0x80000000u &&
                  __float_as_uint(un.cam_pos[1]) != 0x80000000u && __float_as_uint(un.cam_pos[2]) != 0x80000000u) ? 1 : 0;
     S.tiles_x = (L.tile.tex_w + 7) >> 3;
-    S.ntiles_frame = S.tiles_x * ((L.tile.local_rows + 7) >> 3);
+    S.ntiles_frame = L.ntiles_active > 0 ? L.ntiles_active : S.tiles_x * ((L.tile.local_rows + 7) >> 3);
     S.ntiles = S.ntiles_frame * L.nframes;
     S.grp_jobs = (L.job_group > 0 && L.job_group < S.ntiles_frame) ? L.job_group * L.nframes : 0;
     S.grp_full = S.grp_jobs ? S.ntiles_frame / L.job_group : 0;
@@ -1742,13 +1763,7 @@
             if (wave_times) st_switch(4);
 #endif
             PT_SERVICE_PART();
-            if (shade_miss) {
-                
-                float u, v;
-                env_uv_from_dir(d, sinr, cosr, u, v);
-                const f3 env = sample_env(sc.env, ENV_W, ENV_H, u, v);
-                light = light + (ray_color * env) * un.env_intensity;
-            }
+            if (shade_miss) light = miss_light(sc.env, d, sinr, cosr, ray_color, light, un.env_intensity);
             PT_SERVICE_PART();
             if (shade_hit || shade_miss) {
                 mode = M_DEAD;
@@ -1828,7 +1843,7 @@
                                     (uint32_t)px < res_w && (uint32_t)pgy < res_h;
                     if (ok) {
                         got_job = true;
-                        seed = ((uint32_t)px + (uint32_t)pgy * res_w) + (un.frame + (uint32_t)fslot) * 719393u + PT_SEED;
+                        seed = sample_seed((uint32_t)px, (uint32_t)pgy, res_w, un.frame + (uint32_t)fslot);
                         job_px = (uint32_t)px; job_py = (uint32_t)pgy;
                         gx = (uint32_t)ply * (uint32_t)L.tile.tex_w + (uint32_t)px;
                         slot = (uint32_t)fslot << 16;
@@ -1866,10 +1881,8 @@
                     const f3 dir0 = camera_direction(cf, un.aspect, uvx, uvy);
                     fbase = cam_pos + dir0 * un.focal_distance;
                 }
-                float jx, jy, kx, ky;
-                rand_point_in_circle(seed, jx, jy);
-                const f3 jitter = F3(jx * inv_res_x, jy * inv_res_y, 0.0f);
-                const f3 focal = fbase + jitter;
+                float kx, ky;
+                const f3 focal = camera_focal_point(seed, fbase, inv_res_x, inv_res_y);
                 if (pinhole) {
                     (void)rand1(seed);
                     (void)rand1(seed);
@@ -2002,9 +2015,9 @@
     }
 }
 
-int raytrace_persistent_blocks(const Tile &tile, int nframes, int waves_per_cu, int num_cus, bool tuned, int waves_per_simd)
-{
-    const int ntiles = raytrace_grid_blocks(tile);
+int raytrace_persistent_blocks(const Tile &tile, int nframes, int waves_per_cu, int num_cus, bool tuned, int waves_per_simd, int job_tiles)
+{
+    const int ntiles = job_tiles > 0 ? job_tiles : raytrace_grid_blocks(tile);
     if (num_cus <= 0) num_cus = 256;
     if (waves_per_simd <= 0) waves_per_simd = tuned ? SM_TUNED_WAVES_PER_SIMD : SM_OTHER_WAVES_PER_SIMD;
     if (waves_per_cu > 4 * waves_per_simd) waves_per_cu = 0;
@@ -2026,6 +2039,11 @@
     const int tiles_x = (tile.tex_w + 7) / 8;
     const int tiles_y = (tile.local_rows + 7) / 8;
     return tiles_x * tiles_y;
+}
+
+int raytrace_job_tiles(const RtLaunch &L)
+{
+    return L.ntiles_active > 0 ? L.ntiles_active : raytrace_grid_blocks(L.tile);
 }
 
 static bool launch_packs(const RtLaunch &L)
@@ -2094,14 +2112,14 @@
         if (L.wave_times && L.diag_lite) return SM_TUNED_WAVES_PER_SIMD;
 #endif
         if (L.six_waves >= 0) return L.six_waves ? SM_SIX_WAVES_PER_SIMD : SM_TUNED_WAVES_PER_SIMD;
-        const long long jobs = (long long)raytrace_grid_blocks(L.tile) * (L.nframes > 0 ? L.nframes : 1);
+        const long long jobs = (long long)raytrace_job_tiles(L) * (L.nframes > 0 ? L.nframes : 1);
         return jobs >= (L.walk_min == PT_DEEP_WALK_MIN ? PT_SIX_WAVES_MIN_JOBS / 10 : PT_SIX_WAVES_MIN_JOBS) ? SM_SIX_WAVES_PER_SIMD : SM_TUNED_WAVES_PER_SIMD;
     }
     return SM_TUNED_WAVES_PER_SIMD;
 }
 static int persistent_blocks_for(const RtLaunch &L, const RtRoute &r)
 {
-    return raytrace_persistent_blocks(L.tile, L.nframes, L.waves_per_cu, L.num_cus, r.kind == 1 && r.lean, route_waves_per_simd(L, r));
+    return raytrace_persistent_blocks(L.tile, L.nframes, L.waves_per_cu, L.num_cus, r.kind == 1 && r.lean, route_waves_per_simd(L, r), L.ntiles_active);
 }
 RtRoute raytrace_route(const RtLaunch &L, int variant)
 {
@@ -2651,6 +2669,46 @@
     out[i] = r;
 }
 
+__global__ void __launch_bounds__(256) k_sky_samples(const RtLaunch L, const uint32_t *__restrict__ tiles, uint64_t samples)
+{
+    if (blockIdx.x == 0 && blockIdx.y == 0 && threadIdx.x == 0 && L.block_counters) {
+        L.block_counters[CNT_RAYS] += samples; L.block_counters[CNT_MISS] += samples; L.block_counters[CNT_PIXELS] += samples;
+    }
+    const RtUniforms &un = L.un;
+    const int lane = (int)(threadIdx.x & 63u);
+    const int fslot = (int)blockIdx.y * 4 + (int)(threadIdx.x >> 6);
+    if (fslot >= L.nframes) return;
+    const int tiles_x = (L.tile.tex_w + 7) >> 3;
+    const int ftile = (int)tiles[blockIdx.x];
+    const int trow = ftile / tiles_x;
+    const int px = (ftile - trow * tiles_x) * 8 + (lane & 7);
+    const int ply = trow * 8 + (lane >> 3);
+    const int pgy = local_to_global_row(ply, L.tile);
+    const uint32_t res_w = (uint32_t)un.res_x, res_h = (uint32_t)un.res_y;
+    const bool ok = px < L.tile.tex_w && ply < L.tile.local_rows && pgy < L.tile.tex_h &&
+                    (uint32_t)px < res_w && (uint32_t)pgy < res_h;
+    if (!ok) return;
+    uint32_t seed = sample_seed((uint32_t)px, (uint32_t)pgy, res_w, un.frame + (uint32_t)fslot);
+    const uint32_t gx = (uint32_t)ply * (uint32_t)L.tile.tex_w + (uint32_t)px;
+    const f3 fbase = xyz(L.cam_base[gx]);
+    const f3 focal = camera_focal_point(seed, fbase, 1.0f / un.res_x, 1.0f / un.res_y);
+    (void)rand1(seed);
+    (void)rand1(seed);
+    const f3 o = F3(un.cam_pos[0], un.cam_pos[1], un.cam_pos[2]);
+    const f3 d = normalize(focal - o);
+    float sinr, cosr;
+    ptm::sincos(un.env_rotation, sinr, cosr);
+    const f3 light = miss_light(L.scene.env, d, sinr, cosr, F3(1.0f, 1.0f, 1.0f), F3(0.0f, 0.0f, 0.0f), un.env_intensity);
+    const f3 pix = F3(0.0f, 0.0f, 0.0f) + light;
+    write_radiance(L, gx, (uint32_t)fslot, pix);
+}
+
+void launch_sky_samples(const RtLaunch &L, const uint32_t *tiles, int ntiles, uint64_t samples, hipStream_t s)
+{
+    if (ntiles <= 0 || L.nframes <= 0 || !L.cam_base || !tiles) return;
+    hipLaunchKernelGGL(k_sky_samples, dim3((unsigned)ntiles, (unsigned)((L.nframes + 3) / 4)), dim3(256), 0, s, L, tiles, samples);
+}
+
 __global__ void __launch_bounds__(256) k_walk_stats(const uint64_t *__restrict__ counters, int nblocks, uint64_t *prev, uint64_t *out, uint64_t seq)
 {
     __shared__ uint64_t sb[256], sr[256];
diff --git a/webgpu-pathtracer_amd/py/mi3pt_host/capi.py b/webgpu-pathtracer_amd/py/mi3pt_host/capi.py
--- a/webgpu-pathtracer_amd/py/mi3pt_host/capi.py
+++ b/webgpu-pathtracer_amd/py/mi3pt_host/capi.py
@@ -14,7 +14,7 @@
 (OPT_WALK_MIN, OPT_LEAF_MIN, OPT_SHADE_SPLIT, OPT_TAIL_POLICY, OPT_TOP_PACKETS, OPT_TRI_PAIR, OPT_JOB_REVERSE, OPT_JOB_GROUP,
  OPT_JOB_CHUNK, OPT_BATCH_LIMIT, OPT_BATCH, OPT_WAVES_PER_CU, OPT_CULL, OPT_WIDE, OPT_GATE, OPT_SLOT_SETS, OPT_PIPELINE,
  OPT_COST_ORDER, OPT_PRESENT_DEPTH, OPT_HOST_ANALYSES, OPT_GATHER_STAGED, OPT_DIAG_LITE,
- OPT_GATE_TIMEOUT_MS, OPT_GATE_RELEASES, OPT_DEBUG_SUPPRESS_DRAIN, OPT_CAMERA_BASE, OPT_PACKET_ORDER, OPT_SIX_WAVES, OPT_COLLAPSE, OPT_LAST_BUILD, OPT_WALK_ADAPT) = range(31)
+ OPT_GATE_TIMEOUT_MS, OPT_GATE_RELEASES, OPT_DEBUG_SUPPRESS_DRAIN, OPT_CAMERA_BASE, OPT_PACKET_ORDER, OPT_SIX_WAVES, OPT_COLLAPSE, OPT_LAST_BUILD, OPT_WALK_ADAPT, OPT_SKY_TILES) = range(32)
 COUNTER_NAMES = ("rays", "box_tests", "tri_tests", "hits", "misses", "stack_overflows", "pixels", "reserved")
 
 SYMBOLS = (
@@ -29,7 +29,7 @@
     "mi3pt_set_env_sampling", "mi3pt_device_build_bvh",
     "mi3pt_set_pipelining", "mi3pt_flush", "mi3pt_set_present_mode", "mi3pt_raytrace_launch_span", "mi3pt_batch_capacity", "mi3pt_debug_active_variant", "mi3pt_debug_last_launch", "mi3pt_submit_frames", "mi3pt_debug_set_packet_layout",
     "mi3pt_debug_intersect", "mi3pt_debug_math", "mi3pt_debug_wave_times", "mi3pt_host_build_bvh", "mi3pt_host_build_bvh_f64",
-    "mi3pt_host_env_cdf", "mi3pt_host_eight_wide_check", "mi3pt_debug_set_option", "mi3pt_debug_get_option",
+    "mi3pt_host_env_cdf", "mi3pt_host_eight_wide_check", "mi3pt_host_sky_tiles", "mi3pt_debug_set_option", "mi3pt_debug_get_option",
     "mi3pt_create_group", "mi3pt_group_size", "mi3pt_group_member",
     "mi3pt_tile_global_row", "mi3pt_tile_owner",
 )
@@ -105,6 +105,7 @@
     lib.mi3pt_host_build_bvh_f64.argtypes = [c_void_p, c_size_t, c_void_p, c_size_t, ctypes.POINTER(c_size_t), c_int]
     lib.mi3pt_host_env_cdf.argtypes = [c_void_p, c_int, c_int, c_void_p]
     lib.mi3pt_host_eight_wide_check.argtypes = [c_void_p, c_size_t, c_void_p, c_size_t, c_int, c_void_p]
+    lib.mi3pt_host_sky_tiles.argtypes = [c_void_p, c_size_t, c_void_p, c_int, c_int, c_int, c_int, c_int, c_void_p, c_size_t, ctypes.POINTER(c_size_t)]
     lib.mi3pt_device_count.argtypes = [ctypes.POINTER(c_int)]
     lib.mi3pt_device_name.argtypes = [c_int, ctypes.c_char_p, c_size_t]
     lib.mi3pt_tile_local_rows.argtypes = [c_int, c_int, c_int, c_int]
@@ -175,6 +176,18 @@
     count = ctypes.c_size_t(0)
     _check(lib, lib.mi3pt_host_build_bvh_f64(_ptr(pos), n, _ptr(nodes), nodes.nbytes, ctypes.byref(count), nthreads))
     return nodes[:count.value]
+
+
+def host_sky_tiles(nodes, raytrace_uniforms, width, height, rank=0, nranks=1, block_rows=8):
+    lib = load_library()
+    nd = np.ascontiguousarray(nodes)
+    un = np.frombuffer(bytes(raytrace_uniforms), np.uint8).copy()
+    n = ctypes.c_size_t(0)
+    _check(lib, lib.mi3pt_host_sky_tiles(_ptr(nd), nd.nbytes, _ptr(un), width, height, rank, nranks, block_rows, None, 0, ctypes.byref(n)))
+    out = np.zeros(max(n.value, 1), np.uint8)
+    _check(lib, lib.mi3pt_host_sky_tiles(_ptr(nd), nd.nbytes, _ptr(un), width, height, rank, nranks, block_rows, _ptr(out), out.nbytes, ctypes.byref(n)))
+    tiles_x = (width + 7) // 8
+    return out[:n.value].reshape(-1, tiles_x)
 
 
 def host_eight_wide_check(nodes, triangles, greedy=False):
```
